# cortes-ciriano-lab/DeMethify

Measured on AMD Instinct MI355X. Metric: NMF update iters/sec (1e6 CpG x 256 samples x 16 types), higher is better.
Workload: dtype f64; 1 GPU; headline_1e6x256_12+4; N_cpg=1000000, S_samples=256, n_known=12, n_unknown=4, inner_iters=20, restarts=64, restart_seed=1 + k, restart_placement=k mod n_gpus, parallelism=restart-sharded x1

## Files before the change

demethify_amd/_lib.py:

```python
from __future__ import annotations

import ctypes as C
from pathlib import Path

LIB_PATH = Path(__file__).resolve().parent / "libdemethify_hip.so"

DMF_OK = 0
DMF_PTR_DEVICE = 1
DMF_INIT_IN_UNIT_RANGE = 4
DMF_SELECT_COUNTS_F32_EXACT, DMF_SELECT_PURITY, DMF_SELECT_ALPHA_OUTSIDE_UNIT, DMF_SELECT_V_UNALIGNED = 1, 2, 4, 8
DMF_SELECT_X16 = 16
DMF_COUNTS_F64 = 2
DMF_WLS_TARGET_V, DMF_WLS_TARGET_DV = 0, 1
DMF_WLS_F64_ARRAYS = 8
DMF_ERR_BAD_ARG, DMF_ERR_NONFINITE, DMF_ERR_UNSUPPORTED = 1, 4, 5
DMF_ERR_BAD_SHAPE = 2
DMF_GRAM_INTEGER, DMF_GRAM_FP64, DMF_GRAM_LAST = 0, 1, 2
DMF_ROUTE_SOLVER, DMF_ROUTE_UPDATE_U = 0, 1
MOMENTUM_SCALARS = ("a1", "a2", "l_w", "l_w_prev", "l_h", "l_h_prev", "dsq", "rt_norm2", "u_norm2", "cf", "cf_prev",
                    "iters", "done", "arrive", "mom_n", "mom_i")
REPORT_INTS = ("N", "S", "n_c", "ND", "SD", "N16", "plane_stride", "has_D16", "has_X16", "has_W16", "has_Dt8", "has_mask_bits",
               "rtp_width", "rtp_borrows_rt", "n_test", "d_f32_exact")
REPORT_DBLS = ("kDsq", "kRtSumsq", "kDmax", "kF32ResidualMax", "kIntCountMax", "kRtOutsideUnit", "x16_dev", "x16_sum")
PROBLEM_ARRAYS = {"V": 0, "D": 1, "Rt": 2, "Rtp": 3, "D16": 4, "X16": 5, "W16": 6, "Dt8": 7, "mask_bits": 8, "consts": 9}
DMF_MODE_PARTIAL = 0
DMF_MODE_UNSUPERVISED = 1
MAX_K = 64
SMALL_MAX_S, SMALL_MAX_K, SMALL_MAX_NU, SMALL_MAX_ELEMENTS = 64, 16, 4, 1 << 20
SVD_MAX_S, SVD_MAX_NC, SVD_MAX_RANK, SVD_MAX_LDS = 512, 64, 64, 160 * 1024


def svd_project_lds_bytes(n_samples, rank):
    return 8 * (n_samples * rank + 8 * ((n_samples + 63) // 64 * 64 + 16) + 512)


KERNEL_ROWPASS, KERNEL_GRAM, KERNEL_ALPHA, KERNEL_COST = 0, 1, 2, 3
KERNEL_FAMILIES = ("rowpass", "gram", "alpha", "cost")

_p = C.c_void_p
_i64 = C.c_int64
_dbl_p = C.POINTER(C.c_double)

SIGNATURES = {
    "dmf_status_string": (C.c_char_p, [C.c_int]),
    "dmf_last_error": (C.c_char_p, []),
    "dmf_abi_version": (C.c_int, []),
    "dmf_context_create": (C.c_int, [C.c_int, _p, C.POINTER(_p)]),
    "dmf_context_destroy": (C.c_int, [_p]),
    "dmf_context_synchronize": (C.c_int, [_p]),
    "dmf_context_set_profiling": (C.c_int, [_p, C.c_int]),
    "dmf_context_kernel_time": (C.c_int, [_p, C.c_int, _dbl_p, C.POINTER(_i64)]),
    "dmf_context_reset_kernel_time": (C.c_int, [_p]),
    "dmf_context_set_generic": (C.c_int, [_p, C.c_int]),
    "dmf_context_set_x16": (C.c_int, [_p, C.c_int]),
    "dmf_context_set_rowpass_pair": (C.c_int, [_p, C.c_int]),
    "dmf_context_set_stop_confirmation": (C.c_int, [_p, C.c_int]),
    "dmf_problem_create": (C.c_int, [_p, _i64, _i64, _i64, _p, _p, _p, C.c_int, C.POINTER(_p)]),
    "dmf_problem_gather": (C.c_int, [_p, _p, _p, _i64, C.POINTER(_p)]),
    "dmf_problem_gather_device": (C.c_int, [_p, _p, _p, _i64, C.POINTER(_p)]),
    "dmf_problem_mask": (C.c_int, [_p, _p, _p, C.c_int, C.POINTER(_p)]),
    "dmf_solver_holdout_error": (C.c_int, [_p, _p, _dbl_p, C.POINTER(_i64)]),
    "dmf_problem_destroy": (C.c_int, [_p]),
    "dmf_problem_shape": (C.c_int, [_p, C.POINTER(_i64), C.POINTER(_i64), C.POINTER(_i64)]),
    "dmf_problem_gram_known": (C.c_int, [_p, _p, C.c_char_p, _i64]),
    "dmf_problem_report": (C.c_int, [_p, C.POINTER(_i64), _dbl_p]),
    "dmf_problem_copy_out": (C.c_int, [_p, C.c_int, _p, _i64]),
    "dmf_gram_i8_describe": (C.c_int, [_i64, _i64, _i64, _i64, C.c_int, C.c_char_p, _i64]),
    "dmf_solver_gram": (C.c_int, [_p, C.c_int, _p, C.c_char_p, _i64]),
    "dmf_solver_row_moments": (C.c_int, [_p, _p, C.c_char_p, _i64]),
    "dmf_solver_momentum_state": (C.c_int, [_p, _dbl_p, _p, _p]),
    "dmf_cost": (C.c_int, [_p, _p, _p, _i64, _p, C.c_int, _dbl_p]),
    "dmf_cost_describe": (C.c_int, [_i64, _i64, _i64, C.c_int, _i64, C.c_int, C.c_int, C.c_int, C.c_char_p, _i64]),
    "dmf_problem_cost_describe": (C.c_int, [_p, _p, _i64, C.c_char_p, _i64]),
    "dmf_project_simplex": (C.c_int, [_p, _p, _i64, _i64, C.c_double, C.c_int, _p]),
    "dmf_update_u": (C.c_int, [_p, _p, _p, _p, _p, _i64, _i64, C.c_int, C.c_int, _dbl_p, _p, _p]),
    "dmf_update_alpha": (C.c_int, [_p, _p, _p, _i64, _p, _p, _i64, C.c_int, _dbl_p, _p, _p]),
    "dmf_wls_intercept": (C.c_int, [_p, _p, _p, _i64, C.c_int, C.c_int, _p, C.POINTER(C.c_int)]),
    "dmf_wls_moments": (C.c_int, [_p, _p, _p, _i64, C.c_int, C.c_int, _p]),
    "dmf_nnls_normal": (C.c_int, [_p, _p, _p, _i64, _i64, _p, C.POINTER(C.c_int)]),
    "dmf_svd_gram": (C.c_int, [_p, _p, _p, C.c_int, _p, C.POINTER(_i64)]),
    "dmf_svd_factor": (C.c_int, [_p, _p, _p, _p, _i64, C.c_int, _p, C.POINTER(_p)]),
    "dmf_svd_finish": (C.c_int, [_p, _p, _i64, _i64, _p, _p, C.c_int, _p]),
    "dmf_percentile_axis0": (C.c_int, [_p, _p, _i64, _i64, _p, _i64, C.c_int, _p]),
    "dmf_nanpercentile_axis0": (C.c_int, [_p, _p, _i64, _i64, _p, _i64, C.c_int, _p]),
    "dmf_solver_create": (C.c_int, [_p, _p, _p, _p, _i64, C.c_int, C.c_int, C.POINTER(_p)]),
    "dmf_solver_set_purity": (C.c_int, [_p, _p, C.c_int]),
    "dmf_solver_step": (C.c_int, [_p, _i64, _i64, C.c_double, C.POINTER(_i64), C.POINTER(C.c_int)]),
    "dmf_solver_get": (C.c_int, [_p, C.c_int, _p, _p, _dbl_p, C.POINTER(_i64)]),
    "dmf_solver_match_components": (C.c_int, [_p, _p, _i64, _p, _p]),
    "dmf_solver_get_u_permuted": (C.c_int, [_p, C.POINTER(C.c_int32), _p]),
    "dmf_solver_get_u_by_row": (C.c_int, [_p, _p, _i64, C.POINTER(C.c_int32), _p]),
    "dmf_solver_cost": (C.c_int, [_p, _dbl_p]),
    "dmf_solver_cost_begin": (C.c_int, [_p]),
    "dmf_solver_cost_end": (C.c_int, [_p, _dbl_p]),
    "dmf_solver_destroy": (C.c_int, [_p]),
    "dmf_solver_describe": (C.c_int, [_p, _i64, C.c_char_p, _i64]),
    "dmf_select_describe": (C.c_int, [_i64, _i64, _i64, _i64, C.c_int, C.c_int, _i64, C.c_int, C.c_char_p, _i64]),
    "dmf_u_phase_describe": (C.c_int, [_i64, _i64, _i64, _i64, C.c_int, C.c_int, _i64, C.c_int, C.c_int, C.c_char_p, _i64]),
    "dmf_solver_u_phase_describe": (C.c_int, [_p, _i64, C.c_int, C.c_char_p, _i64]),
    "dmf_solver_stop_info": (C.c_int, [_p, C.POINTER(C.c_int), C.POINTER(_i64), C.POINTER(_i64), _dbl_p]),
    "dmf_solver_rowpass_launches": (C.c_int, [_p, C.POINTER(_i64), C.POINTER(_i64)]),
    "dmf_table_scan": (C.c_int, [C.c_char_p, C.c_char, C.POINTER(_i64), C.POINTER(C.c_int), C.POINTER(C.c_int),
                                 C.POINTER(C.c_int)]),
    "dmf_table_read": (C.c_int, [C.c_char_p, C.c_char, C.c_int, C.c_int, _i64, _p, _i64, C.c_double, _p, _i64, C.c_int]),
    "dmf_host_alloc": (_p, [C.c_size_t, C.POINTER(C.c_int)]),
    "dmf_host_free": (None, [_p, C.c_int]),
    "dmf_write_interval_csv": (C.c_int, [C.c_char_p, C.c_char_p, _p, _p, _i64, C.c_int, C.c_int, C.c_int]),
    "dmf_stage_upload": (C.c_int, [_p, _p, C.c_size_t, C.POINTER(C.c_void_p)]),
    "dmf_stage_free": (C.c_int, [_p, _p]),
    "dmf_stage_download": (C.c_int, [_p, _p, C.c_size_t, _p]),
    "dmf_mask_draw": (C.c_int, [_p, _p, C.POINTER(C.c_int), _i64, _i64, C.c_uint64, C.POINTER(C.c_void_p),
                                C.POINTER(_i64)]),
    "dmf_solve": (C.c_int, [_p, _p, _p, _p, _i64, C.c_int, _i64, _i64, C.c_double, C.c_int, _p, _p,
                            _dbl_p, C.POINTER(_i64)]),
    "dmf_solve_small_supported": (C.c_int, [_i64, _i64, _i64, _i64, C.c_int]),
    "dmf_solve_small": (C.c_int, [_p, _p, _i64, _p, _p, _p, _i64, C.c_int, _i64, _i64, C.c_double, _i64, C.c_int, _p, _p, _p, _p]),
    "dmf_solve_small_purity": (C.c_int, [_p, _p, _i64, _p, _p, _p, _p, _i64, C.c_int, _i64, _i64, C.c_double, _i64, C.c_int, _p, _p,
                                         _p, _p]),
}

_lib = None


class DemethifyHipError(RuntimeError):

    def __init__(self, status: int, where: str, detail: str = ""):
        self.status = status
        msg = f"{where}: status {status}"
        if detail:
            msg += f" ({detail})"
        super().__init__(msg)


def _preload_torch_hip_runtime():
    import importlib.util
    import os

    if os.environ.get("DEMETHIFY_SYSTEM_HIP") == "1":
        return
    try:
        spec = importlib.util.find_spec("torch")
        if spec is None or not spec.submodule_search_locations:
            return
        cand = Path(list(spec.submodule_search_locations)[0]) / "lib" / "libamdhip64.so"
        if cand.exists():
            C.CDLL(str(cand), mode=C.RTLD_GLOBAL)
    except Exception:
        pass


def load():
    global _lib
    if _lib is not None:
        return _lib
    if not LIB_PATH.exists():
        raise ImportError(
            f"{LIB_PATH} is missing: build it with `python -m demethify_amd._build` "
            "(there is no CPU fallback)")
    import sys

    torch = sys.modules.get("torch")
    if torch is not None:
        try:
            if torch.cuda.is_available():
                torch.cuda.init()
        except Exception:
            pass
    else:
        _preload_torch_hip_runtime()
    lib = C.CDLL(str(LIB_PATH))
    for name, (restype, argtypes) in SIGNATURES.items():
        fn = getattr(lib, name)
        fn.restype = restype
        fn.argtypes = argtypes
    _lib = lib
    return lib


def check(status: int, where: str):
    if status != DMF_OK:
        lib = load()
        text = lib.dmf_status_string(status).decode()
        err = lib.dmf_last_error().decode()
        raise DemethifyHipError(status, where, f"{text}; {err}" if err else text)
```

demethify_amd/csrc/dmf_api.h:

```cpp
#pragma once
#include <hip/hip_runtime.h>

#include <cmath>
#include <cstdio>
#include <cstdlib>
#include <cstring>
#include <memory>
#include <mutex>
#include <new>
#include <unordered_map>
#include <utility>
#include <vector>

#include "../../include/demethify_hip.h"
#include "dmf_internal.h"
#include "dmf_select.h"

using dmf::SolverState;

namespace dmf_api {

int hip_fail(hipError_t e, const char* what, const char* file, int line);

#define HIP_TRY(expr)                                                                          \
    do {                                                                                       \
        hipError_t e_ = (expr);                                                                \
        if (e_ != hipSuccess) return dmf_api::hip_fail(e_, #expr, __FILE_NAME__, __LINE__);    \
    } while (0)

#define DMF_TRY(expr)                 \
    do {                              \
        int s_ = (expr);              \
        if (s_ != DMF_OK) return s_;  \
    } while (0)

constexpr int kEventPool = 2048;

struct FamilyClock {
    std::vector<hipEvent_t> start, stop;
    int used = 0;
    double total_ms = 0.0;
    int64_t launches = 0;
};

}

struct dmf_context {
    int device = 0;
    hipStream_t stream = nullptr;
    bool own_stream = false;
    unsigned profiling = 0;
    int stop_confirmation = 0;
    int generic_level = 0;
    bool x16 = true;
    bool rowpass_pair = true;
    double* scratch = nullptr;
    hipMemPool_t pool = nullptr;
    std::unordered_map<void*, size_t> live;
    std::unordered_map<size_t, std::vector<void*>> kept;
    size_t kept_bytes = 0;
    std::vector<hipEvent_t> events;
    std::vector<double*> pinned_moms;
    std::vector<void*> pinned_states;
    hipStream_t copy_stream = nullptr;
    std::mutex copy_mutex;
    dmf_api::FamilyClock clocks[DMF_KERNEL_FAMILIES];
};

namespace dmf_api {

hipError_t pool_alloc(dmf_context* ctx, void** p, size_t bytes);
void pool_free(dmf_context* ctx, void* p);
hipError_t stage_alloc(dmf_context* ctx, hipStream_t st, void** p, size_t bytes);
void stage_release(dmf_context* ctx, hipStream_t st, void* p);

template <class T>
class DevBuf {
  public:
    DevBuf() = default;
    DevBuf(DevBuf&& o) noexcept : ctx_(o.ctx_), ptr_(o.ptr_), owned_(o.owned_), stage_(o.stage_) {
        o.ptr_ = nullptr, o.owned_ = false;
    }
    DevBuf& operator=(DevBuf&& o) noexcept {
        if (this != &o) {
            reset();
            ctx_ = o.ctx_, ptr_ = o.ptr_, owned_ = o.owned_, stage_ = o.stage_;
            o.ptr_ = nullptr, o.owned_ = false;
        }
        return *this;
    }
    ~DevBuf() { reset(); }
    hipError_t alloc(dmf_context* ctx, size_t count) {
        reset();
        const hipError_t e = pool_alloc(ctx, (void**)&ptr_, count * sizeof(T));
        if (e != hipSuccess) ptr_ = nullptr;
        ctx_ = ctx, owned_ = e == hipSuccess, stage_ = nullptr;
        return e;
    }
    hipError_t alloc_staged(dmf_context* ctx, size_t count, hipStream_t st) {
        reset();
        const hipError_t e = stage_alloc(ctx, st, (void**)&ptr_, count * sizeof(T));
        if (e != hipSuccess) ptr_ = nullptr;
        ctx_ = ctx, owned_ = e == hipSuccess, stage_ = st;
        return e;
    }
    T* release() {
        T* p = ptr_;
        ptr_ = nullptr, owned_ = false;
        return p;
    }
    void borrow(const T* p) { reset(), ptr_ = const_cast<T*>(p); }
    void reset() {
        if (owned_ && stage_ != nullptr) stage_release(ctx_, stage_, ptr_);
        else if (owned_) pool_free(ctx_, ptr_);
        ptr_ = nullptr, owned_ = false;
    }
    T* get() const { return ptr_; }
    operator T*() const { return ptr_; }
    T* operator->() const { return ptr_; }

  private:
    dmf_context* ctx_ = nullptr;
    T* ptr_ = nullptr;
    bool owned_ = false;
    hipStream_t stage_ = nullptr;
};

enum ProblemConst { kDsq, kRtSumsq, kDmax, kF32ResidualMax, kIntCountMax, kRtOutsideUnit, kProblemConsts };

struct JobTable {
    std::vector<short> h_k, h_l;
    std::vector<int> h_dst;
    DevBuf<short> k, l;
    DevBuf<int> dst;
    int n = 0;
    template <class Keep>
    void build(int l_first, int l_last, Keep keep) {
        for (int ll = l_first; ll <= l_last; ++ll)
            for (int kk = 0; kk <= ll; ++kk) {
                if (!keep(kk, ll)) continue;
                h_k.push_back((short)kk);
                h_l.push_back((short)ll);
                h_dst.push_back(dmf::tri(kk, ll));
            }
        n = (int)h_k.size();
    }
    int upload(dmf_context* ctx) {
        HIP_TRY(k.alloc(ctx, n));
        HIP_TRY(l.alloc(ctx, n));
        HIP_TRY(dst.alloc(ctx, n));
        HIP_TRY(hipMemcpyAsync(k, h_k.data(), n * sizeof(short), hipMemcpyHostToDevice, ctx->stream));
        HIP_TRY(hipMemcpyAsync(l, h_l.data(), n * sizeof(short), hipMemcpyHostToDevice, ctx->stream));
        HIP_TRY(hipMemcpyAsync(dst, h_dst.data(), n * sizeof(int), hipMemcpyHostToDevice, ctx->stream));
        return DMF_OK;
    }
};

}

struct dmf_problem {
    dmf_context* ctx = nullptr;
    int64_t N = 0, S = 0, n_c = 0;
    dmf_api::DevBuf<double> V, D, Rt;
    dmf_api::DevBuf<double> Rtp;
    dmf_api::DevBuf<double> consts;
    double h_consts[dmf_api::kProblemConsts] = {};
    dmf_api::DevBuf<unsigned short> D16;
    dmf_api::DevBuf<signed char> Dt8;
    int ND = 0;
    int SD = 0;
    int64_t N16 = 0, plane_stride = 0;
    dmf_api::DevBuf<unsigned short> X16;
    double x16_dev = 0.0, x16_sum = 0.0;
    bool d_f32_exact = false;
    dmf_api::DevBuf<double> gb_known;
    dmf::GramRan known_ran;
    dmf_api::DevBuf<unsigned char> mask_bits;
    dmf_api::DevBuf<unsigned short> W16;
    int64_t n_test = 0;
    dmf::ProblemView view() const {
        dmf::ProblemView v;
        v.V = V, v.D = D, v.D16 = D16, v.X16 = X16, v.Dt8 = Dt8;
        v.plane_stride = plane_stride, v.SD = SD, v.ND = ND;
        v.Rt = Rt, v.Rtp = Rtp;
        v.N = N, v.S = (int)S, v.n_c = (int)n_c;
        return v;
    }
};

constexpr size_t kPinnedStateBytes = (sizeof(SolverState) + 15) / 16 * 16 + 16;

struct dmf_solver {
    dmf_context* ctx = nullptr;
    const dmf_problem* p = nullptr;
    int64_t n_u = 0;
    int mode = 0;
    dmf::ShapeKey key;
    dmf::PathSpec spec;
    dmf_api::DevBuf<double> cm;
    dmf_api::DevBuf<double> beta_tab;
    int64_t beta_cap = 0;
    dmf_api::DevBuf<long long> slab_i8;
    int64_t slab_i8_words = 0;
    dmf_api::DevBuf<long long> acc_i8;
    dmf_api::DevBuf<double> purity;
    dmf_api::DevBuf<double> u2_partials;
    dmf_api::DevBuf<double> u, u_prev, u_next;
    dmf_api::DevBuf<double> alpha, alpha_prev;
    dmf_api::DevBuf<double> gb;
    dmf::GramRan last_gram;
    int last_gram_source = -1;
    dmf_api::DevBuf<double> slab;
    int64_t slab_doubles = 0;
    dmf_api::DevBuf<double> partials;
    dmf_api::DevBuf<SolverState> state;
    SolverState* h_state = nullptr;
    dmf_api::JobTable jobs;
    bool cf_pending = true;
    double* mom_host = nullptr;
    dmf_api::DevBuf<double> mom_dev;
    hipEvent_t cost_event = nullptr;
    bool cost_pending = false;
    bool in_flight = false;
    bool confirm_stops = false;
    double cf_stream = 0.0;
    long long cf_stream_iter = -1;
    long long n_rowpass = 0, n_rowpass_pair = 0;
    long long n_confirmed = 0, n_unconfirmed = 0;
    dmf::IterateView iterate() const {
        dmf::IterateView it;
        it.u = u, it.u_prev = u_prev, it.alpha = alpha, it.state = state;
        it.n_u = (int)n_u, it.mode = mode;
        return it;
    }
    dmf::AlphaView alpha_view() const {
        dmf::AlphaView a;
        a.gb = gb, a.alpha = alpha, a.alpha_prev = alpha_prev, a.purity = purity, a.state = state, a.partials = partials;
        a.S = (int)p->S, a.n_c = (int)p->n_c, a.n_u = (int)n_u;
        return a;
    }
    dmf::UScratch scratch() const {
        dmf::UScratch sc;
        sc.cm = cm, sc.beta = beta_tab, sc.slab = slab, sc.u2_partials = u2_partials;
        return sc;
    }
};

namespace dmf_api {

struct HandleDeleter {
    void operator()(dmf_problem* p) const { dmf_problem_destroy(p); }
    void operator()(dmf_solver* s) const { dmf_solver_destroy(s); }
};
using ProblemPtr = std::unique_ptr<dmf_problem, HandleDeleter>;
using SolverPtr = std::unique_ptr<dmf_solver, HandleDeleter>;

int clock_drain(dmf_context* ctx, FamilyClock& c);

struct FamilyScope {
    dmf_context* ctx;
    FamilyClock* c = nullptr;
    int slot = -1;
    FamilyScope(dmf_context* ctx_, int family) : ctx(ctx_) {
        if (!((ctx->profiling >> family) & 1u)) return;
        c = &ctx->clocks[family];
        if (c->start.empty()) {
            c->start.resize(kEventPool);
            c->stop.resize(kEventPool);
            for (int i = 0; i < kEventPool; ++i) {
                hipEventCreateWithFlags(&c->start[i], hipEventDisableSystemFence);
                hipEventCreateWithFlags(&c->stop[i], hipEventDisableSystemFence);
            }
        }
        if (c->used == kEventPool) clock_drain(ctx, *c);
        slot = c->used++;
        hipEventRecord(c->start[slot], ctx->stream);
    }
    ~FamilyScope() {
        if (c != nullptr) hipEventRecord(c->stop[slot], ctx->stream);
    }
};

int check_ctx(dmf_context* ctx);

template <class T>
int import_array(dmf_context* ctx, const void* src, size_t count, int flags, DevBuf<T>& dst) {
    dst.reset();
    if (count == 0) return DMF_OK;
    if (flags & DMF_PTR_DEVICE) {
        dst.borrow(static_cast<const T*>(src));
        return DMF_OK;
    }
    HIP_TRY(dst.alloc(ctx, count));
    HIP_TRY(hipMemcpyAsync(dst, src, count * sizeof(T), hipMemcpyHostToDevice, ctx->stream));
    HIP_TRY(hipStreamSynchronize(ctx->stream));
    return DMF_OK;
}
int export_array(dmf_context* ctx, const void* dev_src, size_t bytes, int flags, void* dst);

hipError_t enqueue_cost(dmf_context* ctx, const dmf::ProblemView& p, const double* u, const double* alpha, int n_u,
                        double* scratch, double* out);
bool cost_reads_u16_only(dmf_context* ctx, const dmf::ProblemView& p, int n_u);
int cost_to_host(dmf_context* ctx, const dmf::ProblemView& p, const double* u, const double* alpha, int n_u,
                 double* host_slot, bool wait);

int enqueue_u_phase(dmf_solver* s, int n_iter2, dmf::RowKind row);
dmf::RowKind standalone_row_kind(const dmf_solver* s, int n_iter2);
int enqueue_gram(dmf_solver* s, dmf::GramKind kind, bool heed_done = true, dmf::GramRan* ran = nullptr);
dmf::GramKind fp64_gram_kind(const dmf_solver* s);
int enqueue_alpha_phase(dmf_solver* s, dmf::AlphaKind kind, int n_iter2);
int fetch_state(dmf_solver* s);
int push_state(dmf_solver* s);

}
```

demethify_amd/csrc/dmf_api_context.hip:

```cpp
#include "dmf_api.h"

namespace dmf_api {

static thread_local char g_last_error[512] = "";

int hip_fail(hipError_t e, const char* what, const char* file, int line) {
    snprintf(g_last_error, sizeof(g_last_error), "%s failed at %s:%d: %s", what, file, line, hipGetErrorString(e));
    return DMF_ERR_HIP;
}

int clock_drain(dmf_context* ctx, FamilyClock& c) {
    if (c.used == 0) return DMF_OK;
    HIP_TRY(hipStreamSynchronize(ctx->stream));
    for (int i = 0; i < c.used; ++i) {
        float ms = 0.f;
        HIP_TRY(hipEventElapsedTime(&ms, c.start[i], c.stop[i]));
        c.total_ms += ms;
    }
    c.launches += c.used;
    c.used = 0;
    return DMF_OK;
}

static bool pool_enabled() {
    static const bool on = [] {
        const char* v = getenv("DEMETHIFY_NO_POOL");
        return !(v != nullptr && v[0] == '1');
    }();
    return on;
}
constexpr size_t kKeepMinBytes = (size_t)1 << 20, kKeepBytes = (size_t)24 << 30;
constexpr int kKeepPerSize = 3;
hipError_t pool_alloc(dmf_context* ctx, void** p, size_t bytes) {
    if (!pool_enabled() || ctx->pool == nullptr) return hipMalloc(p, bytes);
    if (bytes >= kKeepMinBytes) {
        auto it = ctx->kept.find(bytes);
        if (it != ctx->kept.end() && !it->second.empty()) {
            *p = it->second.back();
            it->second.pop_back();
            ctx->kept_bytes -= bytes;
            ctx->live[*p] = bytes;
            return hipSuccess;
        }
    }
    hipError_t e = hipMallocFromPoolAsync(p, bytes, ctx->pool, ctx->stream);
    if (e != hipSuccess && ctx->kept_bytes > 0) {
        (void)hipGetLastError();
        for (auto& kv : ctx->kept)
            for (void* q : kv.second) (void)hipFreeAsync(q, ctx->stream);
        ctx->kept.clear();
        ctx->kept_bytes = 0;
        (void)hipStreamSynchronize(ctx->stream);
        e = hipMallocFromPoolAsync(p, bytes, ctx->pool, ctx->stream);
    }
    if (e == hipSuccess && bytes >= kKeepMinBytes) ctx->live[*p] = bytes;
    return e;
}
void pool_free(dmf_context* ctx, void* p) {
    if (p == nullptr) return;
    if (!pool_enabled() || ctx->pool == nullptr) {
        (void)hipStreamSynchronize(ctx->stream);
        (void)hipFree(p);
        return;
    }
    auto it = ctx->live.find(p);
    if (it != ctx->live.end()) {
        const size_t bytes = it->second;
        ctx->live.erase(it);
        auto& slot = ctx->kept[bytes];
        if ((int)slot.size() < kKeepPerSize && ctx->kept_bytes + bytes <= kKeepBytes) {
            slot.push_back(p);
            ctx->kept_bytes += bytes;
            return;
        }
    }
    (void)hipFreeAsync(p, ctx->stream);
}

hipError_t stage_alloc(dmf_context* ctx, hipStream_t st, void** p, size_t bytes) {
    if (!pool_enabled() || ctx->pool == nullptr) return hipMalloc(p, bytes);
    return hipMallocFromPoolAsync(p, bytes, ctx->pool, st);
}
void stage_release(dmf_context* ctx, hipStream_t st, void* p) {
    if (!pool_enabled() || ctx->pool == nullptr) (void)hipFree(p);
    else (void)hipFreeAsync(p, st);
}

int export_array(dmf_context* ctx, const void* dev_src, size_t bytes, int flags, void* dst) {
    if (bytes == 0 || dst == nullptr) return DMF_OK;
    const hipMemcpyKind kind = (flags & DMF_PTR_DEVICE) ? hipMemcpyDeviceToDevice : hipMemcpyDeviceToHost;
    HIP_TRY(hipMemcpyAsync(dst, dev_src, bytes, kind, ctx->stream));
    HIP_TRY(hipStreamSynchronize(ctx->stream));
    return DMF_OK;
}

int check_ctx(dmf_context* ctx) {
    if (ctx == nullptr) return DMF_ERR_BAD_ARG;
    HIP_TRY(hipSetDevice(ctx->device));
    return DMF_OK;
}

}

using namespace dmf_api;

extern "C" {

const char* dmf_status_string(int status) {
    switch (status) {
        case DMF_OK: return "ok";
        case DMF_ERR_BAD_ARG: return "bad argument";
        case DMF_ERR_BAD_SHAPE: return "shape mismatch";
        case DMF_ERR_HIP: return "HIP runtime error";
        case DMF_ERR_NONFINITE: return "non-finite input";
        case DMF_ERR_UNSUPPORTED: return "unsupported size";
        case DMF_ERR_NO_DEVICE: return "no gfx950 device";
        default: return "unknown status";
    }
}

const char* dmf_last_error(void) { return g_last_error; }

int dmf_abi_version(void) { return 1; }

int dmf_context_create(int device, void* stream, dmf_context** out) {
    if (out == nullptr) return DMF_ERR_BAD_ARG;
    *out = nullptr;
    int count = 0;
    if (hipGetDeviceCount(&count) != hipSuccess || count <= 0) return DMF_ERR_NO_DEVICE;
    if (device < 0 || device >= count) return DMF_ERR_BAD_ARG;
    HIP_TRY(hipSetDevice(device));
    hipDeviceProp_t prop;
    HIP_TRY(hipGetDeviceProperties(&prop, device));
    if (strncmp(prop.gcnArchName, "gfx950", 6) != 0) {
        snprintf(g_last_error, sizeof(g_last_error), "device %d is %s, this library is built for gfx950",
                 device, prop.gcnArchName);
        return DMF_ERR_NO_DEVICE;
    }
    dmf_context* ctx = new (std::nothrow) dmf_context();
    if (ctx == nullptr) return DMF_ERR_BAD_ARG;
    ctx->device = device;
    if (stream != nullptr) {
        ctx->stream = (hipStream_t)stream;
    } else {
        hipError_t e = hipStreamCreateWithFlags(&ctx->stream, hipStreamNonBlocking);
        if (e != hipSuccess) {
            delete ctx;
            return hip_fail(e, "hipStreamCreate", __FILE_NAME__, __LINE__);
        }
        ctx->own_stream = true;
    }
    hipError_t e = hipMalloc((void**)&ctx->scratch, 4096 * sizeof(double));
    if (e != hipSuccess) {
        if (ctx->own_stream) hipStreamDestroy(ctx->stream);
        delete ctx;
        return hip_fail(e, "hipMalloc(scratch)", __FILE_NAME__, __LINE__);
    }
    if (pool_enabled()) {
        hipMemPoolProps props = {};
        props.allocType = hipMemAllocationTypePinned;
        props.handleTypes = hipMemHandleTypeNone;
        props.location.type = hipMemLocationTypeDevice;
        props.location.id = device;
        if (hipMemPoolCreate(&ctx->pool, &props) == hipSuccess && ctx->pool != nullptr) {
            uint64_t keep = UINT64_MAX;
            (void)hipMemPoolSetAttribute(ctx->pool, hipMemPoolAttrReleaseThreshold, &keep);
        } else {
            ctx->pool = nullptr;
            (void)hipGetLastError();
        }
    }
    *out = ctx;
    return DMF_OK;
}

int dmf_context_destroy(dmf_context* ctx) {
    if (ctx == nullptr) return DMF_OK;
    hipSetDevice(ctx->device);
    hipStreamSynchronize(ctx->stream);
    for (auto& c : ctx->clocks) {
        for (auto ev : c.start) hipEventDestroy(ev);
        for (auto ev : c.stop) hipEventDestroy(ev);
    }
    hipFree(ctx->scratch);
    for (auto& kv : ctx->kept)
        for (void* q : kv.second) (void)hipFreeAsync(q, ctx->stream);
    ctx->kept.clear();
    (void)hipStreamSynchronize(ctx->stream);
    for (void* h : ctx->pinned_states) (void)hipHostFree(h);
    for (double* h : ctx->pinned_moms) (void)hipHostFree(h);
    for (hipEvent_t ev : ctx->events) (void)hipEventDestroy(ev);
    if (ctx->copy_stream != nullptr) {
        hipStreamSynchronize(ctx->copy_stream);
        hipStreamDestroy(ctx->copy_stream);
    }
    if (ctx->pool != nullptr) (void)hipMemPoolDestroy(ctx->pool);
    if (ctx->own_stream) hipStreamDestroy(ctx->stream);
    delete ctx;
    return DMF_OK;
}

int dmf_stage_upload(dmf_context* ctx, const void* host, size_t bytes, void** out_dev) {
    if (ctx == nullptr || host == nullptr || out_dev == nullptr || bytes == 0) return DMF_ERR_BAD_ARG;
    HIP_TRY(hipSetDevice(ctx->device));
    std::lock_guard<std::mutex> lock(ctx->copy_mutex);
    if (ctx->copy_stream == nullptr) HIP_TRY(hipStreamCreateWithFlags(&ctx->copy_stream, hipStreamNonBlocking));
    void* d = nullptr;
    HIP_TRY(stage_alloc(ctx, ctx->copy_stream, &d, bytes));
    hipError_t e = hipMemcpyAsync(d, host, bytes, hipMemcpyHostToDevice, ctx->copy_stream);
    e = e != hipSuccess ? e : hipStreamSynchronize(ctx->copy_stream);
    if (e != hipSuccess) {
        stage_release(ctx, ctx->copy_stream, d);
        return hip_fail(e, "dmf_stage_upload", __FILE_NAME__, __LINE__);
    }
    *out_dev = d;
    return DMF_OK;
}

int dmf_stage_download(dmf_context* ctx, const void* dev, size_t bytes, void* host) {
    if (ctx == nullptr || dev == nullptr || host == nullptr || bytes == 0) return DMF_ERR_BAD_ARG;
    HIP_TRY(hipSetDevice(ctx->device));
    std::lock_guard<std::mutex> lock(ctx->copy_mutex);
    if (ctx->copy_stream == nullptr) HIP_TRY(hipStreamCreateWithFlags(&ctx->copy_stream, hipStreamNonBlocking));
    HIP_TRY(hipMemcpyAsync(host, dev, bytes, hipMemcpyDeviceToHost, ctx->copy_stream));
    HIP_TRY(hipStreamSynchronize(ctx->copy_stream));
    return DMF_OK;
}

int dmf_mask_draw(dmf_context* ctx, uint32_t key[624], int* pos, int64_t N, int64_t S, uint64_t threshold, void** out_bits,
                  int64_t* n_kept) {
    if (ctx == nullptr || key == nullptr || pos == nullptr || out_bits == nullptr || n_kept == nullptr) return DMF_ERR_BAD_ARG;
    *out_bits = nullptr;
    if (*pos < 0 || *pos > 624 || N < 1 || S < 1 || threshold > ((uint64_t)1 << 53)) return DMF_ERR_BAD_ARG;
    if (S > dmf::kMaskDrawMaxS || N > dmf::kMaskDrawMaxElements / S) return DMF_ERR_UNSUPPORTED;
    HIP_TRY(hipSetDevice(ctx->device));
    std::lock_guard<std::mutex> lock(ctx->copy_mutex);
    if (ctx->copy_stream == nullptr) HIP_TRY(hipStreamCreateWithFlags(&ctx->copy_stream, hipStreamNonBlocking));
    const hipStream_t st = ctx->copy_stream;
    constexpr size_t kStateWords = 624 + 4;
    DevBuf<unsigned char> bits;
    DevBuf<uint32_t> state;
    HIP_TRY(bits.alloc_staged(ctx, (size_t)N * (size_t)((S + 7) / 8), st));
    HIP_TRY(state.alloc_staged(ctx, kStateWords, st));
    uint32_t h_state[kStateWords] = {};
    std::memcpy(h_state, key, 624 * sizeof(uint32_t));
    HIP_TRY(hipMemcpyAsync(state, h_state, sizeof(h_state), hipMemcpyHostToDevice, st));
    HIP_TRY(dmf::launch_mask_draw(state, *pos, N, S, threshold, bits, reinterpret_cast<unsigned long long*>(state + 624), st));
    HIP_TRY(hipMemcpyAsync(h_state, state, sizeof(h_state), hipMemcpyDeviceToHost, st));
    HIP_TRY(hipStreamSynchronize(st));
    unsigned long long result[2];
    std::memcpy(result, h_state + 624, sizeof(result));
    std::memcpy(key, h_state, 624 * sizeof(uint32_t));
    *pos = (int)result[1];
    *n_kept = (int64_t)result[0];
    *out_bits = bits.release();
    return DMF_OK;
}

int dmf_stage_free(dmf_context* ctx, void* dev) {
    if (ctx == nullptr) return DMF_ERR_BAD_ARG;
    if (dev == nullptr) return DMF_OK;
    HIP_TRY(hipSetDevice(ctx->device));
    pool_free(ctx, dev);
    return DMF_OK;
}

int dmf_context_synchronize(dmf_context* ctx) {
    DMF_TRY(check_ctx(ctx));
    HIP_TRY(hipStreamSynchronize(ctx->stream));
    return DMF_OK;
}

int dmf_context_set_profiling(dmf_context* ctx, int enabled) {
    DMF_TRY(check_ctx(ctx));
    if (!enabled)
        for (auto& c : ctx->clocks) DMF_TRY(clock_drain(ctx, c));
    ctx->profiling = enabled == 0 ? 0u : enabled == 1 ? ~0u : (unsigned)enabled >> 1;
    return DMF_OK;
}

int dmf_context_kernel_time(dmf_context* ctx, int family, double* total_ms, int64_t* launches) {
    DMF_TRY(check_ctx(ctx));
    if (family < 0 || family >= DMF_KERNEL_FAMILIES) return DMF_ERR_BAD_ARG;
    FamilyClock& c = ctx->clocks[family];
    DMF_TRY(clock_drain(ctx, c));
    if (total_ms) *total_ms = c.total_ms;
    if (launches) *launches = c.launches;
    return DMF_OK;
}

int dmf_context_reset_kernel_time(dmf_context* ctx) {
    DMF_TRY(check_ctx(ctx));
    for (auto& c : ctx->clocks) {
        DMF_TRY(clock_drain(ctx, c));
        c.total_ms = 0.0;
        c.launches = 0;
    }
    return DMF_OK;
}

int dmf_context_set_generic(dmf_context* ctx, int enabled) {
    if (ctx == nullptr) return DMF_ERR_BAD_ARG;
    if (enabled < 0 || enabled > 4) return DMF_ERR_BAD_ARG;
    ctx->generic_level = enabled;
    return DMF_OK;
}

int dmf_context_set_x16(dmf_context* ctx, int enabled) {
    if (ctx == nullptr || enabled < 0 || enabled > 1) return DMF_ERR_BAD_ARG;
    ctx->x16 = enabled != 0;
    return DMF_OK;
}

int dmf_context_set_rowpass_pair(dmf_context* ctx, int enabled) {
    if (ctx == nullptr || enabled < 0 || enabled > 1) return DMF_ERR_BAD_ARG;
    ctx->rowpass_pair = enabled != 0;
    return DMF_OK;
}

int dmf_context_set_stop_confirmation(dmf_context* ctx, int mode) {
    if (ctx == nullptr || mode < 0 || mode > 2) return DMF_ERR_BAD_ARG;
    ctx->stop_confirmation = mode;
    return DMF_OK;
}

}
```

demethify_amd/csrc/dmf_api_solver.hip:

```cpp
#include "dmf_api.h"

namespace dmf_api {

using dmf::kSplitInnerSteps;

static int ensure_split_scratch(dmf_solver* s, int n_iter2) {
    dmf_context* ctx = s->ctx;
    if (s->cm == nullptr) HIP_TRY(s->cm.alloc(ctx, (size_t)dmf::u_phase_split_cm_doubles(s->p->N, (int)s->n_u)));
    if (s->beta_cap < n_iter2 || s->beta_tab == nullptr) {
        s->beta_cap = n_iter2 > 0 ? n_iter2 : 1;
        HIP_TRY(s->beta_tab.alloc(ctx, (size_t)s->beta_cap));
    }
    return DMF_OK;
}

int enqueue_u_phase(dmf_solver* s, int n_iter2, dmf::RowKind row) {
    dmf_context* ctx = s->ctx;
    const dmf::ProblemView pv = s->p->view();
    FamilyScope scope(ctx, DMF_KERNEL_ROWPASS);
    switch (row) {
        case dmf::RowKind::CmI8InnerRows:
            DMF_TRY(ensure_split_scratch(s, n_iter2));
            HIP_TRY(dmf::launch_u_phase_split_i8(pv, s->iterate(), n_iter2, s->scratch(), ctx->stream));
            return DMF_OK;
        case dmf::RowKind::UPhaseBig:
            HIP_TRY(dmf::launch_u_phase_big(pv, s->iterate(), n_iter2, ctx->stream));
            return DMF_OK;
        case dmf::RowKind::UPhaseMfmaSplit:
            DMF_TRY(ensure_split_scratch(s, n_iter2));
            HIP_TRY(dmf::launch_u_phase_split(pv, s->iterate(), n_iter2, s->scratch(), ctx->stream));
            return DMF_OK;
        case dmf::RowKind::UPhaseMfma:
            HIP_TRY(dmf::launch_u_phase_mfma(pv, s->iterate(), n_iter2, ctx->stream));
            return DMF_OK;
        case dmf::RowKind::UPhaseGram:
            HIP_TRY(dmf::launch_u_phase_gram(pv, s->iterate(), n_iter2, ctx->stream));
            return DMF_OK;
        case dmf::RowKind::UStepDirect:
            for (int t = 0; t < n_iter2; ++t) {
                HIP_TRY(dmf::launch_u_step_direct(pv, s->iterate(), s->u_next, t, ctx->stream));
                std::swap(s->u_prev, s->u);
                std::swap(s->u, s->u_next);
            }
            return DMF_OK;
        default: return DMF_ERR_BAD_ARG;
    }
}

dmf::RowKind standalone_row_kind(const dmf_solver* s, int n_iter2) {
    return dmf::plan_iteration(s->key, dmf::standalone_spec(s->spec), n_iter2, false).row;
}

struct GramI8Buffers {
    double* slab_bu = nullptr;
    long long* slab_i8 = nullptr;
    int64_t slab_i8_words = 0;
    long long* acc = nullptr;
    double* gb = nullptr;
    const int* done = nullptr;
};

static GramI8Buffers solver_i8_buffers(dmf_solver* s) {
    GramI8Buffers b;
    b.slab_bu = s->slab, b.slab_i8 = s->slab_i8, b.slab_i8_words = s->slab_i8_words, b.acc = s->acc_i8, b.gb = s->gb;
    b.done = &s->state->done;
    return b;
}

static int gram_i8_and_reduce(dmf_solver* s, const GramI8Buffers& b, int n_slabs, const double* u2_partials, int n_u2,
                              dmf::GramRan* ran = nullptr) {
    dmf_context* ctx = s->ctx;
    const dmf_problem* p = s->p;
    const int S = (int)p->S, n_c = (int)p->n_c, n_u = (int)s->n_u, nf = n_c * n_u + n_u * (n_u + 1) / 2;
    int ny = 0;
    HIP_TRY(dmf::launch_gram_i8(p->view(), s->u, n_u, s->jobs.k, s->jobs.l, nf, b.slab_i8, b.slab_i8_words, b.done, &ny,
                                ctx->stream, ran));
    HIP_TRY(dmf::launch_gram_v2_reduce(b.slab_i8, ny, nf, p->SD, b.slab_bu, n_slabs, n_u, S, b.acc, s->jobs.dst, b.gb, b.done,
                                       u2_partials, n_u2, s->state, ctx->stream));
    return DMF_OK;
}

static int gram_bu_cols_i8(dmf_solver* s, const GramI8Buffers& b, dmf::GramRan* ran = nullptr) {
    int n_slabs = 0;
    HIP_TRY(dmf::launch_bu_cols(s->p->view(), s->u, (int)s->n_u, b.slab_bu, b.done, &n_slabs, s->ctx->stream));
    return gram_i8_and_reduce(s, b, n_slabs, nullptr, 0, ran);
}

int enqueue_gram(dmf_solver* s, dmf::GramKind kind, bool heed_done, dmf::GramRan* ran) {
    dmf_context* ctx = s->ctx;
    const dmf::ProblemView pv = s->p->view();
    const int S = pv.S, n_u = (int)s->n_u;
    const int* done = heed_done ? &s->state->done : nullptr;
    FamilyScope scope(ctx, DMF_KERNEL_GRAM);
    if (kind == dmf::GramKind::BuColsI8) {
        GramI8Buffers b = solver_i8_buffers(s);
        b.done = done;
        return gram_bu_cols_i8(s, b, ran);
    }
    if (kind == dmf::GramKind::GramU) {
        int ny = 0;
        HIP_TRY(dmf::launch_gram_u(pv, s->u, n_u, s->slab, done, &ny, ctx->stream, ran));
        HIP_TRY(dmf::launch_gram_reduce(s->slab, ny, s->jobs.n, S, s->jobs.dst, s->gb, done, ctx->stream));
        return DMF_OK;
    }
    dmf::GramJobTable jobs{s->jobs.k, s->jobs.l, s->jobs.dst, s->jobs.n};
    if (kind == dmf::GramKind::GramMfma) {
        int ny = 0;
        HIP_TRY(dmf::launch_gram_mfma(pv, s->u, n_u, jobs, s->jobs.n - n_u, s->slab, s->slab_doubles, done, &ny, ctx->stream, ran));
        HIP_TRY(dmf::launch_gram_reduce(s->slab, ny, s->jobs.n, S, s->jobs.dst, s->gb, done, ctx->stream));
        return DMF_OK;
    }
    HIP_TRY(dmf::launch_gram(pv, s->u, n_u, jobs, s->slab, s->slab_doubles, s->gb, done, ctx->stream, ran));
    return DMF_OK;
}

dmf::GramKind fp64_gram_kind(const dmf_solver* s) {
    return s->spec.use_gram_spec ? dmf::GramKind::GramU : s->spec.use_gram_mfma ? dmf::GramKind::GramMfma : dmf::GramKind::Gram;
}

int enqueue_alpha_phase(dmf_solver* s, dmf::AlphaKind kind, int n_iter2) {
    FamilyScope scope(s->ctx, DMF_KERNEL_ALPHA);
    HIP_TRY(dmf::launch_alpha(kind, s->alpha_view(), n_iter2, s->ctx->stream));
    return DMF_OK;
}

constexpr int kLastGramI8Tail = 100, kLastGramFused = 101;
static dmf::GramRan* last_gram_slot(dmf_solver* s, int source) {
    if (s->last_gram_source == source) return nullptr;
    s->last_gram_source = source;
    return &s->last_gram;
}

static int enqueue_gram_i8_tail(dmf_solver* s, dmf::AlphaKind alpha, int n_iter2, int grid) {
    {
        FamilyScope scope(s->ctx, DMF_KERNEL_GRAM);
        DMF_TRY(gram_i8_and_reduce(s, solver_i8_buffers(s), grid, s->u2_partials, grid, last_gram_slot(s, kLastGramI8Tail)));
    }
    return enqueue_alpha_phase(s, alpha, n_iter2);
}

static int enqueue_outer_iteration(dmf_solver* s, int n_iter2) {
    dmf_context* ctx = s->ctx;
    s->in_flight = true;
    const dmf_problem* p = s->p;
    const int S = (int)p->S;
    const dmf::IterationPlan plan = dmf::plan_iteration(s->key, s->spec, n_iter2, s->purity != nullptr);
    if (plan.row == dmf::RowKind::RowpassV2) {
        int grid = 0;
        bool paired = false;
        {
            FamilyScope scope(ctx, DMF_KERNEL_ROWPASS);
            dmf::ProblemView pv = p->view();
            if (!s->key.x16) pv.X16 = nullptr;
            HIP_TRY(dmf::launch_rowpass_v2(pv, s->iterate(), n_iter2, s->scratch(), &grid, s->key.rowpass_pair, &paired,
                                           ctx->stream));
            ++s->n_rowpass;
            s->n_rowpass_pair += paired ? 1 : 0;
        }
        return enqueue_gram_i8_tail(s, plan.alpha, n_iter2, grid);
    }
    if (plan.row == dmf::RowKind::CmI8InnerBu) {
        int grid = 0;
        DMF_TRY(ensure_split_scratch(s, n_iter2));
        {
            FamilyScope scope(ctx, DMF_KERNEL_ROWPASS);
            HIP_TRY(dmf::launch_u_phase_split_i8_bu(p->view(), s->iterate(), n_iter2, s->scratch(), &grid, ctx->stream));
        }
        return enqueue_gram_i8_tail(s, plan.alpha, n_iter2, grid);
    }
    if (plan.row == dmf::RowKind::RowpassFused) {
        const int64_t n_full = p->N - (p->N & 15), n_tail = p->N - n_full;
        const dmf::ProblemView pv = p->view();
        int grid = 0, ny_tail = 0;
        {
            FamilyScope scope(ctx, DMF_KERNEL_ROWPASS);
            HIP_TRY(dmf::launch_rowpass_fused(pv.rows(0, n_full), s->iterate(), n_iter2, s->scratch(), &grid, ctx->stream));
        }
        if (n_tail > 0) {
            const dmf::ProblemView tail = pv.rows(n_full, n_tail);
            const dmf::IterateView it_tail = s->iterate().rows(n_full);
            HIP_TRY(dmf::launch_u_phase_mfma(tail, it_tail, n_iter2, ctx->stream));
            HIP_TRY(dmf::launch_sumsq_f64(it_tail.u, n_tail * s->n_u, ctx->scratch, s->u2_partials + grid, &s->state->done,
                                          ctx->stream));
            HIP_TRY(dmf::launch_gram_u(tail, it_tail.u, it_tail.n_u, s->slab + (int64_t)2 * grid * s->jobs.n * S,
                                       &s->state->done, &ny_tail, ctx->stream));
        }
        if (dmf::GramRan* ran = last_gram_slot(s, kLastGramFused))
            snprintf(ran->text, sizeof(ran->text), "k_rowpass_fused<%d,%d> phase C slabs=%d%s", (int)(p->n_c + 3) / 4, (int)s->n_u,
                     2 * grid, n_tail > 0 ? " + k_gram_u tail" : "");
        HIP_TRY(dmf::launch_finish_u_norm(s->u2_partials, grid + (n_tail > 0 ? 1 : 0), s->state, ctx->stream));
        {
            FamilyScope scope(ctx, DMF_KERNEL_GRAM);
            HIP_TRY(dmf::launch_gram_reduce(s->slab, 2 * grid + ny_tail, s->jobs.n, S, s->jobs.dst, s->gb,
                                            &s->state->done, ctx->stream));
        }
        return enqueue_alpha_phase(s, plan.alpha, n_iter2);
    }
    DMF_TRY(enqueue_u_phase(s, n_iter2, plan.row));
    HIP_TRY(dmf::launch_sumsq_f64(s->u, p->N * s->n_u, ctx->scratch, &s->state->u_norm2, &s->state->done,
                                  ctx->stream));
    HIP_TRY(dmf::launch_set_lh(s->state, ctx->stream));
    DMF_TRY(enqueue_gram(s, plan.gram, true, last_gram_slot(s, (int)plan.gram)));
    return enqueue_alpha_phase(s, plan.alpha, n_iter2);
}

int fetch_state(dmf_solver* s) {
    HIP_TRY(hipMemcpyAsync(s->h_state, s->state, sizeof(SolverState), hipMemcpyDeviceToHost, s->ctx->stream));
    HIP_TRY(hipStreamSynchronize(s->ctx->stream));
    s->in_flight = false;
    return DMF_OK;
}

int push_state(dmf_solver* s) {
    HIP_TRY(hipMemcpyAsync(s->state, s->h_state, sizeof(SolverState), hipMemcpyHostToDevice, s->ctx->stream));
    HIP_TRY(hipStreamSynchronize(s->ctx->stream));
    return DMF_OK;
}

constexpr int kMomRows = 64, kMomSteps = 64;

__global__ void k_set_momentum(SolverState* state, const double* mom, int stride, int rows, int n) {
    state->mom = mom;
    state->mom_stride = stride;
    state->mom_rows = rows;
    state->mom_i = 0;
    state->mom_n = n;
}

static double momentum_advance(double& a) {
#pragma clang fp contract(off)
    const double a0 = a;
    const double sq = 4.0 * a0 * a0;
    a = (1.0 + std::sqrt(1.0 + sq)) / 2.0;
    return (a0 - 1.0) / a;
}

static int upload_momentum_rows(dmf_solver* s, int rows, int n) {
    dmf_context* ctx = s->ctx;
    const int stride = 2 + 2 * n;
    if (s->mom_host == nullptr) {
        if (!ctx->pinned_moms.empty()) {
            s->mom_host = ctx->pinned_moms.back();
            ctx->pinned_moms.pop_back();
        } else {
            HIP_TRY(hipHostMalloc((void**)&s->mom_host, (size_t)kMomRows * (2 + 2 * kMomSteps) * sizeof(double)));
        }
        HIP_TRY(s->mom_dev.alloc(ctx, (size_t)kMomRows * (2 + 2 * kMomSteps)));
    }
    double a1 = s->h_state->a1, a2 = s->h_state->a2;
    for (int r = 0; r < rows; ++r) {
        double* row = s->mom_host + (size_t)r * stride;
        for (int t = 0; t < n; ++t) {
            row[2 + t] = momentum_advance(a1);
            row[2 + n + t] = momentum_advance(a2);
        }
        row[0] = a1;
        row[1] = a2;
    }
    HIP_TRY(hipMemcpyAsync(s->mom_dev, s->mom_host, (size_t)rows * stride * sizeof(double), hipMemcpyHostToDevice, ctx->stream));
    hipLaunchKernelGGL(k_set_momentum, dim3(1), dim3(1), 0, ctx->stream, s->state.get(), (const double*)s->mom_dev.get(), stride,
                       rows, n);
    HIP_TRY(hipGetLastError());
    return DMF_OK;
}

__global__ void k_set_tol(SolverState* state, double tol, double band) {
    state->tol = tol;
    state->band = band;
}

constexpr double kConfirmBand = 10.0;
constexpr double kGramCostRelErr = 1e-15;

static double* cost_slot(const dmf_solver* s) {
    return reinterpret_cast<double*>(reinterpret_cast<char*>(s->h_state) + kPinnedStateBytes - 16);
}

static int solver_setup(dmf_solver* s, const double* u0, const double* alpha0, int flags) {
    dmf_context* ctx = s->ctx;
    const dmf_problem* p = s->p;
    const int64_t N = p->N, S = p->S, n_c = p->n_c, n_u = s->n_u, K = n_c + n_u;
    dmf::ShapeKey& key = s->key;
    key.N = N;
    key.S = (int)S;
    key.n_c = (int)n_c;
    key.n_u = (int)n_u;
    key.nd = (p->ND > 0 && p->D16 != nullptr) ? p->ND : 0;
    key.SD = p->SD;
    key.x16 = key.nd > 0 && p->X16 != nullptr;
    key.rowpass_pair = ctx->rowpass_pair;
    key.level = ctx->generic_level;
    key.d_f32_exact = p->d_f32_exact;
    key.rtp_present = n_c == 0 || p->Rtp != nullptr;
    key.v_align = (unsigned)(reinterpret_cast<uintptr_t>(p->V.get()) & 15);
    key.rtp_align = (unsigned)(reinterpret_cast<uintptr_t>(p->Rtp.get()) & 15);
    key.alpha_unit = true;
    s->spec = dmf::select_path(key);
    if ((s->spec.use_v2 || s->spec.use_cm_i8) && !(flags & DMF_INIT_IN_UNIT_RANGE)) {
        bool in_unit = true;
        if (flags & DMF_PTR_DEVICE) {
            double outside = 0.0;
            HIP_TRY(dmf::launch_unit_range_check(alpha0, K * S, ctx->scratch, ctx->scratch + 2048, ctx->stream));
            HIP_TRY(hipMemcpyAsync(&outside, ctx->scratch + 2048, sizeof(double), hipMemcpyDeviceToHost, ctx->stream));
            HIP_TRY(hipStreamSynchronize(ctx->stream));
            in_unit = outside == 0.0;
        } else {
            for (int64_t i = 0; i < K * S; ++i)
                if (!(alpha0[i] >= 0.0 && alpha0[i] <= 1.0)) {
                    in_unit = false;
                    break;
                }
        }
        if (!in_unit) {
            key.alpha_unit = false;
            s->spec = dmf::select_path(key);
        }
    }
    if (!s->spec.supported) return DMF_ERR_UNSUPPORTED;
    s->in_flight = true;
    s->jobs.build((int)n_c, (int)K, [n_c, K](int k, int l) {
        if (l == (int)K && k < (int)n_c) return false;
        return !(l == (int)K && k == (int)K);
    });
    const int n_jobs = s->jobs.n;
    s->slab_doubles = dmf::gram_slab_doubles(N, (int)S, n_jobs);
    if (s->spec.use_gram_spec) {
        const int64_t spec = dmf::gram_u_slab_doubles(N, (int)S, (int)n_c, (int)n_u);
        if (spec > s->slab_doubles) s->slab_doubles = spec;
    }
    if (s->spec.use_gram_mfma) {
        const int64_t need = dmf::gram_mfma_slab_doubles(N, (int)S, n_jobs);
        if (need > s->slab_doubles) s->slab_doubles = need;
    }
    if (s->spec.use_fused) {
        const int64_t spec = dmf::rowpass_fused_slab_doubles(N - (N & 15), (int)S, (int)n_c, (int)n_u) +
                             dmf::gram_u_slab_doubles(16, (int)S, (int)n_c, (int)n_u);
        if (spec > s->slab_doubles) s->slab_doubles = spec;
    }
    if (s->spec.use_v2) {
        const int64_t bu = (int64_t)dmf::rowpass_v2_grid(N, (int)S) * n_u * S;
        if (bu > s->slab_doubles) s->slab_doubles = bu;
    }
    if (s->spec.use_gram_i8) {
        const int64_t bu = (int64_t)dmf::bu_cols_grid(N) * n_u * S;
        if (bu > s->slab_doubles) s->slab_doubles = bu;
        if (s->spec.use_cm_i8) {
            const int64_t bu2 = (int64_t)dmf::u_inner_bu_grid(N, (int)S) * n_u * S;
            if (bu2 > s->slab_doubles) s->slab_doubles = bu2;
        }
    }
    const size_t un = (size_t)N * n_u, an = (size_t)K * S;
    const size_t un_alloc = (un + 1) & ~(size_t)1;
    const size_t gbn = (size_t)(K + 1) * (K + 2) / 2 * S;
    const int nb_alpha = (int)((S + 63) / 64);
    HIP_TRY(s->u.alloc(ctx, un_alloc));
    HIP_TRY(s->u_prev.alloc(ctx, un_alloc));
    if (s->spec.u_path == 2) HIP_TRY(s->u_next.alloc(ctx, un_alloc));
    HIP_TRY(s->alpha.alloc(ctx, an));
    HIP_TRY(s->alpha_prev.alloc(ctx, an));
    HIP_TRY(s->gb.alloc(ctx, gbn));
    HIP_TRY(s->slab.alloc(ctx, (size_t)s->slab_doubles));
    HIP_TRY(s->partials.alloc(ctx, (size_t)2 * (nb_alpha + S)));
    HIP_TRY(s->u2_partials.alloc(ctx, 4096));
    if (s->spec.use_v2 || s->spec.use_gram_i8) {
        s->slab_i8_words = dmf::gram_i8_slab_words(N, p->SD, (int)n_c, (int)n_u);
        HIP_TRY(s->slab_i8.alloc(ctx, (size_t)s->slab_i8_words));
        const size_t acc_words = (size_t)dmf::gram_i8_acc_words((int)S, (int)n_c, (int)n_u);
        HIP_TRY(s->acc_i8.alloc(ctx, acc_words));
        HIP_TRY(hipMemsetAsync(s->acc_i8, 0, acc_words * sizeof(long long), ctx->stream));
    }
    HIP_TRY(s->state.alloc(ctx, 1));
    if (!ctx->pinned_states.empty()) {
        s->h_state = (SolverState*)ctx->pinned_states.back();
        ctx->pinned_states.pop_back();
    } else {
        HIP_TRY(hipHostMalloc((void**)&s->h_state, kPinnedStateBytes));
    }
    const hipMemcpyKind in_kind = (flags & DMF_PTR_DEVICE) ? hipMemcpyDeviceToDevice : hipMemcpyHostToDevice;
    HIP_TRY(hipMemsetAsync(s->state, 0, sizeof(SolverState), ctx->stream));
    HIP_TRY(hipMemsetAsync(s->gb, 0, gbn * sizeof(double), ctx->stream));
    HIP_TRY(hipMemcpyAsync(s->u, u0, un * sizeof(double), in_kind, ctx->stream));
    HIP_TRY(hipMemcpyAsync(s->u_prev, s->u, un * sizeof(double), hipMemcpyDeviceToDevice, ctx->stream));
    HIP_TRY(hipMemcpyAsync(s->alpha, alpha0, an * sizeof(double), in_kind, ctx->stream));
    HIP_TRY(hipMemcpyAsync(s->alpha_prev, s->alpha, an * sizeof(double), hipMemcpyDeviceToDevice, ctx->stream));
    DMF_TRY(s->jobs.upload(ctx));
    HIP_TRY(dmf::launch_scatter_known_block(p->gb_known, s->gb, (int)n_c, (int)K, (int)S, ctx->stream));
    HIP_TRY(dmf::launch_sumsq_f64(s->u, N * n_u, ctx->scratch, &s->state->u_norm2, nullptr, ctx->stream));
    HIP_TRY(dmf::launch_init_state(s->state, p->consts, s->alpha, (int)S, (int)n_c, (int)n_u, ctx->stream));
    if (!(flags & DMF_PTR_DEVICE)) HIP_TRY(hipStreamSynchronize(ctx->stream));
    return DMF_OK;
}

}

using namespace dmf_api;

extern "C" {

int dmf_solver_create(dmf_context* ctx, const dmf_problem* p, const double* u0, const double* alpha0,
                      int64_t n_u, int mode, int flags, dmf_solver** out) {
    DMF_TRY(check_ctx(ctx));
    if (out == nullptr) return DMF_ERR_BAD_ARG;
    *out = nullptr;
    if (p == nullptr || u0 == nullptr || alpha0 == nullptr || n_u < 1) return DMF_ERR_BAD_ARG;
    if (mode != DMF_MODE_PARTIAL && mode != DMF_MODE_UNSUPERVISED) return DMF_ERR_BAD_ARG;
    if (p->n_c + n_u > dmf::kMaxK) return DMF_ERR_UNSUPPORTED;
    SolverPtr s(new (std::nothrow) dmf_solver());
    if (s == nullptr) return DMF_ERR_BAD_ARG;
    s->ctx = ctx;
    s->p = p;
    s->n_u = n_u;
    s->mode = mode;
    DMF_TRY(solver_setup(s.get(), u0, alpha0, flags));
    *out = s.release();
    return DMF_OK;
}

int dmf_solver_step(dmf_solver* s, int64_t n_outer, int64_t n_iter2, double tol,
                    int64_t* iters_done_total, int* converged) {
    if (s == nullptr || n_outer < 0 || n_iter2 < 0 || n_iter2 > (1 << 20)) return DMF_ERR_BAD_ARG;
    dmf_context* ctx = s->ctx;
    DMF_TRY(check_ctx(ctx));
    const dmf_problem* p = s->p;
    const double gram_err = kGramCostRelErr * (double)p->N * (double)p->S * p->h_consts[kDmax] +
                            (s->key.x16 ? p->x16_dev * p->x16_sum : 0.0);
    s->confirm_stops = tol > 0.0 && ctx->stop_confirmation != 2 && (ctx->stop_confirmation == 1 || gram_err >= tol / 20.0);
    hipLaunchKernelGGL(k_set_tol, dim3(1), dim3(1), 0, ctx->stream, s->state.get(), tol, s->confirm_stops ? kConfirmBand : 1.0);
    HIP_TRY(hipGetLastError());
    if (s->cf_pending && tol > 0.0 && n_outer > 0) {
        FamilyScope scope(ctx, DMF_KERNEL_COST);
        HIP_TRY(enqueue_cost(ctx, p->view(), s->u, s->alpha, (int)s->n_u, ctx->scratch + 1024, &s->state->cf));
        s->cf_pending = false;
        s->cf_stream_iter = -2;
    }
    DMF_TRY(fetch_state(s));
    if (s->cf_stream_iter == -2) {
        s->cf_stream = s->h_state->cf;
        s->cf_stream_iter = s->h_state->iters;
    }
    int64_t check_every = s->spec.u_path != 2 ? 8 : 1;
    if (tol == 0.0 && s->spec.u_path != 2) check_every = kMomRows;
    const long long iters0 = s->h_state->iters;
    const dmf::IterationPlan plan = dmf::plan_iteration(s->key, s->spec, (int)n_iter2, s->purity != nullptr);
    const bool use_mom = n_iter2 >= 1 && n_iter2 <= kMomSteps && plan.row == dmf::RowKind::RowpassV2 &&
                         plan.alpha == dmf::AlphaKind::PhaseRow16;
    if (!use_mom && s->h_state->mom_n >= 0) {
        hipLaunchKernelGGL(k_set_momentum, dim3(1), dim3(1), 0, ctx->stream, s->state.get(), (const double*)nullptr, 0, 0, -1);
        HIP_TRY(hipGetLastError());
    }
    while (s->h_state->iters - iters0 < n_outer && s->h_state->done != 1) {
        const int64_t left = n_outer - (s->h_state->iters - iters0);
        const int64_t batch = left < check_every ? left : check_every;
        if (use_mom) DMF_TRY(upload_momentum_rows(s, (int)batch, (int)n_iter2));
        for (int64_t b = 0; b < batch; ++b) DMF_TRY(enqueue_outer_iteration(s, (int)n_iter2));
        DMF_TRY(fetch_state(s));
        if (s->h_state->iters > iters0) s->cf_pending = false;
        if (s->h_state->done == 2) {
            double cs = 0.0;
            DMF_TRY(cost_to_host(ctx, p->view(), s->u, s->alpha, (int)s->n_u, &cs, true));
            bool stop;
            if (s->cf_stream_iter == s->h_state->iters - 1) {
                stop = std::fabs(cs - s->cf_stream) < tol;
                s->n_confirmed += 1;
            } else {
                stop = std::fabs(s->h_state->cf - s->h_state->cf_prev) < tol;
                s->n_unconfirmed += 1;
            }
            s->cf_stream = cs;
            s->cf_stream_iter = s->h_state->iters;
            s->h_state->done = stop ? 1 : 0;
            DMF_TRY(push_state(s));
            check_every = 1;
        } else if (s->spec.u_path != 2 && check_every < 64 && check_every > 1) {
            check_every *= 2;
        }
    }
    if (iters_done_total) *iters_done_total = s->h_state->iters;
    if (converged) *converged = s->h_state->done == 1;
    return DMF_OK;
}

int dmf_solver_set_purity(dmf_solver* s, const double* purity, int flags) {
    if (s == nullptr || purity == nullptr) return DMF_ERR_BAD_ARG;
    dmf_context* ctx = s->ctx;
    DMF_TRY(check_ctx(ctx));
    if (s->mode != DMF_MODE_PARTIAL) return DMF_ERR_BAD_ARG;
    const size_t bytes = (size_t)s->p->S * sizeof(double);
    if (s->purity == nullptr) HIP_TRY(s->purity.alloc(ctx, (size_t)s->p->S));
    const hipMemcpyKind kind = (flags & DMF_PTR_DEVICE) ? hipMemcpyDeviceToDevice : hipMemcpyHostToDevice;
    HIP_TRY(hipMemcpyAsync(s->purity, purity, bytes, kind, ctx->stream));
    HIP_TRY(hipStreamSynchronize(ctx->stream));
    return DMF_OK;
}

int dmf_solver_get(dmf_solver* s, int flags, double* out_u, double* out_alpha, double* out_cost,
                   int64_t* out_iters) {
    if (s == nullptr) return DMF_ERR_BAD_ARG;
    dmf_context* ctx = s->ctx;
    DMF_TRY(check_ctx(ctx));
    const dmf_problem* p = s->p;
    DMF_TRY(export_array(ctx, s->u, (size_t)p->N * s->n_u * sizeof(double), flags, out_u));
    DMF_TRY(export_array(ctx, s->alpha, (size_t)(p->n_c + s->n_u) * p->S * sizeof(double), flags, out_alpha));
    if (s->cf_pending && out_cost != nullptr) {
        FamilyScope scope(ctx, DMF_KERNEL_COST);
        HIP_TRY(enqueue_cost(ctx, p->view(), s->u, s->alpha, (int)s->n_u, ctx->scratch + 1024, &s->state->cf));
        s->cf_pending = false;
    }
    DMF_TRY(fetch_state(s));
    if (out_cost) *out_cost = s->h_state->cf;
    if (out_iters) *out_iters = s->h_state->iters;
    return DMF_OK;
}

int dmf_solver_cost(dmf_solver* s, double* out_cost) {
    if (s == nullptr || out_cost == nullptr) return DMF_ERR_BAD_ARG;
    DMF_TRY(check_ctx(s->ctx));
    return cost_to_host(s->ctx, s->p->view(), s->u, s->alpha, (int)s->n_u, out_cost, true);
}

int dmf_solver_cost_begin(dmf_solver* s) {
    if (s == nullptr) return DMF_ERR_BAD_ARG;
    dmf_context* ctx = s->ctx;
    DMF_TRY(check_ctx(ctx));
    if (s->cost_event == nullptr) {
        if (!ctx->events.empty()) {
            s->cost_event = ctx->events.back();
            ctx->events.pop_back();
        } else {
            HIP_TRY(hipEventCreateWithFlags(&s->cost_event, hipEventDisableTiming));
        }
    }
    DMF_TRY(cost_to_host(ctx, s->p->view(), s->u, s->alpha, (int)s->n_u, cost_slot(s), false));
    HIP_TRY(hipEventRecord(s->cost_event, ctx->stream));
    s->cost_pending = true;
    return DMF_OK;
}

int dmf_solver_cost_end(dmf_solver* s, double* out_cost) {
    if (s == nullptr || out_cost == nullptr || !s->cost_pending) return DMF_ERR_BAD_ARG;
    DMF_TRY(check_ctx(s->ctx));
    HIP_TRY(hipEventSynchronize(s->cost_event));
    s->cost_pending = false;
    *out_cost = *cost_slot(s);
    return DMF_OK;
}

int dmf_solver_holdout_error(dmf_solver* s, const dmf_problem* full, double* sum_sq, int64_t* n_test) {
    if (s == nullptr || full == nullptr || sum_sq == nullptr || n_test == nullptr) return DMF_ERR_BAD_ARG;
    dmf_context* ctx = s->ctx;
    DMF_TRY(check_ctx(ctx));
    const dmf_problem* p = s->p;
    if (p->mask_bits == nullptr || full->mask_bits != nullptr || full->ctx != ctx) return DMF_ERR_BAD_ARG;
    if (full->N != p->N || full->S != p->S || full->n_c != p->n_c) return DMF_ERR_BAD_SHAPE;
    *n_test = p->n_test;
    *sum_sq = 0.0;
    if (p->n_test == 0) return DMF_OK;
    dmf::ProblemView pv;
    pv.N = p->N, pv.S = (int)p->S, pv.n_c = (int)p->n_c;
    pv.V = full->V, pv.Rt = p->Rt, pv.Rtp = p->Rtp;
    pv.D16 = p->W16, pv.SD = p->SD;
    DevBuf<double> weights;
    if (!cost_reads_u16_only(ctx, pv, (int)s->n_u)) {
        HIP_TRY(weights.alloc(ctx, (size_t)p->N * p->S));
        HIP_TRY(dmf::launch_holdout_weights_f64(p->mask_bits, weights, p->N, (int)p->S, ctx->stream));
        pv.D = weights, pv.D16 = nullptr, pv.SD = 0;
    }
    return cost_to_host(ctx, pv, s->u, s->alpha, (int)s->n_u, sum_sq, true);
}

static int solver_gram_enqueue(dmf_solver* s, int kind, double* out_gb, dmf::GramRan* ran) {
    dmf_context* ctx = s->ctx;
    const dmf_problem* p = s->p;
    const int64_t N = p->N, S = p->S, n_c = p->n_c, n_u = s->n_u, K = n_c + n_u;
    const size_t gbn = (size_t)(K + 1) * (K + 2) / 2 * S;
    DevBuf<double> slab_bu;
    DevBuf<long long> slab_i8, acc;
    if (kind == DMF_GRAM_LAST) {
        *ran = s->last_gram;
    } else if (kind == DMF_GRAM_FP64) {
        DMF_TRY(enqueue_gram(s, fp64_gram_kind(s), false, ran));
    } else {
        GramI8Buffers b;
        b.slab_i8_words = dmf::gram_i8_slab_words(N, p->SD, (int)n_c, (int)n_u);
        const size_t acc_words = (size_t)dmf::gram_i8_acc_words((int)S, (int)n_c, (int)n_u);
        HIP_TRY(slab_bu.alloc(ctx, (size_t)dmf::bu_cols_grid(N) * n_u * S));
        HIP_TRY(slab_i8.alloc(ctx, (size_t)b.slab_i8_words));
        HIP_TRY(acc.alloc(ctx, acc_words));
        HIP_TRY(hipMemsetAsync(acc, 0, acc_words * sizeof(long long), ctx->stream));
        b.slab_bu = slab_bu, b.slab_i8 = slab_i8, b.acc = acc, b.gb = s->gb;
        FamilyScope scope(ctx, DMF_KERNEL_GRAM);
        DMF_TRY(gram_bu_cols_i8(s, b, ran));
    }
    HIP_TRY(hipMemcpyAsync(out_gb, s->gb, gbn * sizeof(double), hipMemcpyDeviceToHost, ctx->stream));
    HIP_TRY(hipStreamSynchronize(ctx->stream));
    return DMF_OK;
}

int dmf_solver_gram(dmf_solver* s, int kind, double* out_gb, char* out_text, int64_t cap) {
    if (s == nullptr || out_gb == nullptr || (kind != DMF_GRAM_INTEGER && kind != DMF_GRAM_FP64 && kind != DMF_GRAM_LAST))
        return DMF_ERR_BAD_ARG;
    if (out_text != nullptr && cap < 1) return DMF_ERR_BAD_ARG;
    dmf_context* ctx = s->ctx;
    DMF_TRY(check_ctx(ctx));
    const dmf_problem* p = s->p;
    if (kind == DMF_GRAM_INTEGER &&
        (p->ND < 1 || p->D16 == nullptr || p->Dt8 == nullptr || (p->n_c > 0 && p->Rtp == nullptr) ||
         (reinterpret_cast<uintptr_t>(p->Rtp.get()) & 15) != 0 ||
         !dmf::gram_i8_supported((int)p->n_c, (int)s->n_u, p->ND, p->N, p->SD)))
        return DMF_ERR_UNSUPPORTED;
    dmf::GramRan ran;
    s->in_flight = true;
    const int status = solver_gram_enqueue(s, kind, out_gb, &ran);
    if (status != DMF_OK) (void)hipStreamSynchronize(ctx->stream);
    s->in_flight = false;
    if (status == DMF_OK && out_text != nullptr) snprintf(out_text, (size_t)cap, "%s", ran.text);
    return status;
}

static dmf::RowKind row_moments_kind(const dmf_solver* s) { return standalone_row_kind(s, kSplitInnerSteps + 1); }

static int solver_row_moments_enqueue(dmf_solver* s, dmf::RowKind row, double* out_cm, dmf::CmRan* ran) {
    dmf_context* ctx = s->ctx;
    const dmf::ProblemView pv = s->p->view();
    const int n_iter2 = kSplitInnerSteps + 1;
    DMF_TRY(ensure_split_scratch(s, 1));
    {
        FamilyScope scope(ctx, DMF_KERNEL_ROWPASS);
        if (row == dmf::RowKind::UPhaseMfmaSplit) {
            HIP_TRY(dmf::launch_u_phase_mfma_impl(pv, s->iterate(), n_iter2, s->cm, ctx->stream));
            dmf::describe_row_launch(dmf::u_phase_mfma_plan(pv.N, pv.S, pv.n_c, (int)s->n_u, n_iter2, pv.D16 != nullptr, pv.SD, true),
                                     ran->text, sizeof(ran->text));
        } else {
            HIP_TRY(dmf::launch_cm_i8(pv, s->iterate(), s->cm, ctx->stream, ran));
        }
    }
    const size_t n = (size_t)dmf::u_phase_split_cm_doubles(pv.N, (int)s->n_u);
    HIP_TRY(hipMemcpyAsync(out_cm, s->cm, n * sizeof(double), hipMemcpyDeviceToHost, ctx->stream));
    HIP_TRY(hipStreamSynchronize(ctx->stream));
    return DMF_OK;
}

int dmf_solver_row_moments(dmf_solver* s, double* out_cm, char* out_text, int64_t cap) {
    if (s == nullptr || out_cm == nullptr || (out_text != nullptr && cap < 1)) return DMF_ERR_BAD_ARG;
    dmf_context* ctx = s->ctx;
    DMF_TRY(check_ctx(ctx));
    const dmf::RowKind row = row_moments_kind(s);
    if (row != dmf::RowKind::CmI8InnerRows && row != dmf::RowKind::CmI8InnerBu && row != dmf::RowKind::UPhaseMfmaSplit)
        return DMF_ERR_UNSUPPORTED;
    DMF_TRY(fetch_state(s));
    if (s->h_state->done != 0) return DMF_ERR_BAD_ARG;
    dmf::CmRan ran;
    s->in_flight = true;
    const int status = solver_row_moments_enqueue(s, row, out_cm, &ran);
    if (status != DMF_OK) (void)hipStreamSynchronize(ctx->stream);
    s->in_flight = false;
    if (status == DMF_OK && out_text != nullptr) snprintf(out_text, (size_t)cap, "%s", ran.text);
    return status;
}

int dmf_solver_momentum_state(const dmf_solver* s, double* scalars, double* alpha_prev, double* u_prev) {
    if (s == nullptr || scalars == nullptr) return DMF_ERR_BAD_ARG;
    dmf_context* ctx = s->ctx;
    DMF_TRY(check_ctx(ctx));
    const dmf_problem* p = s->p;
    SolverState st;
    HIP_TRY(hipMemcpyAsync(&st, s->state.get(), sizeof(SolverState), hipMemcpyDeviceToHost, ctx->stream));
    if (alpha_prev != nullptr)
        HIP_TRY(hipMemcpyAsync(alpha_prev, s->alpha_prev.get(), (size_t)(p->n_c + s->n_u) * p->S * sizeof(double), hipMemcpyDeviceToHost,
                               ctx->stream));
    if (u_prev != nullptr)
        HIP_TRY(hipMemcpyAsync(u_prev, s->u_prev.get(), (size_t)p->N * s->n_u * sizeof(double), hipMemcpyDeviceToHost, ctx->stream));
    HIP_TRY(hipStreamSynchronize(ctx->stream));
    const double out[DMF_MOMENTUM_SCALARS] = {st.a1, st.a2, st.l_w, st.l_w_prev, st.l_h, st.l_h_prev, st.dsq, st.rt_norm2,
                                              st.u_norm2, st.cf, st.cf_prev, (double)st.iters, (double)st.done,
                                              (double)st.arrive, (double)st.mom_n, (double)st.mom_i};
    for (int i = 0; i < DMF_MOMENTUM_SCALARS; ++i) scalars[i] = out[i];
    return DMF_OK;
}

int dmf_solver_destroy(dmf_solver* s) {
    if (s == nullptr) return DMF_OK;
    dmf_context* ctx = s->ctx;
    hipSetDevice(ctx->device);
    if (s->cost_pending) (void)hipEventSynchronize(s->cost_event);
    if (s->in_flight) (void)hipStreamSynchronize(ctx->stream);
    if (s->cost_event) ctx->events.push_back(s->cost_event);
    if (s->mom_host) ctx->pinned_moms.push_back(s->mom_host);
    if (s->h_state) ctx->pinned_states.push_back(s->h_state);
    delete s;
    return DMF_OK;
}

int dmf_solver_describe(const dmf_solver* s, int64_t n_iter2, char* buf, int64_t cap) {
    if (s == nullptr || buf == nullptr || cap < 1 || n_iter2 < 0) return DMF_ERR_BAD_ARG;
    const dmf::IterationPlan plan = dmf::plan_iteration(s->key, s->spec, (int)n_iter2, s->purity != nullptr);
    dmf::describe_plan(s->key, plan, buf, (size_t)cap);
    return DMF_OK;
}

int dmf_solver_u_phase_describe(const dmf_solver* s, int64_t n_iter2, int route, char* buf, int64_t cap) {
    if (s == nullptr || buf == nullptr || cap < 1 || n_iter2 < 0 || n_iter2 > (1 << 20) ||
        (route != DMF_ROUTE_SOLVER && route != DMF_ROUTE_UPDATE_U))
        return DMF_ERR_BAD_ARG;
    dmf::describe_u_phase(s->key, s->spec, (int)n_iter2, s->purity != nullptr, route == DMF_ROUTE_UPDATE_U, buf, (size_t)cap);
    return DMF_OK;
}

int dmf_solver_stop_info(const dmf_solver* s, int* confirm_stops, int64_t* n_confirmed, int64_t* n_unconfirmed,
                         double* last_stream_cost) {
    if (s == nullptr) return DMF_ERR_BAD_ARG;
    if (confirm_stops) *confirm_stops = s->confirm_stops ? 1 : 0;
    if (n_confirmed) *n_confirmed = s->n_confirmed;
    if (n_unconfirmed) *n_unconfirmed = s->n_unconfirmed;
    if (last_stream_cost) *last_stream_cost = s->cf_stream_iter >= 0 ? s->cf_stream : std::nan("");
    return DMF_OK;
}

int dmf_solver_rowpass_launches(const dmf_solver* s, int64_t* total, int64_t* paired) {
    if (s == nullptr) return DMF_ERR_BAD_ARG;
    if (total) *total = s->n_rowpass;
    if (paired) *paired = s->n_rowpass_pair;
    return DMF_OK;
}

int dmf_solve(dmf_context* ctx, const dmf_problem* p, const double* u0, const double* alpha0, int64_t n_u,
              int mode, int64_t n_iter1, int64_t n_iter2, double tol, int flags, double* out_u,
              double* out_alpha, double* out_cost, int64_t* out_iters) {
    dmf_solver* raw = nullptr;
    DMF_TRY(dmf_solver_create(ctx, p, u0, alpha0, n_u, mode, flags, &raw));
    SolverPtr s(raw);
    DMF_TRY(dmf_solver_step(raw, n_iter1, n_iter2, tol, nullptr, nullptr));
    return dmf_solver_get(raw, flags, out_u, out_alpha, out_cost, out_iters);
}

}
```

demethify_amd/csrc/dmf_internal.h:

```cpp
#pragma once
#include <hip/hip_runtime.h>
#include <stdint.h>

#include "dmf_select.h"

namespace dmf {

struct SolverState {
    double a1;
    double a2;
    double l_w;
    double l_w_prev;
    double l_h;
    double l_h_prev;
    double dsq;
    double rt_norm2;
    double u_norm2;
    double cf;
    double cf_prev;
    double tol;
    long long iters;
    double band;
    int done;
    int arrive;
    const double* mom;
    int mom_stride, mom_rows, mom_i, mom_n;
};

__device__ __forceinline__ const double* momentum_row(const SolverState* __restrict__ state, int n_iter2) {
    return (state->mom != nullptr && state->mom_n == n_iter2 && state->mom_i < state->mom_rows)
               ? state->mom + (int64_t)state->mom_i * state->mom_stride
               : nullptr;
}

__host__ __device__ inline int tri(int k, int l) { return l * (l + 1) / 2 + k; }

constexpr int kMaxK = 64;
constexpr int kGramChunk = 16;
constexpr int kRowsPerBlockU = 64;

struct GramJobTable {
    const short* k_idx;
    const short* l_idx;
    const int* dst_row;
    int count;
};

struct PercentilePlan {
    long long k_prev, k_next;
    double gamma;
    int from_top;
    int pad;
};

struct ProblemView {
    const double* V = nullptr;
    const double* D = nullptr;
    const unsigned short* D16 = nullptr;
    const unsigned short* X16 = nullptr;
    const signed char* Dt8 = nullptr;
    int64_t plane_stride = 0;
    int SD = 0, ND = 0;
    const double* Rt = nullptr;
    const double* Rtp = nullptr;
    int64_t N = 0;
    int S = 0, n_c = 0;
    unsigned v_align() const { return (unsigned)(reinterpret_cast<uintptr_t>(V) & 15); }
    ProblemView rows(int64_t first, int64_t count) const {
        ProblemView r;
        r.V = V + first * S;
        r.D = D + first * S;
        r.Rt = Rt ? Rt + first * n_c : nullptr;
        r.Rtp = Rtp ? Rtp + first * ((n_c + 3) / 4 * 4) : nullptr;
        r.N = count;
        r.S = S;
        r.n_c = n_c;
        return r;
    }
};

struct IterateView {
    double* u = nullptr;
    double* u_prev = nullptr;
    const double* alpha = nullptr;
    SolverState* state = nullptr;
    int n_u = 0, mode = 0;
    IterateView rows(int64_t first) const {
        IterateView r = *this;
        r.u = u + first * n_u;
        r.u_prev = u_prev + first * n_u;
        return r;
    }
};

struct AlphaView {
    const double* gb = nullptr;
    double* alpha = nullptr;
    double* alpha_prev = nullptr;
    const double* purity = nullptr;
    SolverState* state = nullptr;
    double* partials = nullptr;
    int S = 0, n_c = 0, n_u = 0;
};

struct UScratch {
    double* cm = nullptr;
    double* beta = nullptr;
    double* slab = nullptr;
    double* u2_partials = nullptr;
};


hipError_t launch_convert_counts(const long long* src, double* dst, int64_t n, hipStream_t st);
hipError_t launch_max_f64(const double* x, int64_t n, double* scratch, double* out, hipStream_t st);
hipError_t launch_f32_residual_max(const double* x, int64_t n, double* scratch, double* out, hipStream_t st);
hipError_t launch_int_count_max(const double* x, int64_t n, double* scratch, double* out, hipStream_t st);
hipError_t launch_unit_range_check(const double* x, int64_t n, double* scratch, double* out, hipStream_t st);
hipError_t launch_sumsq_f64(const double* x, int64_t n, double* scratch, double* out,
                            const int* done_flag, hipStream_t st);
hipError_t launch_pad_rows(const double* src, double* dst, int64_t n_rows, int width_src, int width_dst,
                           hipStream_t st);
hipError_t launch_index_range_check(const long long* idx, int64_t n_idx, int64_t n_src, unsigned int* flag, hipStream_t st);
hipError_t launch_gather_rows(const double* src, double* dst, const long long* idx, int64_t n_idx,
                              int64_t width, hipStream_t st);

inline CostKey cost_key(const ProblemView& p, int n_u, int level) {
    CostKey k;
    k.S = p.S, k.n_c = p.n_c, k.n_u = n_u;
    k.d16 = p.D16 != nullptr;
    k.SD = p.SD;
    k.v_align = p.v_align();
    k.rtp_present = p.Rtp != nullptr;
    k.level = level;
    return k;
}
hipError_t launch_cost_plan(const CostPlan& plan, const ProblemView& p, const double* u, const double* alpha, int n_u,
                            double* scratch, double* out, hipStream_t st);
int vdv_cols_grid(int64_t N);
hipError_t launch_vdv_cols(const ProblemView& p, double* slab, double* out, hipStream_t st);

struct GramRan {
    char text[192] = "";
};

hipError_t launch_gram(const ProblemView& p, const double* u, int n_u, GramJobTable jobs, double* slab, int64_t slab_doubles,
                       double* gb, const int* done_flag, hipStream_t st, GramRan* ran = nullptr);
int64_t gram_slab_doubles(int64_t N, int S, int n_jobs);
hipError_t launch_gram_reduce(const double* slab, int ny, int n_jobs, int S, const int* dst_row,
                              double* gb, const int* done_flag, hipStream_t st);
bool gram_u_supported(int n_c, int n_u);
int64_t gram_u_slab_doubles(int64_t N, int S, int n_c, int n_u);
hipError_t launch_gram_u(const ProblemView& p, const double* u, int n_u, double* slab, const int* done_flag, int* ny_out,
                         hipStream_t st, GramRan* ran = nullptr);

struct RowLaunch {
    bool supported = false;
    int nw = 0;
    int grid = 0;
    size_t lds = 0;
    bool raise = false;
    int64_t blocks_per_wg = 0;
};
struct UPhaseMfmaPlan : RowLaunch {
    int nkc = 0, nu = 0;
    bool vec = false, d16 = false;
    bool split = false;
};
UPhaseMfmaPlan u_phase_mfma_plan(int64_t N, int S, int n_c, int n_u, int n_iter2, bool has_d16, int SD, bool split);
struct RowpassFusedPlan : RowLaunch {
    int nkc = 0, nu = 0;
};
RowpassFusedPlan rowpass_fused_plan(int64_t N, int S, int n_c, int n_u, int n_iter2);
struct UPhaseBigPlan : RowLaunch {
    int nkc = 0, gs = 16, n_u = 0;
};
UPhaseBigPlan u_phase_big_plan(int64_t N, int S, int n_c, int n_u, int n_iter2);
struct UPhaseGramPlan : RowLaunch {
    int nu = 0;
    bool alpha_in_lds = false;
};
UPhaseGramPlan u_phase_gram_plan(int64_t N, int S, int n_c, int n_u);
struct UStepDirectPlan : RowLaunch {
    int n_u = 0;
};
UStepDirectPlan u_step_direct_plan(int64_t N, int S, int n_c, int n_u);
int describe_row_launch(const UPhaseMfmaPlan& g, char* buf, size_t cap);
int describe_row_launch(const RowpassFusedPlan& g, char* buf, size_t cap);
int describe_row_launch(const UPhaseBigPlan& g, char* buf, size_t cap);
int describe_row_launch(const UPhaseGramPlan& g, char* buf, size_t cap);
int describe_row_launch(const UStepDirectPlan& g, char* buf, size_t cap);

hipError_t launch_u_phase_gram(const ProblemView& p, const IterateView& it, int n_iter2, hipStream_t st);
bool u_phase_gram_supported(int S, int n_c, int n_u);
bool u_phase_mfma_supported(int S, int n_c, int n_u);
hipError_t launch_u_phase_mfma(const ProblemView& p, const IterateView& it, int n_iter2, hipStream_t st);
hipError_t launch_u_phase_mfma_impl(const ProblemView& p, const IterateView& it, int n_iter2, double* cm_out, hipStream_t st);
bool rowpass_fused_supported(int S, int n_c, int n_u);
int rowpass_fused_grid(int64_t N, int S);
int64_t rowpass_fused_slab_doubles(int64_t N, int S, int n_c, int n_u);
hipError_t launch_rowpass_fused(const ProblemView& p, const IterateView& it, int n_iter2, const UScratch& scratch,
                                int* grid_out, hipStream_t st);
hipError_t launch_finish_u_norm(const double* u2_partials, int n, SolverState* state, hipStream_t st);
hipError_t launch_u_step_direct(const ProblemView& p, const IterateView& it, double* u_next, int t, hipStream_t st);
bool u_step_direct_supported(int S, int n_c, int n_u);

hipError_t launch_alpha(AlphaKind kind, const AlphaView& a, int n_iter2, hipStream_t st);
hipError_t launch_set_lh(SolverState* state, hipStream_t st);
hipError_t launch_project_simplex(const double* X, double* out, int K, int S, double z,
                                  hipStream_t st);
hipError_t launch_scatter_known_block(const double* gb_known, double* gb, int n_c, int K, int S,
                                      hipStream_t st);
hipError_t launch_init_state(SolverState* state, const double* consts, const double* alpha,
                             int S, int n_c, int n_u, hipStream_t st);

int64_t u_phase_split_cm_doubles(int64_t N, int n_u);
hipError_t launch_u_phase_split(const ProblemView& p, const IterateView& it, int n_iter2, const UScratch& scratch,
                                hipStream_t st);

bool cm_i8_supported(unsigned v_align, int S, int n_c, int n_u, int ND, int SD);
struct CmI8Launch {
    int mt0 = 0, mt1 = 0;
    int c_tile = 0, c_store = 0;
    size_t lds = 0;
    int grid = 0;
    int64_t blocks_per_wave = 0;
};
struct CmI8Panel {
    int col0 = 0, Sp = 0;
    bool s4 = false;
    int ncgx = 2;
    int tpl = 0;
    int n_launch = 0;
    CmI8Launch first, last;
};
constexpr int kCmMaxPanels = 8;
struct CmI8Plan {
    bool supported = false;
    int64_t N = 0;
    int S = 0, n_c = 0, n_u = 0;
    int nkc = 0, nd = 1;
    int nmt = 0, n_ct = 0;
    int n_panels = 0;
    CmI8Panel panel[kCmMaxPanels];
};
CmI8Plan cm_i8_plan(int64_t N, int S, int n_c, int n_u, int ND);
CmI8Launch cm_i8_launch_of(const CmI8Plan& g, int panel, int li);
int describe_cm_i8_plan(const CmI8Plan& g, char* buf, size_t cap);
struct CmRan {
    char text[2048] = "";
};
hipError_t launch_cm_i8(const ProblemView& p, const IterateView& it, double* cm, hipStream_t st, CmRan* ran = nullptr);
hipError_t launch_u_phase_split_i8(const ProblemView& p, const IterateView& it, int n_iter2, const UScratch& scratch,
                                   hipStream_t st);

bool u_inner_bu_supported(unsigned v_align, int S, int SD, int n_u, int n_iter2);
int u_inner_bu_grid(int64_t N, int S);
hipError_t launch_u_phase_split_i8_bu(const ProblemView& p, const IterateView& it, int n_iter2, const UScratch& scratch,
                                      int* grid_out, hipStream_t st);

bool u_phase_big_supported(int S, int n_c, int n_u, int n_iter2);
hipError_t launch_u_phase_big(const ProblemView& p, const IterateView& it, int n_iter2, hipStream_t st);

hipError_t launch_gram_mfma(const ProblemView& p, const double* u, int n_u, GramJobTable jobs, int n_dense, double* slab,
                            int64_t slab_doubles, const int* done_flag, int* ny_out, hipStream_t st, GramRan* ran = nullptr);
int64_t gram_mfma_slab_doubles(int64_t N, int S, int n_jobs);

hipError_t launch_gather_counts_int(const unsigned short* src16, const unsigned short* src_x16, const long long* idx,
                                    int64_t n_idx, int SD, int ND, unsigned short* D16, unsigned short* X16, int64_t N16,
                                    signed char* Dt8, int64_t plane_stride, unsigned int* max_out,
                                    unsigned long long* xsum_out, hipStream_t st);
constexpr double kX16MaxDev = 8.0 * 0x1p-53;
hipError_t launch_build_counts_int(const double* D, const double* V, int64_t N, int S, int ND, unsigned short* D16,
                                   unsigned short* X16, int64_t N16, int SD, signed char* Dt8, int64_t plane_stride,
                                   unsigned long long* x_stats, hipStream_t st);
hipError_t launch_build_dt8(const unsigned short* D16, int64_t N, int SD, int ND, signed char* Dt8, int64_t plane_stride,
                            hipStream_t st);
hipError_t launch_mask_problem(const double* srcV, const double* srcD, const unsigned short* src16,
                               const unsigned short* srcX, const unsigned char* bits, double* dstV, double* dstD,
                               unsigned short* dst16, unsigned short* dstX, unsigned short* W16, int64_t N, int64_t N16, int S,
                               int SD, unsigned long long* stats, hipStream_t st);
hipError_t launch_holdout_weights_f64(const unsigned char* bits, double* W, int64_t N, int S, hipStream_t st);
constexpr int64_t kMaskDrawMaxS = ((int64_t)1 << 31) - 1, kMaskDrawMaxElements = (int64_t)1 << 60;
hipError_t launch_mask_draw(unsigned int* key_io, int pos, int64_t N, int64_t S, unsigned long long threshold,
                            unsigned char* bits, unsigned long long* result, hipStream_t st);
bool rowpass_v2_supported(int S, int n_c, int n_u, int n_iter2);
int rowpass_v2_grid(int64_t N, int S);
hipError_t launch_rowpass_v2(const ProblemView& p, const IterateView& it, int n_iter2, const UScratch& scratch, int* grid_out,
                             bool pair, bool* paired_out, hipStream_t st);
bool rowpass_v2_pair_fits(int S, int n_u, int n_iter2);
bool gram_i8_supported(int n_c, int n_u, int ND, int64_t N, int SD);
struct GramI8Plan {
    bool supported = false;
    int xl = 1, nd = 1, ring = 8;
    int nf = 0, launches = 0;
    int nsh = 0, ny = 0;
    int64_t rows_per_wg = 0;
    int blocks = 0, last = 0;
    int tail = 0;
    bool xcd = false;
};
GramI8Plan gram_i8_plan(int64_t N, int SD, int n_c, int n_u, int ND);
void describe_gram_i8_plan(const GramI8Plan& g, char* buf, size_t cap);
int64_t gram_i8_slab_words(int64_t N, int SD, int n_c, int n_u);
int64_t gram_i8_acc_words(int S, int n_c, int n_u);
bool gram_i8_known_supported(int n_c, int ND, int64_t N, int SD);
int64_t gram_i8_slab_words_nf(int64_t N, int SD, int nf);
int64_t gram_i8_acc_words_nf(int S, int nf, int n_bu);
hipError_t launch_gram_i8(const ProblemView& p, const double* u, int n_u, const short* feat_a, const short* feat_b, int NF,
                          long long* slab, int64_t slab_words, const int* done_flag, int* ny_out, hipStream_t st,
                          GramRan* ran = nullptr);
int bu_cols_grid(int64_t N);
hipError_t launch_bu_cols(const ProblemView& p, const double* u, int n_u, double* slab, const int* done_flag,
                          int* n_slabs_out, hipStream_t st, bool* with_vdv = nullptr);
hipError_t launch_gram_v2_reduce(const long long* slab_i8, int ny, int NF, int SD, const double* slab_bu, int n_bu_slabs,
                                 int n_u, int S, long long* acc_words, const int* dst_row, double* gb, const int* done_flag,
                                 const double* u2_partials, int n_u2, SolverState* state, hipStream_t st);

hipError_t launch_percentile_pair(const double* x, int64_t n, int64_t m, PercentilePlan p0, PercentilePlan p1,
                                  double* out0, double* out1, hipStream_t st);
hipError_t launch_nanpercentile_pair(const double* x, int64_t n, int64_t m, PercentilePlan p0, PercentilePlan p1, double q0,
                                     double q1, double* out0, double* out1, hipStream_t st);
int64_t percentile_max_replicates();

int wls_moments_grid(int64_t N);
int64_t wls_slab_doubles(int64_t N, int S, int K);
hipError_t launch_wls_moments(const ProblemView& p, const double* u, int n_u, int target_dv, double* slab, double* mom,
                              hipStream_t st);
hipError_t launch_nnls_intercept(const double* gb, const double* mom, int K, int S, double* out, int* status, hipStream_t st);

constexpr int kSvdMaxS = 512, kSvdMaxNc = 64, kSvdMaxRank = 64;
constexpr size_t kSvdMaxLds = 160 * 1024;
size_t svd_project_lds_bytes(int S, int rank);
struct SvdColumns {
    double sign[kSvdMaxRank], scale[kSvdMaxRank];
};
bool svd_supported(int S, int n_c, int rank);
int svd_gram_grid(int64_t N, int S);
int64_t svd_gram_slab_doubles(int64_t N, int S);
hipError_t launch_svd_gram(const ProblemView& p, const double* H1, double* slab, int* flags, double* C, hipStream_t st);
int64_t svd_project_slab_doubles(int64_t N, int rank);
hipError_t launch_svd_project(const ProblemView& p, const double* H1, const double* Es, int rank, double* T, double* slab,
                              double* norms, hipStream_t st);
hipError_t launch_svd_finish(double* T, int64_t N, int rank, const SvdColumns& cols, hipStream_t st);

struct MatchColumns {
    int src[kMaxK];
};
int match_gram_grid(int64_t N, int n_u);
int64_t match_gram_slab_doubles(int64_t N, int n_u);
hipError_t launch_match_gram(const double* u, const double* anchor, const long long* idx, int64_t N, int64_t n_anchor_rows,
                             int n_u, double* slab, int* flags, double* P, hipStream_t st);
hipError_t launch_copy_cols_permuted(const double* u, double* dst, int64_t N, int n_u, const MatchColumns& cols,
                                     hipStream_t st);
constexpr long long kNotDrawn = 0x7fffffffffffffffLL;
hipError_t launch_first_occurrence(const long long* idx, int64_t M, int64_t n_dst_rows, long long* first,
                                   unsigned long long* n_bad, hipStream_t st);
hipError_t launch_copy_rows_first(const double* u, const long long* first, double* dst, int64_t n_dst_rows, int n_u,
                                  const MatchColumns& cols, hipStream_t st);

}
```

demethify_amd/csrc/dmf_kernels_rowpass2.hip:

```cpp
#include "dmf_device.h"
#include "dmf_dispatch.h"
#include "dmf_internal.h"
#include "dmf_ustep.h"
#include "dmf_fixedpoint.h"
#include <cstdlib>
#include <type_traits>

namespace dmf {

typedef double v4d __attribute__((ext_vector_type(4)));
typedef double v2d __attribute__((ext_vector_type(2)));
typedef unsigned int v4u __attribute__((ext_vector_type(4)));
typedef unsigned int v2u __attribute__((ext_vector_type(2)));
typedef int v4i __attribute__((ext_vector_type(4)));

#ifdef DMF_STAMPS
#define DMF2_STAMP_DECL unsigned long long st_last = dmf2_stamp(), st_seg[16] = {0, 0, 0, 0, 0, 0, 0, 0, 0, 0, 0, 0, 0, 0, 0, 0};
#define DMF2_STAMP(i) { const unsigned long long st_now = dmf2_stamp(); st_seg[i] += st_now - st_last; st_last = st_now; }
#define DMF2_STAMP_FLUSH                                                                                        \
    st_seg[15] = __builtin_amdgcn_s_getreg(4 | (31 << 11));                                                     \
    if (lane == 0) for (int i_ = 0; i_ < 16; ++i_) stamps_out[((size_t)blockIdx.x * 4 + wave) * 16 + i_] = st_seg[i_];
__device__ __forceinline__ unsigned long long dmf2_stamp() {
    unsigned long long t;
    __builtin_amdgcn_sched_barrier(0);
    asm volatile("s_memtime %0\n\ts_waitcnt lgkmcnt(0)" : "=s"(t)::"memory");
    __builtin_amdgcn_sched_barrier(0);
    return t;
}
#define DMF2_SUB_BEGIN unsigned long long st_sub = dmf2_stamp();
#define DMF2_SUB(i) { const unsigned long long st_now = dmf2_stamp(); st_seg[i] += st_now - st_sub; st_sub = st_now; }
#else
#define DMF2_STAMP_DECL
#define DMF2_STAMP(i)
#define DMF2_STAMP_FLUSH
#define DMF2_SUB_BEGIN
#define DMF2_SUB(i)
#endif

#ifndef DMF_V2_STAGGER
#define DMF_V2_STAGGER 12
#endif

namespace {
constexpr int kRowV = 66;
constexpr int kRowD = 72;
constexpr int kTileVBytes2 = 16 * kRowV * 8;
constexpr int kTileDBytes2 = 16 * kRowD * 2;
constexpr int kTileBytes2 = kTileVBytes2 + kTileDBytes2;
constexpr int kTileBytesX = 2 * kTileDBytes2;
}

template <int NU, bool AT_PREV>
__device__ __forceinline__ void inner_steps(double& uu, double& up, double cj, const double (&Ms)[NU], int b_lo, int b_hi,
                                            int t_end, int lane0) {
    int t2 = 0;
    for (; t2 + 1 < t_end; t2 += 2) {
        inner_step<NU, AT_PREV>(uu, up, cj, Ms, b_lo, b_hi, t2, lane0);
        inner_step<NU, AT_PREV>(up, uu, cj, Ms, b_lo, b_hi, t2 + 1, lane0);
    }
    if (t2 < t_end) {
        inner_step<NU, AT_PREV>(uu, up, cj, Ms, b_lo, b_hi, t2, lane0);
        const double tmp = uu;
        uu = up;
        up = tmp;
    }
}

constexpr int kUnrolledSteps = 20;

template <int NU, bool AT_PREV>
__device__ __forceinline__ void inner_steps_unrolled(double& uu, double& up, double cj, const double (&Ms)[NU], int b_lo, int b_hi,
                                                     int lane0) {
    static_assert(kUnrolledSteps % 2 == 0 && kUnrolledSteps <= 64, "pairs of steps; beta_t in lane t of one register pair");
#pragma unroll
    for (int t2 = 0; t2 < kUnrolledSteps; t2 += 2) {
        inner_step<NU, AT_PREV>(uu, up, cj, Ms, b_lo, b_hi, t2, lane0);
        inner_step<NU, AT_PREV>(up, uu, cj, Ms, b_lo, b_hi, t2 + 1, lane0);
    }
}

template <int NKC, int NU, int MAXW = 4, bool XS = false, bool PAIR = false>
__global__ __launch_bounds__(64 * MAXW, MAXW == 4 ? 2 : 1) void k_rowpass_v2(
    const double* __restrict__ V, const unsigned short* __restrict__ D16, const unsigned short* __restrict__ X16, int SD,
    const double* __restrict__ Rtp,
    const double* __restrict__ alpha, double* __restrict__ u, double* __restrict__ u_prev,
    const SolverState* __restrict__ state, int64_t N, int S, int n_c, int n_iter2, int mode, int nd,
    double* __restrict__ slab, double* __restrict__ u2_partials
#ifdef DMF_STAMPS
    , unsigned long long* __restrict__ stamps_out
#endif
    ) {
    static_assert(NU >= 1 && NU <= 4, "one phase-B pass per block, 4x4x4 MFMA for the c product");
    static_assert(!PAIR || (XS && MAXW == 4), "the pair schedule: X16 form, two workgroups per CU");
    constexpr int NSET = PAIR ? 2 : 1;
    constexpr int NCT = 4 * NKC;
    constexpr int NP = NU * (NU + 1) / 2;
    constexpr int SLOT = (NU + 2) & ~1;
    constexpr int NV = NU * SLOT;
    extern __shared__ double lds_dyn[];
    if (state->done) return;

    const int NW = blockDim.x >> 6;
    const int wave = __builtin_amdgcn_readfirstlane(threadIdx.x >> 6);
    const int lane = threadIdx.x & 63;
    const int wcol0 = wave * 64;

    double* __restrict__ beta_tab = lds_dyn;
    double* __restrict__ ubuf = beta_tab + ((n_iter2 + 1) & ~1);
    double* __restrict__ red = ubuf + NSET * 16 * NU;
    double* __restrict__ u2red = red + NSET * MAXW * NV * 16;
    constexpr int TB = XS ? kTileBytesX : kTileBytes2;
    char* __restrict__ tile = reinterpret_cast<char*>(u2red + MAXW) + (size_t)wave * TB;
    struct BlockTile {
        double* V;
        unsigned short *D, *X;
    };
    auto block_tile = [&](int set) {
        char* const t = tile + (size_t)set * NW * TB;
        unsigned short* const d = reinterpret_cast<unsigned short*>(t + (XS ? 0 : kTileVBytes2));
        return BlockTile{reinterpret_cast<double*>(t), d, d + 16 * kRowD};
    };

    if (const double* __restrict__ mrow = momentum_row(state, n_iter2)) {
        const double lw_prev = state->l_w_prev, lw = state->l_w;
        for (int t2 = threadIdx.x; t2 < n_iter2; t2 += blockDim.x)
            beta_tab[t2] = fmin(mrow[2 + t2], t2 == 0 ? 0.9999 * sqrt(lw_prev / lw) : 0.9999);
    } else if (threadIdx.x == 0) {
        fill_momentum_table(state, n_iter2, beta_tab);
    }
    for (int i = threadIdx.x; i < NSET * MAXW * NV * 16; i += blockDim.x) red[i] = 0.0;
    const double inv_lw = 1.0 / state->l_w;
    const double m_scale_v = -inv_lw * 0x1p-52;
    const double m_scale = __hiloint2double(__builtin_amdgcn_readfirstlane(__double2hiint(m_scale_v)),
                                            __builtin_amdgcn_readfirstlane(__double2loint(m_scale_v)));

    const int m16 = lane & 15, q = lane >> 4;
    const int sw_row = (m16 >= 4 && m16 < 12) ? 1 : 0;
    const int qs = q ^ sw_row;
    const int c_row = 8 * (q & 1) + 4 * (q >> 1);
    const int mC = m16 ^ ((q == 1 || q == 2) ? 4 : 0);
    const int e_col = wcol0 + 4 * (m16 & 3) + (m16 >> 2);
    const int k_col = wcol0 + 4 * q;
    double a1r[4][NKC > 0 ? NKC : 1];
    double a2r[4][4];
    v4i pdg[7];
    int pj = 0, pl = 0;
    while ((pl + 1) * (pl + 2) / 2 <= m16) ++pl;
    pj = m16 - pl * (pl + 1) / 2;
    {
        const bool pair_ok = m16 < NP;
        const bool a2_ok = (m16 & 3) < NU;
#pragma unroll
        for (int t = 0; t < 4; ++t) {
#pragma unroll
            for (int kc = 0; kc < NKC; ++kc) {
                const int row = kc * 4 + q, col = e_col + 16 * t;
                a1r[t][kc] = (row < n_c && col < S) ? -alpha[(int64_t)row * S + col] : 0.0;
            }
#pragma unroll
            for (int r = 0; r < 4; ++r) {
                const int col = k_col + 16 * t + r;
                a2r[t][r] = (col < S && a2_ok) ? alpha[(int64_t)(n_c + (m16 & 3)) * S + col] * inv_lw : 0.0;
            }
        }
#pragma unroll
        for (int g = 0; g < 4; ++g) {
            unsigned int lo[4], hi[4], tl[4], th[4];
#pragma unroll
            for (int i = 0; i < 4; ++i) {
                const int col = wcol0 + 16 * q + 4 * g + i;
                const bool in = pair_ok && col < S;
                const double aj = in ? alpha[(int64_t)(n_c + pj) * S + col] : 0.0;
                const double al = in ? alpha[(int64_t)(n_c + pl) * S + col] : 0.0;
                z_to_biased(aj, al, lo[i], hi[i]);
            }
            transpose4(lo, tl);
            transpose4(hi, th);
            pdg[0][g] = (int)(tl[0] ^ 0x80808080u);
            pdg[1][g] = (int)(tl[1] ^ 0x80808080u);
            pdg[2][g] = (int)(tl[2] ^ 0x80808080u);
            pdg[3][g] = (int)(tl[3] ^ 0x80808080u);
            pdg[4][g] = (int)(th[0] ^ 0x80808080u);
            pdg[5][g] = (int)(th[1] ^ 0x80808080u);
            pdg[6][g] = (int)th[2];
        }
    }
    __syncthreads();

    double bu[4] = {0.0, 0.0, 0.0, 0.0};
    double u2_acc = 0.0;
    DMF2_STAMP_DECL
    const int64_t nblk = (N + 15) / 16;
    const int nk = (int)((nblk - blockIdx.x + gridDim.x - 1) / gridDim.x);

    const int ld_row = lane >> 5;
    const int ld_col = (lane & 31) * 2;
    int ld_gcol = wcol0 + ld_col;
    const int last_pair = (S - 1) & ~1;
    if (ld_gcol > last_pair) ld_gcol = last_pair;
    const int d_row = lane >> 3, d_col = (lane & 7) * 8;
    const int ld_col_sw = ((lane & 31) ^ 2) * 2;
    v2d pv[NSET][XS ? 1 : 8];
    v4u pd[NSET][2], px[NSET][XS ? 2 : 1];
    double nrt[NSET][NKC > 0 ? NKC : 1];
    double pu, pup;
    constexpr int RPWB = 64 / NU;
    const int rl = lane / NU, jb = lane - rl * NU;
    const bool b_lane = rl < 16 && rl < RPWB;
    const unsigned int v_off = (unsigned int)(ld_row * S + ld_gcol) * 8u;
    const unsigned int d_off = (unsigned int)(d_row * SD + wcol0 + d_col) * 2u;
    const unsigned int r_off = (unsigned int)(m16 * NCT + q) * 8u;
    const unsigned int u_off = b_lane ? (unsigned int)lane * 8u : 0xFFFFFFF0u;
    auto span = [](int64_t bytes) { return (unsigned int)(bytes < 0 ? 0 : (bytes > 0x7FFFFFFF ? 0x7FFFFFFF : bytes)); };
    auto prefetch_u = [&](int64_t blk) {
        const int64_t r0 = blk * 16;
        const int64_t left = N - r0;
        const __amdgpu_buffer_rsrc_t ru = __builtin_amdgcn_make_buffer_rsrc((void*)(u + r0 * NU), 0, span(left * NU * 8), 0x00020000);
        const __amdgpu_buffer_rsrc_t rp = __builtin_amdgcn_make_buffer_rsrc((void*)(u_prev + r0 * NU), 0, span(left * NU * 8), 0x00020000);
        const v2u a = __builtin_amdgcn_raw_buffer_load_b64(ru, u_off, 0, 0);
        const v2u b = __builtin_amdgcn_raw_buffer_load_b64(rp, u_off, 0, 0);
        pu = __hiloint2double((int)a.y, (int)a.x);
        pup = __hiloint2double((int)b.y, (int)b.x);
    };
    auto prefetch_tile = [&](int64_t blk, int set) {
        const int64_t r0 = blk * 16;
        const int64_t left = N - r0;
        if (NKC > 0) {
            const __amdgpu_buffer_rsrc_t rr = __builtin_amdgcn_make_buffer_rsrc((void*)(Rtp + r0 * NCT), 0, span(left * NCT * 8), 0x00020000);
#pragma unroll
            for (int kc = 0; kc < NKC; ++kc) {
                const v2u a = __builtin_amdgcn_raw_buffer_load_b64(rr, r_off, kc * 32, 0);
                nrt[set][kc] = __hiloint2double((int)a.y, (int)a.x);
            }
        }
        if constexpr (!XS) {
            const __amdgpu_buffer_rsrc_t rv = __builtin_amdgcn_make_buffer_rsrc((void*)(V + r0 * S), 0, span(left * S * 8), 0x00020000);
#pragma unroll
            for (int i = 0; i < 8; ++i) {
                const v4u a = __builtin_amdgcn_raw_buffer_load_b128(rv, v_off, 2 * i * S * 8, 0);
                pv[set][i] = v2d{__hiloint2double((int)a.y, (int)a.x), __hiloint2double((int)a.w, (int)a.z)};
            }
        } else {
            const __amdgpu_buffer_rsrc_t rx = __builtin_amdgcn_make_buffer_rsrc((void*)(X16 + r0 * SD), 0, span((int64_t)16 * SD * 2), 0x00020000);
            px[set][0] = __builtin_amdgcn_raw_buffer_load_b128(rx, d_off, 0, 0);
            px[set][1] = __builtin_amdgcn_raw_buffer_load_b128(rx, d_off, 8 * SD * 2, 0);
        }
        {
            const __amdgpu_buffer_rsrc_t rd = __builtin_amdgcn_make_buffer_rsrc((void*)(D16 + r0 * SD), 0, span((int64_t)16 * SD * 2), 0x00020000);
            pd[set][0] = __builtin_amdgcn_raw_buffer_load_b128(rd, d_off, 0, 0);
            pd[set][1] = __builtin_amdgcn_raw_buffer_load_b128(rd, d_off, 8 * SD * 2, 0);
        }
    };
    auto pair_set = [&](int s) { return (PAIR && s + 1 < nk && wave == (s + 1) % NW) ? 1 : 0; };
    if (nk > 0) {
        prefetch_u(blockIdx.x + (int64_t)pair_set(0) * gridDim.x);
        prefetch_tile(blockIdx.x, 0);
        if (PAIR && nk > 1) prefetch_tile(blockIdx.x + gridDim.x, 1);
    }

    double* __restrict__ const mine_c = red + (size_t)wave * NV * 16 + (m16 * NU + q) * SLOT;
    double* __restrict__ const mine_m1 = red + (size_t)wave * NV * 16 + (4 * q * NU + pl) * SLOT + 1 + (pj - pl + NU) % NU;
    double* __restrict__ const mine_m2 = red + (size_t)wave * NV * 16 + (4 * q * NU + pj) * SLOT + 1 + (pl - pj) % NU;

    auto tile_store = [&](int set) {
        const BlockTile T = block_tile(set);
        if constexpr (XS) {
#pragma unroll
            for (int i = 0; i < 2; ++i) *reinterpret_cast<v4u*>(T.X + (8 * i + d_row) * kRowD + d_col) = px[set][i];
        } else {
#pragma unroll
            for (int i = 0; i < 8; ++i)
                *reinterpret_cast<v2d*>(T.V + (2 * i + ld_row) * kRowV + ((i >= 2 && i < 6) ? ld_col_sw : ld_col)) = pv[set][i];
        }
#ifndef DMF_ABLATE_DSTORE
#pragma unroll
        for (int i = 0; i < 2; ++i) *reinterpret_cast<v4u*>(T.D + (8 * i + d_row) * kRowD + d_col) = pd[set][i];
#endif
    };

    auto phase_a = [&](int set, int st_a, int st_p) {
        const BlockTile T = block_tile(set);
        const double* __restrict__ const tileV = T.V;
        unsigned short* __restrict__ const tileD = T.D;
        unsigned short* __restrict__ const tileX = T.X;
        const double (&rtop)[NKC > 0 ? NKC : 1] = nrt[set];
        struct StripV {
            v2d v01, v23;
            v2u dw;
        };
        struct StripX {
            v2u dw, xw;
        };
        using Strip = std::conditional_t<XS, StripX, StripV>;
        auto load_strip = [&](int t, Strip& R) {
            if constexpr (XS) {
                R.xw = *reinterpret_cast<const v2u*>(tileX + m16 * kRowD + t * 16 + 4 * q);
            } else {
                const double* __restrict__ tv = tileV + m16 * kRowV + t * 16 + 4 * qs;
                R.v01 = *reinterpret_cast<const v2d*>(tv);
                R.v23 = *reinterpret_cast<const v2d*>(tv + 2);
            }
            R.dw = *reinterpret_cast<const v2u*>(tileD + m16 * kRowD + t * 16 + 4 * q);
        };
        double csm0 = 0.0, csm1 = 0.0;
        auto e_init = [&](const Strip& R) {
            if constexpr (XS) return v4d{0.0, 0.0, 0.0, 0.0};
            else return v4d{R.v01.x, R.v01.y, R.v23.x, R.v23.y};
        };
        auto run_strip = [&](const Strip& R, v4d e, const Strip& Rn, const double (&a1n)[NKC > 0 ? NKC : 1],
                             const double (&a2)[4], bool has_next) {
            const v4d d = {(double)(R.dw.x & 0xFFFFu), (double)(R.dw.x >> 16), (double)(R.dw.y & 0xFFFFu), (double)(R.dw.y >> 16)};
            v4d w;
            if constexpr (XS) {
                const v4d x = {(double)(R.xw.x & 0xFFFFu), (double)(R.xw.x >> 16), (double)(R.xw.y & 0xFFFFu), (double)(R.xw.y >> 16)};
#pragma unroll
                for (int r = 0; r < 4; ++r) w[r] = fma(d[r], e[r], x[r]);
            } else {
                w = d * e;
            }
            v4d en = e_init(Rn);
#pragma unroll
            for (int r = 0; r < 4; ++r) {
                if (r & 1) csm1 = __builtin_amdgcn_mfma_f64_4x4x4f64(a2[r], w[r], csm1, 0, 0, 0);
                else csm0 = __builtin_amdgcn_mfma_f64_4x4x4f64(a2[r], w[r], csm0, 0, 0, 0);
                if (has_next && r < NKC) en = __builtin_amdgcn_mfma_f64_16x16x4f64(a1n[r], rtop[r], en, 0, 0, 0);
            }
            return en;
        };
#ifdef DMF_ABLATE_E
        const double csm = XS ? (double)tileX[m16 * kRowD + 4 * q] : tileV[m16 * kRowV + 4 * qs];
#else
        Strip sa, sb;
        load_strip(0, sa);
        load_strip(1, sb);
        __builtin_amdgcn_sched_barrier(0);
        v4d e0 = e_init(sa);
#pragma unroll
        for (int kc = 0; kc < NKC; ++kc) e0 = __builtin_amdgcn_mfma_f64_16x16x4f64(a1r[0][kc], rtop[kc], e0, 0, 0, 0);
        const v4d e1 = run_strip(sa, e0, sb, a1r[1], a2r[0], true);
        load_strip(2, sa);
        __builtin_amdgcn_sched_barrier(0);
        const v4d e2 = run_strip(sb, e1, sa, a1r[2], a2r[1], true);
        load_strip(3, sb);
        __builtin_amdgcn_sched_barrier(0);
        const v4d e3 = run_strip(sa, e2, sb, a1r[3], a2r[2], true);
        (void)run_strip(sb, e3, sb, a1r[3], a2r[3], false);
        const double csm = csm0 + csm1;
#endif
        v4i mw[8];
#pragma unroll
        for (int w8 = 0; w8 < 8; ++w8) mw[w8] = v4i{0, 0, 0, 0};
#ifndef DMF_ABLATE_M
        {
            const v4u wa = *reinterpret_cast<const v4u*>(tileD + m16 * kRowD + 16 * q);
            const v4u wb = *reinterpret_cast<const v4u*>(tileD + m16 * kRowD + 16 * q + 8);
            const unsigned int e0 = wa.x + 0x00800080u, e1 = wa.y + 0x00800080u, e2 = wa.z + 0x00800080u, e3 = wa.w + 0x00800080u;
            const unsigned int e4 = wb.x + 0x00800080u, e5 = wb.y + 0x00800080u, e6 = wb.z + 0x00800080u, e7 = wb.w + 0x00800080u;
            const v4i c0 = {(int)(__builtin_amdgcn_perm(e1, e0, 0x06040200u) ^ 0x80808080u),
                            (int)(__builtin_amdgcn_perm(e3, e2, 0x06040200u) ^ 0x80808080u),
                            (int)(__builtin_amdgcn_perm(e5, e4, 0x06040200u) ^ 0x80808080u),
                            (int)(__builtin_amdgcn_perm(e7, e6, 0x06040200u) ^ 0x80808080u)};
#pragma unroll
            for (int t = 0; t < 7; ++t) mw[t] = __builtin_amdgcn_mfma_i32_16x16x64_i8(c0, pdg[t], mw[t], 0, 0, 0);
            if (nd == 2) {
                const v4i c1 = {(int)__builtin_amdgcn_perm(e1, e0, 0x07050301u), (int)__builtin_amdgcn_perm(e3, e2, 0x07050301u),
                                (int)__builtin_amdgcn_perm(e5, e4, 0x07050301u), (int)__builtin_amdgcn_perm(e7, e6, 0x07050301u)};
#pragma unroll
                for (int t = 0; t < 7; ++t) mw[t + 1] = __builtin_amdgcn_mfma_i32_16x16x64_i8(c1, pdg[t], mw[t + 1], 0, 0, 0);
            }
        }
#endif
        double mrow[4];
#ifdef DMF_ABLATE_M
#pragma unroll
        for (int rr = 0; rr < 4; ++rr) mrow[rr] = 0.25 * (rr == (m16 & 3));
#else
#pragma unroll
        for (int rr = 0; rr < 4; ++rr) {
#ifndef DMF_CHAIN_NO_I32
            const double lo = fma((double)(mw[3][rr] * 256 + mw[2][rr]), 65536.0, (double)(mw[1][rr] * 256 + mw[0][rr]));
            const double hi = fma((double)(mw[7][rr] * 256 + mw[6][rr]), 65536.0, (double)(mw[5][rr] * 256 + mw[4][rr]));
#else
            const double lo = fma(fma(fma((double)mw[3][rr], 256.0, (double)mw[2][rr]), 256.0, (double)mw[1][rr]), 256.0, (double)mw[0][rr]);
            const double hi = fma(fma(fma((double)mw[7][rr], 256.0, (double)mw[6][rr]), 256.0, (double)mw[5][rr]), 256.0, (double)mw[4][rr]);
#endif
            mrow[rr] = fma(hi, 0x1p32, lo) * m_scale;
        }
#endif
        DMF2_STAMP(st_a)
        {
            const size_t so = (size_t)set * MAXW * NV * 16;
            if (q < NU) mine_c[so] = csm;
            if (m16 < NP) {
#pragma unroll
                for (int rr = 0; rr < 4; ++rr) mine_m1[so + rr * NU * SLOT] = mrow[rr];
                if (pj != pl) {
#pragma unroll
                    for (int rr = 0; rr < 4; ++rr) mine_m2[so + rr * NU * SLOT] = mrow[rr];
                }
            }
        }
        DMF2_STAMP(st_p)
    };

    auto phase_b = [&](int set, int64_t row0, double uu0, double up0) {
        __builtin_amdgcn_s_setprio(3);
        DMF2_SUB_BEGIN
        const bool ok = b_lane && row0 + rl < N;
        const int lane0 = lane - jb;
        const int rlc = rl < 16 ? rl : 15;
        double cj = 0.0, Ms[NU];
#pragma unroll
        for (int l = 0; l < NU; ++l) Ms[l] = 0.0;
        {
            const double* __restrict__ slot = red + (size_t)set * MAXW * NV * 16 + (rlc * NU + jb) * SLOT;
#pragma unroll 1
            for (int w0 = 0; w0 < MAXW; w0 += 4) {
                v2d part[4][SLOT / 2];
#pragma unroll
                for (int w = 0; w < 4; ++w)
#pragma unroll
                    for (int h = 0; h < SLOT / 2; ++h)
                        part[w][h] = *reinterpret_cast<const v2d*>(slot + (w0 + w) * NV * 16 + 2 * h);
#pragma unroll
                for (int w = 0; w < 4; ++w) {
                    cj += part[w][0].x;
#pragma unroll
                    for (int l = 0; l < NU; ++l) Ms[l] += (l & 1) ? part[w][(l + 1) / 2].x : part[w][l / 2].y;
                }
            }
        }
        double uu = uu0, up = up0;
        DMF2_SUB(8)
#ifndef DMF_CHAIN_NO_UNROLL
        if (XS && MAXW == 4 && n_iter2 == kUnrolledSteps) {
            const double bvec = beta_tab[lane < kUnrolledSteps ? lane : kUnrolledSteps - 1];
            const int b_lo = __double2loint(bvec), b_hi = __double2hiint(bvec);
            if (mode == 1) {
                inner_steps_unrolled<NU, true>(uu, up, cj, Ms, b_lo, b_hi, lane0);
            } else {
                Ms[0] += 1.0;
                inner_steps_unrolled<NU, false>(uu, up, cj, Ms, b_lo, b_hi, lane0);
            }
        } else
#endif
        for (int t0 = 0; t0 < n_iter2; t0 += 64) {
            const int tl = t0 + lane < n_iter2 ? t0 + lane : n_iter2 - 1;
            const double bvec = beta_tab[tl];
            const int b_lo = __double2loint(bvec), b_hi = __double2hiint(bvec);
            const int t_end = n_iter2 - t0 < 64 ? n_iter2 - t0 : 64;
            if (mode == 1) {
                inner_steps<NU, true>(uu, up, cj, Ms, b_lo, b_hi, t_end, lane0);
            } else {
                if (t0 == 0) Ms[0] += 1.0;
                inner_steps<NU, false>(uu, up, cj, Ms, b_lo, b_hi, t_end, lane0);
            }
        }
        DMF2_SUB(9)
        if (b_lane) ubuf[set * 16 * NU + rl * NU + jb] = ok ? uu : 0.0;
        if (ok) {
            const __amdgpu_buffer_rsrc_t ru = __builtin_amdgcn_make_buffer_rsrc((void*)(u + row0 * NU), 0, span((N - row0) * NU * 8), 0x00020000);
            const __amdgpu_buffer_rsrc_t rp = __builtin_amdgcn_make_buffer_rsrc((void*)(u_prev + row0 * NU), 0, span((N - row0) * NU * 8), 0x00020000);
            __builtin_amdgcn_raw_buffer_store_b64(v2u{(unsigned int)__double2loint(uu), (unsigned int)__double2hiint(uu)}, ru, u_off, 0, 0);
            __builtin_amdgcn_raw_buffer_store_b64(v2u{(unsigned int)__double2loint(up), (unsigned int)__double2hiint(up)}, rp, u_off, 0, 0);
            u2_acc = fma(uu, uu, u2_acc);
        }
        DMF2_SUB(10)
        __builtin_amdgcn_s_setprio(0);
    };

    auto phase_c = [&](int set) {
#ifndef DMF_ABLATE_C
        const BlockTile T = block_tile(set);
        const double* __restrict__ const ub = ubuf + set * 16 * NU;
#pragma unroll
        for (int half = 0; half < 2; ++half) {
            double vv[2][4], ua[2];
            unsigned short dd[2][4];
#pragma unroll
            for (int rr = 0; rr < 2; ++rr) {
                const int row = 2 * half + rr + c_row;
#pragma unroll
                for (int t = 0; t < 4; ++t) {
                    if constexpr (XS) {
                        dd[rr][t] = T.X[row * kRowD + 16 * t + m16];
                    } else {
                        vv[rr][t] = T.V[row * kRowV + 16 * t + mC];
                        dd[rr][t] = T.D[row * kRowD + 16 * t + m16];
                    }
                }
                ua[rr] = (m16 & 3) < NU ? ub[row * NU + (m16 & 3)] : 0.0;
            }
#pragma unroll
            for (int rr = 0; rr < 2; ++rr)
#pragma unroll
                for (int t = 0; t < 4; ++t)
                    bu[t] = __builtin_amdgcn_mfma_f64_4x4x4f64(ua[rr], XS ? (double)dd[rr][t] : (double)dd[rr][t] * vv[rr][t], bu[t], 0, 0, 0);
        }
#endif
    };

    for (int s = 0; s < nk; s += NSET) {
        const bool has2 = PAIR && s + 1 < nk;
        const int64_t blk = blockIdx.x + (int64_t)s * gridDim.x;
        __builtin_amdgcn_s_setprio(1);
        tile_store(0);
        if (has2) tile_store(1);
        const int bset = pair_set(s);
        const bool my_turn = bset == 1 || wave == s % NW;
        const double uu0 = pu;
        const double up0 = pup;
        __builtin_amdgcn_wave_barrier();
        __builtin_amdgcn_s_setprio(0);
        DMF2_STAMP(0)
        phase_a(0, 1, 2);
        if (has2) phase_a(1, 11, 12);
        asm volatile("s_waitcnt lgkmcnt(0)" ::: "memory");
        __builtin_amdgcn_s_barrier();
        DMF2_STAMP(3)
#ifndef DMF_V2_NO_STAGGER
        if (!my_turn) __builtin_amdgcn_s_sleep(DMF_V2_STAGGER);
#endif
        if (s + NSET < nk) {
            const int64_t nb = blk + NSET * (int64_t)gridDim.x;
            prefetch_u(nb + (int64_t)pair_set(s + NSET) * gridDim.x);
            prefetch_tile(nb, 0);
            if (PAIR && s + 3 < nk) prefetch_tile(nb + gridDim.x, 1);
        }
        DMF2_STAMP(7)
        if (my_turn) phase_b(bset, (blk + (int64_t)bset * gridDim.x) * 16, uu0, up0);
        DMF2_STAMP(4)
        asm volatile("s_waitcnt lgkmcnt(0)" ::: "memory");
        __builtin_amdgcn_s_barrier();
        DMF2_STAMP(5)
        phase_c(0);
        DMF2_STAMP(6)
        if (has2) phase_c(1);
        __builtin_amdgcn_s_setprio(0);
        DMF2_STAMP(13)
    }

    DMF2_STAMP_FLUSH
    const double w2 = wave_sum(u2_acc);
    if (lane == 0) u2red[wave] = w2;
    __syncthreads();
    if (q < NU) {
#pragma unroll
        for (int t = 0; t < 4; ++t) {
            const int sC = wcol0 + 16 * t + m16;
            if (sC < S) slab[((int64_t)blockIdx.x * NU + q) * S + sC] = bu[t];
        }
    }
    if (threadIdx.x == 0) {
        double tot = 0.0;
        for (int w = 0; w < NW; ++w) tot += u2red[w];
        u2_partials[blockIdx.x] = tot;
    }
}

size_t rowpass_v2_lds_bytes(int S, int n_u, int n_iter2, bool x16, bool pair = false) {
    const int NW = (S + 63) / 64;
    const int maxw = NW <= 4 ? 4 : 8;
    const int nset = pair ? 2 : 1;
    const int nv = n_u * ((n_u + 2) & ~1);
    const size_t doubles = (size_t)((n_iter2 + 1) & ~1) + (size_t)nset * (16 * n_u + maxw * nv * 16) + maxw;
    return doubles * sizeof(double) + (size_t)nset * NW * (x16 ? kTileBytesX : kTileBytes2);
}

bool rowpass_v2_supported(int S, int n_c, int n_u, int n_iter2) {
    if (S < 2 || S > 512 || n_c > 16 || n_u < 1 || n_u > 4) return false;
    return rowpass_v2_lds_bytes(S, n_u, n_iter2, false) <= (size_t)(S <= 256 ? 80 : 160) * 1024;
}

static int rowpass_v2_per_cu(int NW) {
    return per_cu_knob("DMF_V2_PER_CU", NW > 4 ? 1 : 8 / NW);
}

bool rowpass_v2_pair_fits(int S, int n_u, int n_iter2) {
    const int NW = (S + 63) / 64;
    if (NW < 2 || NW > 4) return false;
    return rowpass_v2_lds_bytes(S, n_u, n_iter2, true, true) * (size_t)rowpass_v2_per_cu(NW) <= (size_t)160 * 1024;
}

int rowpass_v2_grid(int64_t N, int S) {
    const int per_cu = rowpass_v2_per_cu((S + 63) / 64);
    const int64_t nblk = (N + 15) / 16;
    const int64_t g = 256 * per_cu;
    return (int)(nblk < g ? nblk : g);
}

hipError_t launch_rowpass_v2(const ProblemView& p, const IterateView& it, int n_iter2, const UScratch& scratch, int* grid_out,
                             bool pair, bool* paired_out, hipStream_t st) {
    const int S = p.S, NW = (S + 63) / 64;
    pair = pair && p.X16 != nullptr && rowpass_v2_pair_fits(S, it.n_u, n_iter2);
    if (paired_out != nullptr) *paired_out = pair;
    return dispatch_int<0, 4>((p.n_c + 3) / 4, [&](auto nkc) {
        return dispatch_bool(p.X16 != nullptr, [&](auto xs) {
            return dispatch_int<1, 4>(it.n_u, [&](auto nu) {
                const auto launch = [&](auto maxw, auto pair_t) {
                    constexpr int NU = decltype(nu)::value, MAXW = decltype(maxw)::value;
                    constexpr bool XS = decltype(xs)::value, PAIR = decltype(pair_t)::value;
                    constexpr auto kernel = k_rowpass_v2<decltype(nkc)::value, NU, MAXW, XS, PAIR>;
                    const size_t lds = rowpass_v2_lds_bytes(S, NU, n_iter2, XS, PAIR);
                    constexpr size_t kLdsCap = (size_t)(MAXW == 4 ? 80 : 160) * 1024;
                    if (NW > MAXW || (MAXW == 8 && NW <= 4) || (PAIR && NW < 2) || lds > kLdsCap || p.N < 1 ||
                        p.SD < NW * 64 || (p.SD & 7) != 0 || p.ND < 1 || p.ND > 2)
                        return hipErrorInvalidValue;
                    if (lds > 48 * 1024) {
                        const hipError_t e = raise_dynamic_lds<kernel>(kLdsCap);
                        if (e != hipSuccess) return e;
                    }
                    const int grid = rowpass_v2_grid(p.N, S);
                    *grid_out = grid;
                    hipLaunchKernelGGL(kernel, dim3(grid), dim3(NW * 64), lds, st, p.V, p.D16, p.X16, p.SD, p.Rtp, it.alpha,
                                       it.u, it.u_prev, it.state, p.N, S, p.n_c, n_iter2, it.mode, p.ND, scratch.slab,
                                       scratch.u2_partials
#ifdef DMF_STAMPS
                                       , (unsigned long long*)nullptr
#endif
                                       );
                    return hipGetLastError();
                };
                if (S > 256) return launch(std::integral_constant<int, 8>{}, std::false_type{});
                if constexpr (decltype(xs)::value) {
                    if (pair) return launch(std::integral_constant<int, 4>{}, std::true_type{});
                }
                return launch(std::integral_constant<int, 4>{}, std::false_type{});
            });
        });
    });
}

}
```

demethify_amd/csrc/dmf_select.h:

```cpp
#pragma once
#include <cstddef>
#include <cstdint>

namespace dmf {

constexpr int kSplitInnerSteps = 50;
constexpr int kCmI8MinNu = 5;
constexpr int kSplitMinNu = 7;
constexpr int kGramI8MinFp64Acc = 48;
constexpr int kGramI8MinPairsNoKnown = 33;

struct ShapeKey {
    int64_t N = 0;
    int S = 0, n_c = 0, n_u = 0;
    int nd = 0;
    int SD = 0;
    bool x16 = false;
    bool rowpass_pair = true;
    int level = 0;
    bool d_f32_exact = false;
    bool rtp_present = true;
    unsigned v_align = 0;
    unsigned rtp_align = 0;
    bool alpha_unit = true;
};

struct PathSpec {
    int u_path = 2;
    bool use_gram_spec = false, use_gram_mfma = false, use_u_big = false;
    bool use_v2 = false, use_cm_i8 = false, use_gram_i8 = false, use_fused = false;
    bool supported = true;
};

enum class RowKind {
    RowpassV2,
    CmI8InnerBu,
    CmI8InnerRows,
    RowpassFused,
    UPhaseBig,
    UPhaseMfmaSplit,
    UPhaseMfma,
    UPhaseGram,
    UStepDirect
};
enum class GramKind { InRowPass, I8, BuColsI8, GramU, GramMfma, Gram };
enum class AlphaKind { FrankWolfeRow16, FrankWolfe, PhaseRow16, PhaseLanes, Phase, PhaseDyn };

struct IterationPlan {
    RowKind row = RowKind::UStepDirect;
    GramKind gram = GramKind::Gram;
    AlphaKind alpha = AlphaKind::PhaseDyn;
};

PathSpec select_path(const ShapeKey& k);
IterationPlan plan_iteration(const ShapeKey& k, const PathSpec& s, int n_iter2, bool purity);
int describe_plan(const ShapeKey& k, const IterationPlan& plan, char* buf, size_t cap);
PathSpec standalone_spec(PathSpec s);
int describe_u_phase(const ShapeKey& k, const PathSpec& s, int n_iter2, bool purity, bool standalone, char* buf, size_t cap);

struct CostKey {
    int S = 0, n_c = 0, n_u = 0;
    bool d16 = false;
    int SD = 0;
    unsigned v_align = 0;
    bool rtp_present = true;
    int level = 0;
};
enum class CostKind {
    Cols,
    Cols2,
    Cols2Wide,
    Generic
};
struct CostPlan {
    CostKind kind = CostKind::Generic;
    int nkc = 0, nu = 0;
    bool d16 = false;
    bool odd = false;
    bool alpha_in_lds = false;
};
constexpr int kCostPartials = 1024;
CostPlan cost_plan(const CostKey& k);
int describe_cost_plan(const CostPlan& plan, char* buf, size_t cap);

}
```

demethify_amd/device.py:

```python
from __future__ import annotations

import ctypes as C
import os

import numpy as np

from . import _lib as L

_contexts: dict[int, "Context"] = {}


def _is_torch(x) -> bool:
    return type(x).__module__.startswith("torch")


def _host_f64(x, name):
    a = np.ascontiguousarray(x, dtype=np.float64)
    if not np.all(np.isfinite(a)):
        raise ValueError(f"{name} holds non-finite values (use --fillna)")
    return a


def _ptr(a):
    if a is None:
        return None
    if _is_torch(a) or hasattr(a, "data_ptr"):
        return C.c_void_p(a.data_ptr())
    return a.ctypes.data_as(C.c_void_p)


def pack_mask(mask) -> np.ndarray:
    m = np.asarray(mask)
    if m.ndim != 2:
        raise ValueError(f"a mask is N x S, got shape {m.shape}")
    return np.packbits(m.astype(bool, copy=False), axis=1, bitorder="little")


def mask_threshold(fraction) -> int:
    import math

    f = float(fraction)
    if not f > 0.0:
        return 0
    if f >= 1.0:
        return 1 << 53
    return math.ceil(f * 9007199254740992.0)


class Context:

    def __init__(self, device: int = 0, stream: int | None = None):
        self._lib = L.load()
        h = C.c_void_p()
        L.check(self._lib.dmf_context_create(int(device), C.c_void_p(stream) if stream else None, C.byref(h)),
                "dmf_context_create")
        self._h = h
        self.device = int(device)
        self.generic_level = 0

    def close(self):
        if getattr(self, "_h", None):
            self._lib.dmf_context_destroy(self._h)
            self._h = None

    def __del__(self):
        try:
            self.close()
        except Exception:
            pass

    def synchronize(self):
        L.check(self._lib.dmf_context_synchronize(self._h), "dmf_context_synchronize")

    def set_profiling(self, enabled, families=None):
        mode = int(bool(enabled))
        if mode and families is not None:
            mode = sum(1 << (1 + int(f)) for f in families)
        L.check(self._lib.dmf_context_set_profiling(self._h, mode), "dmf_context_set_profiling")

    def set_generic(self, level: int):
        L.check(self._lib.dmf_context_set_generic(self._h, int(level)), "dmf_context_set_generic")
        self.generic_level = int(level)

    def set_x16(self, enabled: bool):
        L.check(self._lib.dmf_context_set_x16(self._h, int(bool(enabled))), "dmf_context_set_x16")

    def set_rowpass_pair(self, enabled: bool):
        L.check(self._lib.dmf_context_set_rowpass_pair(self._h, int(bool(enabled))), "dmf_context_set_rowpass_pair")

    def set_stop_confirmation(self, mode: int):
        L.check(self._lib.dmf_context_set_stop_confirmation(self._h, int(mode)), "dmf_context_set_stop_confirmation")

    def reset_kernel_time(self):
        L.check(self._lib.dmf_context_reset_kernel_time(self._h), "dmf_context_reset_kernel_time")

    def kernel_time(self, family: int):
        ms, n = C.c_double(), C.c_int64()
        L.check(self._lib.dmf_context_kernel_time(self._h, int(family), C.byref(ms), C.byref(n)),
                "dmf_context_kernel_time")
        return ms.value, n.value

    def project_simplex(self, X, z=1.0):
        X = np.ascontiguousarray(X, dtype=np.float64)
        out = np.empty_like(X)
        K, S = X.shape
        L.check(self._lib.dmf_project_simplex(self._h, _ptr(X), K, S, float(z), 0, _ptr(out)),
                "dmf_project_simplex")
        return out

    def nnls_normal(self, G, mom):
        mom = np.ascontiguousarray(mom, dtype=np.float64)
        if mom.ndim != 2 or mom.shape[0] < 4 or mom.shape[0] % 2:
            raise ValueError(f"mom is (2 K + 2) x S, got shape {mom.shape}")
        K, S = mom.shape[0] // 2 - 1, mom.shape[1]
        G = np.asarray(G, dtype=np.float64)
        if G.shape == (S, K, K):
            if not np.array_equal(G, G.transpose(0, 2, 1)):
                raise ValueError("G must be symmetric")
            i, j = np.triu_indices(K)
            gb = np.empty((K * (K + 1) // 2, S), dtype=np.float64)
            gb[j * (j + 1) // 2 + i] = G[:, i, j].T
        elif G.shape == (K * (K + 1) // 2, S):
            gb = np.ascontiguousarray(G)
        else:
            raise ValueError(f"G shape {G.shape} is neither {(S, K, K)} nor {(K * (K + 1) // 2, S)}")
        out = np.full((K, S), np.nan, dtype=np.float64)
        status = np.full(S, -1, dtype=np.intc)
        L.check(self._lib.dmf_nnls_normal(self._h, _ptr(gb), _ptr(mom), K, S, _ptr(out),
                                          status.ctypes.data_as(C.POINTER(C.c_int))), "dmf_nnls_normal")
        return out, status

    def percentile_axis0(self, x, q):
        return self._percentile_axis0(x, q, "dmf_percentile_axis0")

    def nanpercentile_axis0(self, x, q):
        return self._percentile_axis0(x, q, "dmf_nanpercentile_axis0")

    def _percentile_axis0(self, x, q, entry):
        fn = getattr(self._lib, entry)
        qs = np.ascontiguousarray(np.atleast_1d(q), dtype=np.float64)
        if _is_torch(x) and x.is_cuda:
            import torch

            if x.dtype != torch.float64:
                raise TypeError(f"{entry[4:]} takes float64 data")
            x = x.contiguous()
            n, tail = x.shape[0], tuple(x.shape[1:])
            m = int(np.prod(tail, dtype=np.int64))
            out = torch.empty((len(qs),) + tail, dtype=torch.float64, device=x.device)
            torch.cuda.current_stream(x.device).synchronize()
            L.check(fn(self._h, _ptr(x), n, m, _ptr(qs), len(qs), L.DMF_PTR_DEVICE, _ptr(out)), entry)
            return out
        if _is_torch(x):
            x = x.numpy()
        x = np.ascontiguousarray(x, dtype=np.float64)
        n, tail = x.shape[0], tuple(x.shape[1:])
        m = int(np.prod(tail, dtype=np.int64))
        out = np.empty((len(qs),) + tail, dtype=np.float64)
        L.check(fn(self._h, _ptr(x), n, m, _ptr(qs), len(qs), 0, _ptr(out)), entry)
        return out


def get_context(device: int | None = None) -> Context:
    if device is None:
        device = int(os.environ.get("DEMETHIFY_DEVICE", os.environ.get("LOCAL_RANK", "0")))
    ctx = _contexts.get(device)
    if ctx is None:
        ctx = _contexts[device] = Context(device)
    return ctx


def _route(route) -> int:
    try:
        return {"solver": L.DMF_ROUTE_SOLVER, "update_u": L.DMF_ROUTE_UPDATE_U}[route]
    except KeyError:
        raise ValueError(f'route must be "solver" or "update_u", got {route!r}') from None


def u_phase_describe(N, S, n_c, n_u, nd=0, level=0, n_iter2=20, flags=0, route="solver"):
    buf = C.create_string_buffer(2048)
    st = L.load().dmf_u_phase_describe(int(N), int(S), int(n_c), int(n_u), int(nd), int(level), int(n_iter2), int(flags),
                                       _route(route), buf, len(buf))
    if st == L.DMF_ERR_UNSUPPORTED:
        return None
    L.check(st, "dmf_u_phase_describe")
    return buf.value.decode()


def small_solve_supported(N, S, n_c, n_u, mode=L.DMF_MODE_PARTIAL) -> bool:
    return bool(L.load().dmf_solve_small_supported(int(N), int(S), int(n_c), int(n_u), int(mode)))


class Problem:

    def __init__(self, ctx: Context, V, counts, Rt=None):
        self.ctx = ctx
        self._lib = ctx._lib
        flags = 0
        if _is_torch(V):
            import torch

            flags |= L.DMF_PTR_DEVICE
            for t in (V, counts) + ((Rt,) if Rt is not None else ()):
                if not (t.is_cuda and t.is_contiguous() and t.device.index == ctx.device):
                    raise ValueError("device tensors must be contiguous and on the context's GPU")
            if V.dtype != torch.float64 or (Rt is not None and Rt.dtype != torch.float64):
                raise ValueError("V and R_trunc must be float64")
            if counts.dtype == torch.float64:
                flags |= L.DMF_COUNTS_F64
            elif counts.dtype != torch.int64:
                raise ValueError("counts must be int64 or float64")
            torch.cuda.current_stream(V.device).synchronize()
            N, S = V.shape
        else:
            V = _host_f64(V, "meth_frequency")
            counts = np.asarray(counts)
            if counts.dtype.kind in "iub":
                counts = np.ascontiguousarray(counts, dtype=np.int64)
            else:
                counts = _host_f64(counts, "counts")
                flags |= L.DMF_COUNTS_F64
            if Rt is not None:
                Rt = _host_f64(Rt, "R_trunc")
            N, S = V.shape
        if tuple(counts.shape) != (N, S):
            raise ValueError(f"counts shape {tuple(counts.shape)} != meth_frequency shape {(N, S)}")
        n_c = 0
        if Rt is not None:
            if Rt.ndim != 2 or Rt.shape[0] != N:
                raise ValueError(f"R_trunc shape {tuple(Rt.shape)} does not match {N} CpG rows")
            n_c = int(Rt.shape[1])
        self._keep = (V, counts, Rt)
        self.N, self.S, self.n_c = int(N), int(S), n_c
        h = C.c_void_p()
        L.check(self._lib.dmf_problem_create(ctx._h, self.N, self.S, self.n_c, _ptr(V), _ptr(counts),
                                             _ptr(Rt) if n_c else None, flags, C.byref(h)),
                "dmf_problem_create")
        self._h = h

    @classmethod
    def _from_handle(cls, ctx, h, N, S, n_c):
        self = cls.__new__(cls)
        self.ctx, self._lib, self._h = ctx, ctx._lib, h
        self.N, self.S, self.n_c = N, S, n_c
        self._keep = ()
        return self

    def gather(self, idx) -> "Problem":
        h = C.c_void_p()
        if getattr(idx, "is_cuda", False):
            n = int(np.prod(idx.shape))
            L.check(self._lib.dmf_problem_gather_device(self.ctx._h, self._h, C.c_void_p(idx.data_ptr()), n, C.byref(h)),
                    "dmf_problem_gather_device")
            return Problem._from_handle(self.ctx, h, n, self.S, self.n_c)
        idx = np.ascontiguousarray(idx, dtype=np.int64)
        L.check(self._lib.dmf_problem_gather(self.ctx._h, self._h, _ptr(idx), idx.size, C.byref(h)),
                "dmf_problem_gather")
        return Problem._from_handle(self.ctx, h, int(idx.size), self.S, self.n_c)

    def masked(self, train_mask) -> "Problem":
        nb = (self.S + 7) // 8
        flags = 0
        if getattr(train_mask, "is_cuda", False):
            if _is_torch(train_mask):
                import torch

                ok = (train_mask.dtype == torch.uint8 and train_mask.is_contiguous()
                      and tuple(train_mask.shape) == (self.N, nb) and train_mask.device.index == self.ctx.device)
                if ok:
                    torch.cuda.current_stream(train_mask.device).synchronize()
            else:
                ok = getattr(train_mask, "packed_mask", None) == (self.N, nb) and train_mask.ctx is self.ctx
            if not ok:
                raise ValueError(f"a device mask must be the packed bits: contiguous uint8, shape {(self.N, nb)}, on the "
                                 "context's GPU")
            bits, flags = train_mask, L.DMF_PTR_DEVICE
        else:
            m = np.asarray(train_mask)
            if m.dtype == np.bool_:
                if m.shape != (self.N, self.S):
                    raise ValueError(f"mask shape {m.shape} != problem shape {(self.N, self.S)}")
                bits = pack_mask(m)
            elif m.dtype == np.uint8:
                if m.shape != (self.N, nb):
                    raise ValueError(f"packed mask shape {m.shape} != {(self.N, nb)} (ceil(S / 8) bytes per row)")
                bits = np.ascontiguousarray(m)
            else:
                raise TypeError("train_mask must be a bool N x S array or packed uint8 bits")
        h = C.c_void_p()
        L.check(self._lib.dmf_problem_mask(self.ctx._h, self._h, _ptr(bits), flags, C.byref(h)), "dmf_problem_mask")
        out = Problem._from_handle(self.ctx, h, self.N, self.S, self.n_c)
        out._keep = (self,)
        return out

    def close(self):
        if getattr(self, "_h", None):
            if getattr(self.ctx, "_h", None):
                self._lib.dmf_problem_destroy(self._h)
            self._h = None
            self._keep = ()

    def __del__(self):
        try:
            self.close()
        except Exception:
            pass

    def __enter__(self):
        return self

    def __exit__(self, *exc):
        self.close()

    def cost(self, u, alpha) -> float:
        alpha = np.ascontiguousarray(alpha, dtype=np.float64)
        n_u = 0
        if u is not None:
            u = np.ascontiguousarray(u, dtype=np.float64).reshape(self.N, -1)
            n_u = u.shape[1]
        if alpha.shape != (self.n_c + n_u, self.S):
            raise ValueError(f"alpha shape {alpha.shape} != {(self.n_c + n_u, self.S)}")
        out = C.c_double()
        L.check(self._lib.dmf_cost(self.ctx._h, self._h, _ptr(u) if n_u else None, n_u, _ptr(alpha), 0,
                                   C.byref(out)), "dmf_cost")
        return out.value

    def cost_describe(self, n_u: int) -> str:
        buf = C.create_string_buffer(128)
        L.check(self._lib.dmf_problem_cost_describe(self.ctx._h, self._h, int(n_u), buf, len(buf)),
                "dmf_problem_cost_describe")
        return buf.value.decode()

    def gram_known(self):
        out = np.empty(((self.n_c + 1) * (self.n_c + 2) // 2, self.S), dtype=np.float64)
        buf = C.create_string_buffer(256)
        L.check(self._lib.dmf_problem_gram_known(self._h, _ptr(out), buf, len(buf)), "dmf_problem_gram_known")
        return out, buf.value.decode()

    def report(self) -> dict:
        ints = (C.c_int64 * len(L.REPORT_INTS))()
        dbls = (C.c_double * len(L.REPORT_DBLS))()
        L.check(self._lib.dmf_problem_report(self._h, ints, dbls), "dmf_problem_report")
        out = {k: int(v) for k, v in zip(L.REPORT_INTS, ints)}
        out.update({k: float(v) for k, v in zip(L.REPORT_DBLS, dbls)})
        return out

    def copy_out(self, name: str, report: dict | None = None) -> np.ndarray:
        r = self.report() if report is None else report
        shape, dtype = {
            "V": ((r["N"], r["S"]), np.float64), "D": ((r["N"], r["S"]), np.float64),
            "Rt": ((r["N"], r["n_c"]), np.float64), "Rtp": ((r["N"], r["rtp_width"]), np.float64),
            "D16": ((r["N16"], r["SD"]), np.uint16), "X16": ((r["N16"], r["SD"]), np.uint16),
            "W16": ((r["N16"], r["SD"]), np.uint16),
            "Dt8": ((r["ND"], (r["N"] + 31) // 32, r["SD"] // 32, 32, 32), np.int8),
            "mask_bits": ((r["N"], (r["S"] + 7) // 8), np.uint8), "consts": ((6,), np.float64),
        }[name]
        out = np.empty(shape, dtype=dtype)
        L.check(self._lib.dmf_problem_copy_out(self._h, L.PROBLEM_ARRAYS[name], _ptr(out), out.nbytes),
                "dmf_problem_copy_out")
        return out

    def wls_intercept(self, u=None, target="v", host_arrays=None, f64_arrays=False):
        tg, u, n_u, flags = self._wls_args(u, target, f64_arrays)
        K = self.n_c + n_u
        out = np.zeros((K, self.S), dtype=np.float64)
        status = np.full(self.S, -1, dtype=np.intc)
        L.check(self._lib.dmf_wls_intercept(self.ctx._h, self._h, _ptr(u) if n_u else None, n_u, tg, flags, _ptr(out),
                                            status.ctypes.data_as(C.POINTER(C.c_int))), "dmf_wls_intercept")
        self.wls_status = status
        if (status == 2).any():
            raise ZeroDivisionError("Weights sum to zero, can't be normalized")
        redo = np.flatnonzero(status != 0)
        if redo.size:
            if host_arrays is None:
                raise RuntimeError(f"wls_intercept: the device did not solve samples {redo.tolist()} (rank-deficient "
                                   "profiles or iteration cap) and no host_arrays were given to solve them on the host")
            from .init_func import wls_intercept as host_wls

            meth_f, counts, R_full = host_arrays() if callable(host_arrays) else host_arrays
            for k in redo:
                x = counts[:, k:k + 1] * meth_f[:, k:k + 1] if target == "dv" else meth_f[:, k:k + 1]
                out[:, k:k + 1] = host_wls(x, counts[:, k:k + 1], R_full)
        return out

    def wls_moments(self, u=None, target="v", f64_arrays=False):
        tg, u, n_u, flags = self._wls_args(u, target, f64_arrays)
        out = np.empty((2 * (self.n_c + n_u) + 2, self.S), dtype=np.float64)
        L.check(self._lib.dmf_wls_moments(self.ctx._h, self._h, _ptr(u) if n_u else None, n_u, tg, flags, _ptr(out)),
                "dmf_wls_moments")
        return out

    def _wls_args(self, u, target, f64_arrays):
        try:
            tg = {"v": L.DMF_WLS_TARGET_V, "dv": L.DMF_WLS_TARGET_DV}[target]
        except KeyError:
            raise ValueError(f'target must be "v" or "dv", got {target!r}') from None
        flags, n_u = 0, 0
        if u is not None:
            if getattr(u, "is_cuda", False):
                from .staging import DeviceArray

                if isinstance(u, DeviceArray):
                    ok = u.ctx is self.ctx
                else:
                    ok = (_is_torch(u) and u.is_contiguous() and u.element_size() == 8 and u.is_floating_point()
                          and u.device.index == self.ctx.device)
                    if ok:
                        import torch

                        torch.cuda.current_stream(u.device).synchronize()
                if not ok:
                    raise ValueError("a device u must be a float64 staging.DeviceArray / contiguous CUDA tensor on the "
                                     "context's GPU")
                u = u.reshape(self.N, -1)
                flags = L.DMF_PTR_DEVICE
            else:
                u = _host_f64(u, "u").reshape(self.N, -1)
            n_u = int(u.shape[1])
        if f64_arrays:
            flags |= L.DMF_WLS_F64_ARRAYS
        return tg, u, n_u, flags

    def svd_gram(self, H1=None):
        if self.n_c:
            H1 = _host_f64(H1, "H1")
            if H1.shape != (self.n_c, self.S):
                raise ValueError(f"H1 shape {H1.shape} != {(self.n_c, self.S)}")
        else:
            H1 = None
        out = np.empty((self.S, self.S), dtype=np.float64)
        counts = (C.c_int64 * 2)()
        L.check(self._lib.dmf_svd_gram(self.ctx._h, self._h, _ptr(H1), 0, _ptr(out), counts), "dmf_svd_gram")
        return out, int(counts[0]), int(counts[1])

    def nndsvd(self, rank, keep_on_device=False, host_arrays=None):
        from .init_func import constrained_nndsvd, nndsvd_from_eig, nndsvd_initialize

        rank = int(rank)
        if rank < 1:
            raise ValueError(f"rank must be at least 1, got {rank}")

        def host_route():
            if host_arrays is None:
                raise RuntimeError("nndsvd: the device route does not take this problem and no host_arrays were given")
            meth_f, counts, R_trunc = host_arrays() if callable(host_arrays) else host_arrays
            if self.n_c:
                W, H = constrained_nndsvd(meth_f, R_trunc, counts, rank)
                u0 = W[:, self.n_c:]
            else:
                W, H = nndsvd_initialize(meth_f, rank)
                u0 = np.clip(W, 0, 1)
            u0 = np.ascontiguousarray(u0)
            if keep_on_device:
                from .staging import to_device

                u0, = to_device((u0,), self.ctx)
            return u0, H

        if rank > self.S:
            raise ValueError(f"rank {rank} exceeds the {self.S} samples")
        H1 = self.wls_intercept(None, "v", host_arrays=host_arrays, f64_arrays=True) if self.n_c else None
        try:
            gram, negatives, _ = self.svd_gram(H1)
        except L.DemethifyHipError as e:
            if e.status != L.DMF_ERR_UNSUPPORTED:
                raise
            return host_route()
        if not self.n_c and negatives:
            raise ValueError("The input matrix contains negative elements.")
        lam, vec = np.linalg.eigh(gram)
        lam, vec = lam[::-1][:rank], np.ascontiguousarray(vec[:, ::-1][:, :rank])
        if not lam[-1] > 1e-10 * lam[0]:
            return host_route()
        sigma = np.sqrt(lam)
        try:
            u_dev, norms = self.svd_factor(H1, vec / sigma)
        except L.DemethifyHipError as e:
            if e.status != L.DMF_ERR_UNSUPPORTED:
                raise
            return host_route()
        sign, scale, H2 = nndsvd_from_eig(sigma, vec, norms)
        u0 = self.svd_finish(u_dev, sign, scale, keep_on_device)
        return u0, (np.vstack([H1, H2]) if self.n_c else H2)

    def svd_factor(self, H1, e_over_sigma):
        from .staging import DeviceArray

        H1 = _host_f64(H1, "H1") if self.n_c else None
        e_over_sigma = _host_f64(e_over_sigma, "e_over_sigma")
        if e_over_sigma.ndim != 2 or e_over_sigma.shape[0] != self.S:
            raise ValueError(f"e_over_sigma shape {e_over_sigma.shape} does not match {self.S} samples")
        rank = int(e_over_sigma.shape[1])
        norms = np.empty((2, rank), dtype=np.float64)
        t = C.c_void_p()
        L.check(self._lib.dmf_svd_factor(self.ctx._h, self._h, _ptr(H1), _ptr(e_over_sigma), rank, 0, _ptr(norms),
                                         C.byref(t)), "dmf_svd_factor")
        return DeviceArray(self.ctx, t.value, (self.N, rank)), norms

    def svd_finish(self, t_dev, sign, scale, keep_on_device=False):
        n, rank = t_dev.shape
        sign = np.ascontiguousarray(sign, dtype=np.float64)
        scale = np.ascontiguousarray(scale, dtype=np.float64)
        if sign.shape != (rank,) or scale.shape != (rank,):
            raise ValueError(f"sign and scale need {rank} values each")
        if keep_on_device:
            L.check(self._lib.dmf_svd_finish(self.ctx._h, _ptr(t_dev), n, rank, _ptr(sign), _ptr(scale), L.DMF_PTR_DEVICE,
                                             None), "dmf_svd_finish")
            return t_dev
        u0 = np.empty((n, rank), dtype=np.float64)
        try:
            L.check(self._lib.dmf_svd_finish(self.ctx._h, _ptr(t_dev), n, rank, _ptr(sign), _ptr(scale), 0, _ptr(u0)),
                    "dmf_svd_finish")
        finally:
            t_dev.close()
        return u0

    def solve_many(self, u0s, alpha0s, mode, n_iter1, n_iter2, tol, idx=None, iters_per_launch=0, purity=None):
        u0s = np.ascontiguousarray(u0s, dtype=np.float64)
        alpha0s = np.ascontiguousarray(alpha0s, dtype=np.float64)
        if u0s.ndim != 3 or u0s.shape[1] != self.N:
            raise ValueError(f"u0s is B x {self.N} x n_u, got shape {u0s.shape}")
        B, _, n_u = u0s.shape
        K = self.n_c + n_u
        if alpha0s.shape != (B, K, self.S):
            raise ValueError(f"alpha0s shape {alpha0s.shape} != {(B, K, self.S)}")
        if idx is not None:
            idx = np.ascontiguousarray(idx, dtype=np.int64)
            if idx.shape != (B, self.N):
                raise ValueError(f"idx shape {idx.shape} != {(B, self.N)}")
        if purity is not None:
            purity = np.ascontiguousarray(purity, dtype=np.float64)
            if purity.shape != (self.S,):
                raise ValueError(f"purity needs one value per sample ({self.S}), got shape {purity.shape}")
            if int(mode) != L.DMF_MODE_PARTIAL:
                raise ValueError("a purity constraint needs the partial-reference mode (DMF_MODE_PARTIAL)")
            if self.n_c < 1:
                raise ValueError("a purity constraint needs a reference: there is no known block to hold at that mass")
        u = np.empty((B, self.N, n_u), dtype=np.float64)
        alpha = np.empty((B, K, self.S), dtype=np.float64)
        cost = np.empty(B, dtype=np.float64)
        iters = np.empty(B, dtype=np.int64)
        if purity is not None:
            L.check(self._lib.dmf_solve_small_purity(self.ctx._h, self._h, B, _ptr(idx), _ptr(u0s), _ptr(alpha0s), _ptr(purity),
                                                     n_u, int(mode), int(n_iter1), int(n_iter2), float(tol),
                                                     int(iters_per_launch), 0, _ptr(u), _ptr(alpha), _ptr(cost), _ptr(iters)),
                    "dmf_solve_small_purity")
            return u, alpha, cost, iters
        L.check(self._lib.dmf_solve_small(self.ctx._h, self._h, B, _ptr(idx), _ptr(u0s), _ptr(alpha0s), n_u, int(mode),
                                          int(n_iter1), int(n_iter2), float(tol), int(iters_per_launch), 0, _ptr(u),
                                          _ptr(alpha), _ptr(cost), _ptr(iters)), "dmf_solve_small")
        return u, alpha, cost, iters

    def update_u(self, u, u_prev, alpha, n_iter2, a1, l_w_prev, l_w, mode=L.DMF_MODE_PARTIAL):
        u = np.ascontiguousarray(u, dtype=np.float64).reshape(self.N, -1)
        u_prev = np.ascontiguousarray(u_prev, dtype=np.float64).reshape(u.shape)
        alpha = np.ascontiguousarray(alpha, dtype=np.float64)
        n_u = u.shape[1]
        if alpha.shape != (self.n_c + n_u, self.S):
            raise ValueError(f"alpha shape {alpha.shape} != {(self.n_c + n_u, self.S)}")
        sc = (C.c_double * 3)(float(a1), float(l_w_prev), float(l_w))
        out_u, out_up = np.empty_like(u), np.empty_like(u)
        L.check(self._lib.dmf_update_u(self.ctx._h, self._h, _ptr(u), _ptr(u_prev), _ptr(alpha), n_u,
                                       int(n_iter2), int(mode), 0, sc, _ptr(out_u), _ptr(out_up)),
                "dmf_update_u")
        return out_u, out_up, sc[0], sc[1]

    def update_alpha(self, u, alpha, alpha_prev, n_iter2, a2, l_h_prev, l_h):
        u = np.ascontiguousarray(u, dtype=np.float64).reshape(self.N, -1)
        alpha = np.ascontiguousarray(alpha, dtype=np.float64)
        alpha_prev = np.ascontiguousarray(alpha_prev, dtype=np.float64)
        n_u = u.shape[1]
        if alpha.shape != (self.n_c + n_u, self.S) or alpha_prev.shape != alpha.shape:
            raise ValueError(f"alpha shape {alpha.shape} != {(self.n_c + n_u, self.S)}")
        sc = (C.c_double * 3)(float(a2), float(l_h_prev), float(l_h))
        out_a, out_ap = np.empty_like(alpha), np.empty_like(alpha)
        L.check(self._lib.dmf_update_alpha(self.ctx._h, self._h, _ptr(u), n_u, _ptr(alpha), _ptr(alpha_prev),
                                           int(n_iter2), 0, sc, _ptr(out_a), _ptr(out_ap)),
                "dmf_update_alpha")
        return out_a, out_ap, sc[0], sc[1]


class Solver:

    def __init__(self, problem: Problem, u0, alpha0, mode=L.DMF_MODE_PARTIAL):
        self.problem = problem
        self._lib = problem._lib
        flags = 0
        if getattr(u0, "is_cuda", False) or getattr(alpha0, "is_cuda", False):
            from .staging import DeviceArray

            for t in (u0, alpha0):
                if isinstance(t, DeviceArray):
                    ok = t.ctx is problem.ctx
                else:
                    ok = (_is_torch(t) and t.is_cuda and t.is_contiguous() and t.element_size() == 8
                          and t.is_floating_point() and t.device.index == problem.ctx.device)
                if not ok:
                    raise ValueError("u0 and alpha0 must both be host arrays, or both be float64 device arrays "
                                     "(staging.DeviceArray / contiguous CUDA tensors) on the context's GPU")
            u0 = u0.reshape(problem.N, -1)
            flags = L.DMF_PTR_DEVICE
            if getattr(alpha0, "in_unit_range", None) is True:
                flags |= L.DMF_INIT_IN_UNIT_RANGE
        else:
            u0 = np.ascontiguousarray(u0, dtype=np.float64).reshape(problem.N, -1)
            alpha0 = np.ascontiguousarray(alpha0, dtype=np.float64)
        self.n_u = int(u0.shape[1])
        self.K = problem.n_c + self.n_u
        if tuple(alpha0.shape) != (self.K, problem.S):
            raise ValueError(f"alpha shape {tuple(alpha0.shape)} != {(self.K, problem.S)}")
        h = C.c_void_p()
        L.check(self._lib.dmf_solver_create(problem.ctx._h, problem._h, _ptr(u0), _ptr(alpha0), self.n_u,
                                            int(mode), flags, C.byref(h)), "dmf_solver_create")
        self._h = h

    def set_purity(self, purity):
        purity = np.ascontiguousarray(purity, dtype=np.float64).ravel()
        if purity.shape != (self.problem.S,):
            raise ValueError(f"purity needs one value per sample ({self.problem.S}), got {purity.shape}")
        L.check(self._lib.dmf_solver_set_purity(self._h, _ptr(purity), 0), "dmf_solver_set_purity")

    def step(self, n_outer: int, n_iter2: int, tol: float):
        it, conv = C.c_int64(), C.c_int()
        L.check(self._lib.dmf_solver_step(self._h, int(n_outer), int(n_iter2), float(tol), C.byref(it),
                                          C.byref(conv)), "dmf_solver_step")
        return it.value, bool(conv.value)

    def get(self):
        u = np.empty((self.problem.N, self.n_u), dtype=np.float64)
        alpha = np.empty((self.K, self.problem.S), dtype=np.float64)
        cost, it = C.c_double(), C.c_int64()
        L.check(self._lib.dmf_solver_get(self._h, 0, _ptr(u), _ptr(alpha), C.byref(cost), C.byref(it)),
                "dmf_solver_get")
        return u, alpha, cost.value, it.value

    def direct_cost(self) -> float:
        out = C.c_double()
        L.check(self._lib.dmf_solver_cost(self._h, C.byref(out)), "dmf_solver_cost")
        return out.value

    def holdout_error(self, full: Problem):
        ss, n = C.c_double(), C.c_int64()
        L.check(self._lib.dmf_solver_holdout_error(self._h, full._h, C.byref(ss), C.byref(n)), "dmf_solver_holdout_error")
        return ss.value, n.value

    def cost_begin(self):
        L.check(self._lib.dmf_solver_cost_begin(self._h), "dmf_solver_cost_begin")

    def cost_end(self) -> float:
        out = C.c_double()
        L.check(self._lib.dmf_solver_cost_end(self._h, C.byref(out)), "dmf_solver_cost_end")
        return out.value

    def describe(self, n_iter2: int = 20) -> str:
        buf = C.create_string_buffer(512)
        L.check(self._lib.dmf_solver_describe(self._h, int(n_iter2), buf, len(buf)), "dmf_solver_describe")
        return buf.value.decode()

    def u_phase_describe(self, n_iter2: int = 20, route="solver") -> str:
        buf = C.create_string_buffer(2048)
        L.check(self._lib.dmf_solver_u_phase_describe(self._h, int(n_iter2), _route(route), buf, len(buf)),
                "dmf_solver_u_phase_describe")
        return buf.value.decode()

    def gram(self, kind="integer"):
        try:
            k = {"integer": L.DMF_GRAM_INTEGER, "fp64": L.DMF_GRAM_FP64, "last": L.DMF_GRAM_LAST}[kind]
        except KeyError:
            raise ValueError(f'kind must be "integer", "fp64" or "last", got {kind!r}') from None
        out = np.empty(((self.K + 1) * (self.K + 2) // 2, self.problem.S), dtype=np.float64)
        buf = C.create_string_buffer(256)
        L.check(self._lib.dmf_solver_gram(self._h, k, _ptr(out), buf, len(buf)), "dmf_solver_gram")
        return out, buf.value.decode()

    def row_moments(self):
        n_u = self.n_u
        out = np.empty((self.problem.N, n_u + n_u * (n_u + 1) // 2), dtype=np.float64)
        buf = C.create_string_buffer(2048)
        L.check(self._lib.dmf_solver_row_moments(self._h, _ptr(out), buf, len(buf)), "dmf_solver_row_moments")
        return out, buf.value.decode()

    def momentum_state(self, arrays=True):
        sc = (C.c_double * len(L.MOMENTUM_SCALARS))()
        alpha_prev = np.empty((self.K, self.problem.S), dtype=np.float64) if arrays else None
        u_prev = np.empty((self.problem.N, self.n_u), dtype=np.float64) if arrays else None
        L.check(self._lib.dmf_solver_momentum_state(self._h, sc, _ptr(alpha_prev), _ptr(u_prev)),
                "dmf_solver_momentum_state")
        out = {name: (int(v) if i >= 11 else float(v)) for i, (name, v) in enumerate(zip(L.MOMENTUM_SCALARS, sc))}
        if arrays:
            out["alpha_prev"], out["u_prev"] = alpha_prev, u_prev
        return out

    def stop_info(self):
        on, nc, nu, cs = C.c_int(), C.c_int64(), C.c_int64(), C.c_double()
        L.check(self._lib.dmf_solver_stop_info(self._h, C.byref(on), C.byref(nc), C.byref(nu), C.byref(cs)),
                "dmf_solver_stop_info")
        return {"confirm_stops": bool(on.value), "n_confirmed": nc.value, "n_unconfirmed": nu.value,
                "last_stream_cost": cs.value}

    def rowpass_launches(self):
        total, paired = C.c_int64(), C.c_int64()
        L.check(self._lib.dmf_solver_rowpass_launches(self._h, C.byref(total), C.byref(paired)),
                "dmf_solver_rowpass_launches")
        return total.value, paired.value

    def get_alpha(self):
        alpha = np.empty((self.K, self.problem.S), dtype=np.float64)
        L.check(self._lib.dmf_solver_get(self._h, 0, None, _ptr(alpha), None, None), "dmf_solver_get")
        return alpha

    def _on_device(self, t, floating):
        from .staging import DeviceArray

        ctx = self.problem.ctx
        if isinstance(t, DeviceArray):
            return t.ctx is ctx
        ok = (_is_torch(t) and t.is_cuda and t.is_contiguous() and t.element_size() == 8
              and t.is_floating_point() == floating and t.device.index == ctx.device)
        if ok:
            import torch

            ok = floating or t.dtype == torch.int64
        if ok:
            torch.cuda.current_stream(t.device).synchronize()
        return ok

    def match_components(self, anchor, idx=None):
        on_device = self._on_device
        if not on_device(anchor, True):
            raise ValueError("anchor must be a float64 staging.DeviceArray / contiguous CUDA tensor on the context's GPU")
        n_el = int(np.prod(tuple(anchor.shape)))
        if n_el == 0 or n_el % self.n_u:
            raise ValueError(f"anchor shape {tuple(anchor.shape)} does not hold rows of {self.n_u} profiles")
        n_rows = n_el // self.n_u
        if idx is not None:
            if not on_device(idx, False):
                raise ValueError("idx must be the int64 row indices in HBM (staging.indices_to_device) on the context's GPU")
            if int(np.prod(tuple(idx.shape))) != self.problem.N:
                raise ValueError(f"idx holds {int(np.prod(tuple(idx.shape)))} indices, the problem has {self.problem.N} rows")
        P = np.empty((self.n_u, self.n_u), dtype=np.float64)
        L.check(self._lib.dmf_solver_match_components(self._h, _ptr(anchor), n_rows, _ptr(idx), _ptr(P)),
                "dmf_solver_match_components")
        return P

    def copy_u_to(self, tensor, columns=None):
        if not (_is_torch(tensor) and tensor.is_cuda and tensor.is_contiguous() and tensor.numel() == self.problem.N * self.n_u
                and tensor.element_size() == 8 and tensor.device.index == self.problem.ctx.device):
            raise ValueError("copy_u_to needs a contiguous float64 CUDA tensor of N * n_u elements on the context's GPU")
        if columns is not None:
            cols = np.ascontiguousarray(columns, dtype=np.int32).ravel()
            if cols.size != self.n_u or not np.array_equal(np.sort(cols), np.arange(self.n_u)):
                raise ValueError(f"columns must be a permutation of 0..{self.n_u - 1}, got {list(np.ravel(columns))}")
            L.check(self._lib.dmf_solver_get_u_permuted(self._h, cols.ctypes.data_as(C.POINTER(C.c_int32)), _ptr(tensor)),
                    "dmf_solver_get_u_permuted")
            return
        L.check(self._lib.dmf_solver_get(self._h, L.DMF_PTR_DEVICE, _ptr(tensor), None, None, None), "dmf_solver_get")

    def copy_u_by_cpg(self, tensor, idx, n_rows, columns=None):
        n_rows = int(n_rows)
        if not (_is_torch(tensor) and tensor.is_cuda and tensor.is_contiguous() and tensor.numel() == n_rows * self.n_u
                and n_rows >= 1 and tensor.element_size() == 8 and tensor.is_floating_point()
                and tensor.device.index == self.problem.ctx.device):
            raise ValueError("copy_u_by_cpg needs a contiguous float64 CUDA tensor of n_rows * n_u elements on the context's GPU")
        if not self._on_device(idx, False):
            raise ValueError("idx must be the int64 row indices in HBM (staging.indices_to_device) on the context's GPU")
        if int(np.prod(tuple(idx.shape))) != self.problem.N:
            raise ValueError(f"idx holds {int(np.prod(tuple(idx.shape)))} indices, the problem has {self.problem.N} rows")
        cols = None
        if columns is not None:
            cols = np.ascontiguousarray(columns, dtype=np.int32).ravel()
            if cols.size != self.n_u or not np.array_equal(np.sort(cols), np.arange(self.n_u)):
                raise ValueError(f"columns must be a permutation of 0..{self.n_u - 1}, got {list(np.ravel(columns))}")
            cols = cols.ctypes.data_as(C.POINTER(C.c_int32))
        L.check(self._lib.dmf_solver_get_u_by_row(self._h, _ptr(idx), n_rows, cols, _ptr(tensor)), "dmf_solver_get_u_by_row")

    def get_cost(self):
        cost, it = C.c_double(), C.c_int64()
        L.check(self._lib.dmf_solver_get(self._h, 0, None, None, C.byref(cost), C.byref(it)), "dmf_solver_get")
        return cost.value, it.value

    def close(self):
        if getattr(self, "_h", None):
            self._lib.dmf_solver_destroy(self._h)
            self._h = None

    def __del__(self):
        try:
            self.close()
        except Exception:
            pass

    def __enter__(self):
        return self

    def __exit__(self, *exc):
        self.close()
```

include/demethify_hip.h:

```cpp
#ifndef DEMETHIFY_HIP_H
#define DEMETHIFY_HIP_H

#include <stddef.h>
#include <stdint.h>

#ifdef __cplusplus
extern "C" {
#endif

typedef enum dmf_status {
    DMF_OK = 0,
    DMF_ERR_BAD_ARG = 1,
    DMF_ERR_BAD_SHAPE = 2,
    DMF_ERR_HIP = 3,
    DMF_ERR_NONFINITE = 4,
    DMF_ERR_UNSUPPORTED = 5,
    DMF_ERR_NO_DEVICE = 6
} dmf_status;

enum {
    DMF_PTR_DEVICE = 1,
    DMF_COUNTS_F64 = 2,
    DMF_INIT_IN_UNIT_RANGE = 4
};

enum {
    DMF_SELECT_COUNTS_F32_EXACT = 1,
    DMF_SELECT_PURITY = 2,
    DMF_SELECT_ALPHA_OUTSIDE_UNIT = 4,
    DMF_SELECT_V_UNALIGNED = 8,
    DMF_SELECT_X16 = 16
};

enum {
    DMF_MODE_PARTIAL = 0,
    DMF_MODE_UNSUPERVISED = 1
};

enum {
    DMF_KERNEL_ROWPASS = 0,
    DMF_KERNEL_GRAM = 1,
    DMF_KERNEL_ALPHA = 2,
    DMF_KERNEL_COST = 3,
    DMF_KERNEL_FAMILIES = 4
};

typedef struct dmf_context dmf_context;
typedef struct dmf_problem dmf_problem;
typedef struct dmf_solver dmf_solver;

const char* dmf_status_string(int status);
const char* dmf_last_error(void);
int dmf_abi_version(void);

int dmf_context_create(int device, void* stream, dmf_context** out);
int dmf_context_destroy(dmf_context* ctx);
int dmf_context_synchronize(dmf_context* ctx);
int dmf_context_set_profiling(dmf_context* ctx, int enabled);
int dmf_context_kernel_time(dmf_context* ctx, int family, double* total_ms, int64_t* launches);
int dmf_context_reset_kernel_time(dmf_context* ctx);
int dmf_context_set_generic(dmf_context* ctx, int level);
int dmf_context_set_x16(dmf_context* ctx, int enabled);
int dmf_context_set_rowpass_pair(dmf_context* ctx, int enabled);
int dmf_context_set_stop_confirmation(dmf_context* ctx, int mode);

int dmf_problem_create(dmf_context* ctx, int64_t N, int64_t S, int64_t n_c,
                       const double* V, const void* counts, const double* Rt,
                       int flags, dmf_problem** out);
int dmf_problem_gather(dmf_context* ctx, const dmf_problem* src, const int64_t* idx,
                       int64_t n_idx, dmf_problem** out);
int dmf_problem_gather_device(dmf_context* ctx, const dmf_problem* src, const int64_t* idx_dev,
                              int64_t n_idx, dmf_problem** out);
int dmf_problem_mask(dmf_context* ctx, const dmf_problem* src, const uint8_t* train_bits, int flags, dmf_problem** out);
int dmf_problem_destroy(dmf_problem* p);
int dmf_problem_shape(const dmf_problem* p, int64_t* N, int64_t* S, int64_t* n_c);
int dmf_problem_gram_known(const dmf_problem* p, double* out, char* out_text, int64_t cap);
enum { DMF_REPORT_INTS = 16, DMF_REPORT_DBLS = 8 };
int dmf_problem_report(const dmf_problem* p, int64_t* out_ints, double* out_dbls);
enum {
    DMF_ARRAY_V = 0, DMF_ARRAY_D = 1, DMF_ARRAY_RT = 2, DMF_ARRAY_RTP = 3, DMF_ARRAY_D16 = 4, DMF_ARRAY_X16 = 5,
    DMF_ARRAY_W16 = 6, DMF_ARRAY_DT8 = 7, DMF_ARRAY_MASK_BITS = 8, DMF_ARRAY_CONSTS = 9
};
int dmf_problem_copy_out(const dmf_problem* p, int which, void* out, int64_t bytes);

int dmf_cost(dmf_context* ctx, const dmf_problem* p, const double* u, int64_t n_u,
             const double* alpha, int flags, double* out_cost);
int dmf_cost_describe(int64_t S, int64_t n_c, int64_t n_u, int has_u16, int64_t SD, int v_align, int rtp_present, int level,
                      char* buf, int64_t cap);
int dmf_problem_cost_describe(dmf_context* ctx, const dmf_problem* p, int64_t n_u, char* buf, int64_t cap);
int dmf_gram_i8_describe(int64_t N, int64_t S, int64_t n_c, int64_t n_u, int nd, char* buf, int64_t cap);
int dmf_project_simplex(dmf_context* ctx, const double* X, int64_t K, int64_t S, double z,
                        int flags, double* out);
int dmf_update_u(dmf_context* ctx, const dmf_problem* p, const double* u, const double* u_prev,
                 const double* alpha, int64_t n_u, int64_t n_iter2, int mode, int flags,
                 double* scalars_io, double* out_u, double* out_u_prev);
int dmf_update_alpha(dmf_context* ctx, const dmf_problem* p, const double* u, int64_t n_u,
                     const double* alpha, const double* alpha_prev, int64_t n_iter2, int flags,
                     double* scalars_io, double* out_alpha, double* out_alpha_prev);

enum { DMF_WLS_TARGET_V = 0, DMF_WLS_TARGET_DV = 1 };
enum { DMF_WLS_F64_ARRAYS = 8 };
int dmf_wls_intercept(dmf_context* ctx, const dmf_problem* p, const double* u, int64_t n_u, int target,
                      int flags, double* out_alpha, int* out_status);
int dmf_wls_moments(dmf_context* ctx, const dmf_problem* p, const double* u, int64_t n_u, int target, int flags,
                    double* out_mom);
int dmf_nnls_normal(dmf_context* ctx, const double* gb, const double* mom, int64_t K, int64_t S, double* out_alpha,
                    int* out_status);

int dmf_svd_gram(dmf_context* ctx, const dmf_problem* p, const double* H1, int flags, double* out_C, int64_t* out_flags);
int dmf_svd_factor(dmf_context* ctx, const dmf_problem* p, const double* H1, const double* E_over_sigma, int64_t rank,
                   int flags, double* out_norms, void** out_T);
int dmf_svd_finish(dmf_context* ctx, void* T, int64_t N, int64_t rank, const double* sign, const double* scale, int flags,
                   double* out_u);

int dmf_percentile_axis0(dmf_context* ctx, const double* x, int64_t n, int64_t m, const double* q,
                         int64_t n_q, int flags, double* out);
int dmf_nanpercentile_axis0(dmf_context* ctx, const double* x, int64_t n, int64_t m, const double* q,
                            int64_t n_q, int flags, double* out);

int dmf_solver_create(dmf_context* ctx, const dmf_problem* p, const double* u0,
                      const double* alpha0, int64_t n_u, int mode, int flags, dmf_solver** out);
int dmf_solver_set_purity(dmf_solver* s, const double* purity, int flags);
int dmf_solver_step(dmf_solver* s, int64_t n_outer, int64_t n_iter2, double tol,
                    int64_t* iters_done_total, int* converged);
int dmf_solver_get(dmf_solver* s, int flags, double* out_u, double* out_alpha,
                   double* out_cost, int64_t* out_iters);
int dmf_solver_match_components(dmf_solver* s, const void* anchor_dev, int64_t n_anchor_rows, const int64_t* idx_dev,
                                double* out_P);
int dmf_solver_get_u_permuted(dmf_solver* s, const int32_t* src_col, void* dst_dev);
int dmf_solver_get_u_by_row(dmf_solver* s, const int64_t* idx_dev, int64_t n_dst_rows, const int32_t* src_col ,
                            void* dst_dev);
int dmf_solver_cost(dmf_solver* s, double* out_cost);
int dmf_solver_cost_begin(dmf_solver* s);
int dmf_solver_cost_end(dmf_solver* s, double* out_cost);
int dmf_solver_holdout_error(dmf_solver* s, const dmf_problem* full, double* sum_sq, int64_t* n_test);
enum { DMF_GRAM_INTEGER = 0, DMF_GRAM_FP64 = 1, DMF_GRAM_LAST = 2 };
int dmf_solver_gram(dmf_solver* s, int kind, double* out_gb, char* out_text, int64_t cap);
int dmf_solver_row_moments(dmf_solver* s, double* out_cm, char* out_text, int64_t cap);
enum { DMF_MOMENTUM_SCALARS = 16 };
int dmf_solver_momentum_state(const dmf_solver* s, double* scalars, double* alpha_prev, double* u_prev);
int dmf_solver_destroy(dmf_solver* s);
int dmf_solver_describe(const dmf_solver* s, int64_t n_iter2, char* buf, int64_t cap);
int dmf_select_describe(int64_t N, int64_t S, int64_t n_c, int64_t n_u, int nd, int level, int64_t n_iter2, int flags,
                        char* buf, int64_t cap);
enum { DMF_ROUTE_SOLVER = 0, DMF_ROUTE_UPDATE_U = 1 };
int dmf_u_phase_describe(int64_t N, int64_t S, int64_t n_c, int64_t n_u, int nd, int level, int64_t n_iter2, int flags, int route,
                         char* buf, int64_t cap);
int dmf_solver_u_phase_describe(const dmf_solver* s, int64_t n_iter2, int route, char* buf, int64_t cap);
int dmf_solver_stop_info(const dmf_solver* s, int* confirm_stops, int64_t* n_confirmed, int64_t* n_unconfirmed,
                         double* last_stream_cost);
int dmf_solver_rowpass_launches(const dmf_solver* s, int64_t* total, int64_t* paired);
int dmf_solve(dmf_context* ctx, const dmf_problem* p, const double* u0, const double* alpha0,
              int64_t n_u, int mode, int64_t n_iter1, int64_t n_iter2, double tol, int flags,
              double* out_u, double* out_alpha, double* out_cost, int64_t* out_iters);

int dmf_solve_small_supported(int64_t N, int64_t S, int64_t n_c, int64_t n_u, int mode);
int dmf_solve_small(dmf_context* ctx, const dmf_problem* p, int64_t B, const int64_t* idx, const double* u0,
                    const double* alpha0, int64_t n_u, int mode, int64_t n_iter1, int64_t n_iter2, double tol,
                    int64_t iters_per_launch, int flags, double* out_u, double* out_alpha, double* out_cost,
                    int64_t* out_iters);
int dmf_solve_small_purity(dmf_context* ctx, const dmf_problem* p, int64_t B, const int64_t* idx, const double* u0,
                           const double* alpha0, const double* purity, int64_t n_u, int mode, int64_t n_iter1,
                           int64_t n_iter2, double tol, int64_t iters_per_launch, int flags, double* out_u,
                           double* out_alpha, double* out_cost, int64_t* out_iters);

int dmf_table_scan(const char* path, char sep, int64_t* n_rows, int* col_percent_modified, int* col_valid_coverage,
                   int* n_cols);
int dmf_table_read(const char* path, char sep, int col_percent_modified, int col_valid_coverage, int64_t n_rows,
                   double* out_freq, int64_t stride_freq, double divide_by, int64_t* out_cov, int64_t stride_cov,
                   int n_threads);
void* dmf_host_alloc(size_t bytes, int* pinned);
void dmf_host_free(void* p, int pinned);

int dmf_write_interval_csv(const char* path, const char* header_line, const double* lower, const double* upper,
                           int64_t n_rows, int n_cols, int numpy_scalar_repr, int n_threads);

int dmf_stage_upload(dmf_context* ctx, const void* host, size_t bytes, void** out_dev);
int dmf_stage_free(dmf_context* ctx, void* dev);
int dmf_stage_download(dmf_context* ctx, const void* dev, size_t bytes, void* host);

int dmf_mask_draw(dmf_context* ctx, uint32_t key[624], int* pos, int64_t N, int64_t S,
                  uint64_t threshold, void** out_bits, int64_t* n_kept);

#ifdef __cplusplus
}
#endif
#endif
```

Measured before the change: 1799 outer iters/s.

## Defer rowpass phase C into a byte-packed LDS ring processed by idle waves

Adds a deferred-C variant of the paired rowpass kernel. X counts are packed to bytes in a 6-slot per-wave LDS ring, and the phase-C MFMA accumulation runs up to two cycles later on the waves not doing phase B, instead of after a block-wide barrier. A tail loop drains the remaining ring entries. The goal is to overlap phase C with phase B, remove the serialized phase-C step and shrink the X tile footprint. In exchange it adds LDS for the ring and extra ubuf sets, and it only applies when counts fit in a byte, S is 256 and the NKC/NU instance is allowed.

```diff
diff --git a/demethify_amd/_lib.py b/demethify_amd/_lib.py
--- a/demethify_amd/_lib.py
+++ b/demethify_amd/_lib.py
@@ -54,6 +54,7 @@
     "dmf_context_set_generic": (C.c_int, [_p, C.c_int]),
     "dmf_context_set_x16": (C.c_int, [_p, C.c_int]),
     "dmf_context_set_rowpass_pair": (C.c_int, [_p, C.c_int]),
+    "dmf_context_set_rowpass_defer_c": (C.c_int, [_p, C.c_int]),
     "dmf_context_set_stop_confirmation": (C.c_int, [_p, C.c_int]),
     "dmf_problem_create": (C.c_int, [_p, _i64, _i64, _i64, _p, _p, _p, C.c_int, C.POINTER(_p)]),
     "dmf_problem_gather": (C.c_int, [_p, _p, _p, _i64, C.POINTER(_p)]),
@@ -100,6 +101,7 @@
     "dmf_solver_u_phase_describe": (C.c_int, [_p, _i64, C.c_int, C.c_char_p, _i64]),
     "dmf_solver_stop_info": (C.c_int, [_p, C.POINTER(C.c_int), C.POINTER(_i64), C.POINTER(_i64), _dbl_p]),
     "dmf_solver_rowpass_launches": (C.c_int, [_p, C.POINTER(_i64), C.POINTER(_i64)]),
+    "dmf_solver_rowpass_schedule_counts": (C.c_int, [_p, C.POINTER(_i64), C.POINTER(_i64), C.POINTER(_i64)]),
     "dmf_table_scan": (C.c_int, [C.c_char_p, C.c_char, C.POINTER(_i64), C.POINTER(C.c_int), C.POINTER(C.c_int),
                                  C.POINTER(C.c_int)]),
     "dmf_table_read": (C.c_int, [C.c_char_p, C.c_char, C.c_int, C.c_int, _i64, _p, _i64, C.c_double, _p, _i64, C.c_int]),
diff --git a/demethify_amd/csrc/dmf_api.h b/demethify_amd/csrc/dmf_api.h
--- a/demethify_amd/csrc/dmf_api.h
+++ b/demethify_amd/csrc/dmf_api.h
@@ -54,6 +54,7 @@
     int generic_level = 0;
     bool x16 = true;
     bool rowpass_pair = true;
+    bool rowpass_defer_c = true;
     double* scratch = nullptr;
     hipMemPool_t pool = nullptr;
     std::unordered_map<void*, size_t> live;
@@ -226,6 +227,7 @@
     double cf_stream = 0.0;
     long long cf_stream_iter = -1;
     long long n_rowpass = 0, n_rowpass_pair = 0;
+    long long n_rowpass_defer = 0;
     long long n_confirmed = 0, n_unconfirmed = 0;
     dmf::IterateView iterate() const {
         dmf::IterateView it;
diff --git a/demethify_amd/csrc/dmf_api_context.hip b/demethify_amd/csrc/dmf_api_context.hip
--- a/demethify_amd/csrc/dmf_api_context.hip
+++ b/demethify_amd/csrc/dmf_api_context.hip
@@ -318,6 +318,12 @@
     return DMF_OK;
 }
 
+int dmf_context_set_rowpass_defer_c(dmf_context* ctx, int enabled) {
+    if (ctx == nullptr || enabled < 0 || enabled > 1) return DMF_ERR_BAD_ARG;
+    ctx->rowpass_defer_c = enabled != 0;
+    return DMF_OK;
+}
+
 int dmf_context_set_stop_confirmation(dmf_context* ctx, int mode) {
     if (ctx == nullptr || mode < 0 || mode > 2) return DMF_ERR_BAD_ARG;
     ctx->stop_confirmation = mode;
diff --git a/demethify_amd/csrc/dmf_api_solver.hip b/demethify_amd/csrc/dmf_api_solver.hip
--- a/demethify_amd/csrc/dmf_api_solver.hip
+++ b/demethify_amd/csrc/dmf_api_solver.hip
@@ -147,15 +147,16 @@
     const dmf::IterationPlan plan = dmf::plan_iteration(s->key, s->spec, n_iter2, s->purity != nullptr);
     if (plan.row == dmf::RowKind::RowpassV2) {
         int grid = 0;
-        bool paired = false;
+        bool paired = false, deferred = false;
         {
             FamilyScope scope(ctx, DMF_KERNEL_ROWPASS);
             dmf::ProblemView pv = p->view();
             if (!s->key.x16) pv.X16 = nullptr;
             HIP_TRY(dmf::launch_rowpass_v2(pv, s->iterate(), n_iter2, s->scratch(), &grid, s->key.rowpass_pair, &paired,
-                                           ctx->stream));
+                                           s->key.rowpass_defer_c && s->key.x_byte, &deferred, ctx->stream));
             ++s->n_rowpass;
             s->n_rowpass_pair += paired ? 1 : 0;
+            s->n_rowpass_defer += deferred ? 1 : 0;
         }
         return enqueue_gram_i8_tail(s, plan.alpha, n_iter2, grid);
     }
@@ -289,6 +290,8 @@
     key.SD = p->SD;
     key.x16 = key.nd > 0 && p->X16 != nullptr;
     key.rowpass_pair = ctx->rowpass_pair;
+    key.rowpass_defer_c = ctx->rowpass_defer_c;
+    key.x_byte = key.x16 && p->h_consts[kIntCountMax] <= 255.0;
     key.level = ctx->generic_level;
     key.d_f32_exact = p->d_f32_exact;
     key.rtp_present = n_c == 0 || p->Rtp != nullptr;
@@ -723,6 +726,14 @@
     return DMF_OK;
 }
 
+int dmf_solver_rowpass_schedule_counts(const dmf_solver* s, int64_t* total, int64_t* paired, int64_t* deferred) {
+    if (s == nullptr) return DMF_ERR_BAD_ARG;
+    if (total) *total = s->n_rowpass;
+    if (paired) *paired = s->n_rowpass_pair;
+    if (deferred) *deferred = s->n_rowpass_defer;
+    return DMF_OK;
+}
+
 int dmf_solve(dmf_context* ctx, const dmf_problem* p, const double* u0, const double* alpha0, int64_t n_u,
               int mode, int64_t n_iter1, int64_t n_iter2, double tol, int flags, double* out_u,
               double* out_alpha, double* out_cost, int64_t* out_iters) {
diff --git a/demethify_amd/csrc/dmf_internal.h b/demethify_amd/csrc/dmf_internal.h
--- a/demethify_amd/csrc/dmf_internal.h
+++ b/demethify_amd/csrc/dmf_internal.h
@@ -286,7 +286,7 @@
 bool rowpass_v2_supported(int S, int n_c, int n_u, int n_iter2);
 int rowpass_v2_grid(int64_t N, int S);
 hipError_t launch_rowpass_v2(const ProblemView& p, const IterateView& it, int n_iter2, const UScratch& scratch, int* grid_out,
-                             bool pair, bool* paired_out, hipStream_t st);
+                             bool pair, bool* paired_out, bool defer_c, bool* deferred_out, hipStream_t st);
 bool rowpass_v2_pair_fits(int S, int n_u, int n_iter2);
 bool gram_i8_supported(int n_c, int n_u, int ND, int64_t N, int SD);
 struct GramI8Plan {
diff --git a/demethify_amd/csrc/dmf_kernels_rowpass2.hip b/demethify_amd/csrc/dmf_kernels_rowpass2.hip
--- a/demethify_amd/csrc/dmf_kernels_rowpass2.hip
+++ b/demethify_amd/csrc/dmf_kernels_rowpass2.hip
@@ -15,11 +15,12 @@
 typedef int v4i __attribute__((ext_vector_type(4)));
 
 #ifdef DMF_STAMPS
-#define DMF2_STAMP_DECL unsigned long long st_last = dmf2_stamp(), st_seg[16] = {0, 0, 0, 0, 0, 0, 0, 0, 0, 0, 0, 0, 0, 0, 0, 0};
+#define DMF2_NSTAMP 20
+#define DMF2_STAMP_DECL unsigned long long st_last = dmf2_stamp(), st_seg[DMF2_NSTAMP] = {0, 0, 0, 0, 0, 0, 0, 0, 0, 0, 0, 0, 0, 0, 0, 0, 0, 0, 0, 0};
 #define DMF2_STAMP(i) { const unsigned long long st_now = dmf2_stamp(); st_seg[i] += st_now - st_last; st_last = st_now; }
 #define DMF2_STAMP_FLUSH                                                                                        \
     st_seg[15] = __builtin_amdgcn_s_getreg(4 | (31 << 11));                                                     \
-    if (lane == 0) for (int i_ = 0; i_ < 16; ++i_) stamps_out[((size_t)blockIdx.x * 4 + wave) * 16 + i_] = st_seg[i_];
+    if (lane == 0) for (int i_ = 0; i_ < DMF2_NSTAMP; ++i_) stamps_out[((size_t)blockIdx.x * 4 + wave) * DMF2_NSTAMP + i_] = st_seg[i_];
 __device__ __forceinline__ unsigned long long dmf2_stamp() {
     unsigned long long t;
     __builtin_amdgcn_sched_barrier(0);
@@ -40,6 +41,12 @@
 #ifndef DMF_V2_STAGGER
 #define DMF_V2_STAGGER 12
 #endif
+#ifndef DMF_V2_DEFER_PRIO
+#define DMF_V2_DEFER_PRIO 1
+#endif
+#ifndef DMF_V2_STAGGER_DEFER
+#define DMF_V2_STAGGER_DEFER 0
+#endif
 
 namespace {
 constexpr int kRowV = 66;
@@ -48,6 +55,9 @@
 constexpr int kTileDBytes2 = 16 * kRowD * 2;
 constexpr int kTileBytes2 = kTileVBytes2 + kTileDBytes2;
 constexpr int kTileBytesX = 2 * kTileDBytes2;
+constexpr int kRingBlockBytes = 16 * 64;
+constexpr int kRingBytes = 6 * kRingBlockBytes;
+constexpr int kDeferUbufSets = 6;
 }
 
 template <int NU, bool AT_PREV>
@@ -79,7 +89,7 @@
     }
 }
 
-template <int NKC, int NU, int MAXW = 4, bool XS = false, bool PAIR = false>
+template <int NKC, int NU, int MAXW = 4, bool XS = false, bool PAIR = false, bool DEFER_C = false>
 __global__ __launch_bounds__(64 * MAXW, MAXW == 4 ? 2 : 1) void k_rowpass_v2(
     const double* __restrict__ V, const unsigned short* __restrict__ D16, const unsigned short* __restrict__ X16, int SD,
     const double* __restrict__ Rtp,
@@ -92,7 +102,9 @@
     ) {
     static_assert(NU >= 1 && NU <= 4, "one phase-B pass per block, 4x4x4 MFMA for the c product");
     static_assert(!PAIR || (XS && MAXW == 4), "the pair schedule: X16 form, two workgroups per CU");
+    static_assert(!DEFER_C || PAIR, "the deferred-C schedule is a pair schedule");
     constexpr int NSET = PAIR ? 2 : 1;
+    constexpr int NUB = DEFER_C ? kDeferUbufSets : NSET;
     constexpr int NCT = 4 * NKC;
     constexpr int NP = NU * (NU + 1) / 2;
     constexpr int SLOT = (NU + 2) & ~1;
@@ -107,9 +119,9 @@
 
     double* __restrict__ beta_tab = lds_dyn;
     double* __restrict__ ubuf = beta_tab + ((n_iter2 + 1) & ~1);
-    double* __restrict__ red = ubuf + NSET * 16 * NU;
+    double* __restrict__ red = ubuf + NUB * 16 * NU;
     double* __restrict__ u2red = red + NSET * MAXW * NV * 16;
-    constexpr int TB = XS ? kTileBytesX : kTileBytes2;
+    constexpr int TB = XS ? (DEFER_C ? kTileDBytes2 : kTileBytesX) : kTileBytes2;
     char* __restrict__ tile = reinterpret_cast<char*>(u2red + MAXW) + (size_t)wave * TB;
     struct BlockTile {
         double* V;
@@ -119,6 +131,10 @@
         char* const t = tile + (size_t)set * NW * TB;
         unsigned short* const d = reinterpret_cast<unsigned short*>(t + (XS ? 0 : kTileVBytes2));
         return BlockTile{reinterpret_cast<double*>(t), d, d + 16 * kRowD};
+    };
+    unsigned int* const ring = reinterpret_cast<unsigned int*>(tile + (size_t)(NSET * NW - wave) * TB + (size_t)wave * kRingBytes);
+    auto ring_at = [&](int slot, int row, int dword) {
+        return ring + slot * (kRingBlockBytes / 4) + (4 * (row & 3) + (row >> 2)) * 16 + ((dword + 4 * (row & 3)) & 15);
     };
 
     if (const double* __restrict__ mrow = momentum_row(state, n_iter2)) {
@@ -262,9 +278,15 @@
     double* __restrict__ const mine_m1 = red + (size_t)wave * NV * 16 + (4 * q * NU + pl) * SLOT + 1 + (pj - pl + NU) % NU;
     double* __restrict__ const mine_m2 = red + (size_t)wave * NV * 16 + (4 * q * NU + pj) * SLOT + 1 + (pl - pj) % NU;
 
-    auto tile_store = [&](int set) {
+    auto tile_store = [&](int set, int rslot) {
         const BlockTile T = block_tile(set);
-        if constexpr (XS) {
+        if constexpr (DEFER_C) {
+#pragma unroll
+            for (int i = 0; i < 2; ++i)
+                *reinterpret_cast<v2u*>(ring_at(rslot, 8 * i + d_row, 2 * (lane & 7))) =
+                    v2u{__builtin_amdgcn_perm(px[set][i].y, px[set][i].x, 0x06040200u),
+                        __builtin_amdgcn_perm(px[set][i].w, px[set][i].z, 0x06040200u)};
+        } else if constexpr (XS) {
 #pragma unroll
             for (int i = 0; i < 2; ++i) *reinterpret_cast<v4u*>(T.X + (8 * i + d_row) * kRowD + d_col) = px[set][i];
         } else {
@@ -278,7 +300,7 @@
 #endif
     };
 
-    auto phase_a = [&](int set, int st_a, int st_p) {
+    auto phase_a = [&](int set, int rslot, int st_a, int st_p) {
         const BlockTile T = block_tile(set);
         const double* __restrict__ const tileV = T.V;
         unsigned short* __restrict__ const tileD = T.D;
@@ -293,7 +315,9 @@
         };
         using Strip = std::conditional_t<XS, StripX, StripV>;
         auto load_strip = [&](int t, Strip& R) {
-            if constexpr (XS) {
+            if constexpr (DEFER_C) {
+                R.xw.x = *ring_at(rslot, m16, 4 * t + q);
+            } else if constexpr (XS) {
                 R.xw = *reinterpret_cast<const v2u*>(tileX + m16 * kRowD + t * 16 + 4 * q);
             } else {
                 const double* __restrict__ tv = tileV + m16 * kRowV + t * 16 + 4 * qs;
@@ -312,7 +336,8 @@
             const v4d d = {(double)(R.dw.x & 0xFFFFu), (double)(R.dw.x >> 16), (double)(R.dw.y & 0xFFFFu), (double)(R.dw.y >> 16)};
             v4d w;
             if constexpr (XS) {
-                const v4d x = {(double)(R.xw.x & 0xFFFFu), (double)(R.xw.x >> 16), (double)(R.xw.y & 0xFFFFu), (double)(R.xw.y >> 16)};
+                const v4d x = DEFER_C ? v4d{(double)(R.xw.x & 0xFFu), (double)((R.xw.x >> 8) & 0xFFu), (double)((R.xw.x >> 16) & 0xFFu), (double)(R.xw.x >> 24)}
+                                      : v4d{(double)(R.xw.x & 0xFFFFu), (double)(R.xw.x >> 16), (double)(R.xw.y & 0xFFFFu), (double)(R.xw.y >> 16)};
 #pragma unroll
                 for (int r = 0; r < 4; ++r) w[r] = fma(d[r], e[r], x[r]);
             } else {
@@ -403,7 +428,7 @@
         DMF2_STAMP(st_p)
     };
 
-    auto phase_b = [&](int set, int64_t row0, double uu0, double up0) {
+    auto phase_b = [&](int uset, int set, int64_t row0, double uu0, double up0) {
         __builtin_amdgcn_s_setprio(3);
         DMF2_SUB_BEGIN
         const bool ok = b_lane && row0 + rl < N;
@@ -457,7 +482,7 @@
             }
         }
         DMF2_SUB(9)
-        if (b_lane) ubuf[set * 16 * NU + rl * NU + jb] = ok ? uu : 0.0;
+        if (b_lane) ubuf[uset * 16 * NU + rl * NU + jb] = ok ? uu : 0.0;
         if (ok) {
             const __amdgpu_buffer_rsrc_t ru = __builtin_amdgcn_make_buffer_rsrc((void*)(u + row0 * NU), 0, span((N - row0) * NU * 8), 0x00020000);
             const __amdgpu_buffer_rsrc_t rp = __builtin_amdgcn_make_buffer_rsrc((void*)(u_prev + row0 * NU), 0, span((N - row0) * NU * 8), 0x00020000);
@@ -500,12 +525,32 @@
 #endif
     };
 
+    auto phase_c_ring = [&](int pp, int b01) {
+        const int rslot = 2 * (pp % 3) + b01;
+        const double* __restrict__ const ub = ubuf + (2 * (pp % 3) + b01) * 16 * NU;
+        unsigned int xw[4];
+        double ua[4];
+#pragma unroll
+        for (int R = 0; R < 4; ++R) {
+            xw[R] = *ring_at(rslot, R + c_row, m16);
+            ua[R] = (m16 & 3) < NU ? ub[(R + c_row) * NU + (m16 & 3)] : 0.0;
+        }
+#pragma unroll
+        for (int R = 0; R < 4; ++R)
+#pragma unroll
+            for (int t = 0; t < 4; ++t)
+                bu[t] = __builtin_amdgcn_mfma_f64_4x4x4f64(ua[R], (double)((xw[R] >> (8 * t)) & 0xFFu), bu[t], 0, 0, 0);
+    };
+
     for (int s = 0; s < nk; s += NSET) {
         const bool has2 = PAIR && s + 1 < nk;
         const int64_t blk = blockIdx.x + (int64_t)s * gridDim.x;
+        const int cyc = s >> 1;
+        const bool b_role = !DEFER_C || (wave >> 1) == (cyc & 1);
         __builtin_amdgcn_s_setprio(1);
-        tile_store(0);
-        if (has2) tile_store(1);
+        const int rs0 = 2 * (cyc % 3);
+        tile_store(0, rs0);
+        if (has2) tile_store(1, rs0 + 1);
         const int bset = pair_set(s);
         const bool my_turn = bset == 1 || wave == s % NW;
         const double uu0 = pu;
@@ -513,13 +558,17 @@
         __builtin_amdgcn_wave_barrier();
         __builtin_amdgcn_s_setprio(0);
         DMF2_STAMP(0)
-        phase_a(0, 1, 2);
-        if (has2) phase_a(1, 11, 12);
+        phase_a(0, rs0, 1, 2);
+        if (has2) phase_a(1, rs0 + 1, 11, 12);
         asm volatile("s_waitcnt lgkmcnt(0)" ::: "memory");
         __builtin_amdgcn_s_barrier();
         DMF2_STAMP(3)
 #ifndef DMF_V2_NO_STAGGER
-        if (!my_turn) __builtin_amdgcn_s_sleep(DMF_V2_STAGGER);
+        if constexpr (!DEFER_C) {
+            if (!my_turn) __builtin_amdgcn_s_sleep(DMF_V2_STAGGER);
+        } else if (DMF_V2_STAGGER_DEFER > 0) {
+            if (!b_role) __builtin_amdgcn_s_sleep(DMF_V2_STAGGER_DEFER);
+        }
 #endif
         if (s + NSET < nk) {
             const int64_t nb = blk + NSET * (int64_t)gridDim.x;
@@ -527,16 +576,43 @@
             prefetch_tile(nb, 0);
             if (PAIR && s + 3 < nk) prefetch_tile(nb + gridDim.x, 1);
         }
-        DMF2_STAMP(7)
-        if (my_turn) phase_b(bset, (blk + (int64_t)bset * gridDim.x) * 16, uu0, up0);
+        if (b_role) { DMF2_STAMP(7) } else { DMF2_STAMP(16) }
+        if (my_turn) phase_b((DEFER_C ? rs0 : 0) + bset, bset, (blk + (int64_t)bset * gridDim.x) * 16, uu0, up0);
         DMF2_STAMP(4)
+        if constexpr (DEFER_C) {
+            if (!b_role) {
+                if (DMF_V2_DEFER_PRIO > 0) __builtin_amdgcn_s_setprio(DMF_V2_DEFER_PRIO);
+#pragma unroll 1
+                for (int pp = cyc < 2 ? 0 : cyc - 2; pp < cyc; ++pp) {
+                    phase_c_ring(pp, 0);
+                    phase_c_ring(pp, 1);
+                }
+                if (DMF_V2_DEFER_PRIO > 0) __builtin_amdgcn_s_setprio(0);
+            }
+            DMF2_STAMP(6)
+        }
         asm volatile("s_waitcnt lgkmcnt(0)" ::: "memory");
         __builtin_amdgcn_s_barrier();
-        DMF2_STAMP(5)
-        phase_c(0);
-        DMF2_STAMP(6)
-        if (has2) phase_c(1);
-        __builtin_amdgcn_s_setprio(0);
+        if (b_role) { DMF2_STAMP(5) } else { DMF2_STAMP(17) }
+        if constexpr (!DEFER_C) {
+            phase_c(0);
+            DMF2_STAMP(6)
+            if (has2) phase_c(1);
+            __builtin_amdgcn_s_setprio(0);
+            DMF2_STAMP(13)
+        }
+    }
+    if constexpr (DEFER_C) {
+        if (nk > 0) {
+            const int last = (nk - 1) >> 1;
+            const bool lone = (nk & 1) != 0;
+            const int first = ((wave >> 1) != (last & 1) || last == 0) ? last : last - 1;
+#pragma unroll 1
+            for (int pp = first; pp <= last; ++pp) {
+                phase_c_ring(pp, 0);
+                if (pp < last || !lone) phase_c_ring(pp, 1);
+            }
+        }
         DMF2_STAMP(13)
     }
 
@@ -547,7 +623,7 @@
     if (q < NU) {
 #pragma unroll
         for (int t = 0; t < 4; ++t) {
-            const int sC = wcol0 + 16 * t + m16;
+            const int sC = wcol0 + (DEFER_C ? 4 * m16 + t : 16 * t + m16);
             if (sC < S) slab[((int64_t)blockIdx.x * NU + q) * S + sC] = bu[t];
         }
     }
@@ -558,13 +634,15 @@
     }
 }
 
-size_t rowpass_v2_lds_bytes(int S, int n_u, int n_iter2, bool x16, bool pair = false) {
+size_t rowpass_v2_lds_bytes(int S, int n_u, int n_iter2, bool x16, bool pair = false, bool defer_c = false) {
     const int NW = (S + 63) / 64;
     const int maxw = NW <= 4 ? 4 : 8;
     const int nset = pair ? 2 : 1;
+    const int nub = defer_c ? kDeferUbufSets : nset;
     const int nv = n_u * ((n_u + 2) & ~1);
-    const size_t doubles = (size_t)((n_iter2 + 1) & ~1) + (size_t)nset * (16 * n_u + maxw * nv * 16) + maxw;
-    return doubles * sizeof(double) + (size_t)nset * NW * (x16 ? kTileBytesX : kTileBytes2);
+    const size_t doubles = (size_t)((n_iter2 + 1) & ~1) + (size_t)nub * 16 * n_u + (size_t)nset * maxw * nv * 16 + maxw;
+    const int tile = defer_c ? kTileDBytes2 : (x16 ? kTileBytesX : kTileBytes2);
+    return doubles * sizeof(double) + (size_t)nset * NW * tile + (defer_c ? (size_t)NW * kRingBytes : 0);
 }
 
 bool rowpass_v2_supported(int S, int n_c, int n_u, int n_iter2) {
@@ -580,6 +658,14 @@
     const int NW = (S + 63) / 64;
     if (NW < 2 || NW > 4) return false;
     return rowpass_v2_lds_bytes(S, n_u, n_iter2, true, true) * (size_t)rowpass_v2_per_cu(NW) <= (size_t)160 * 1024;
+}
+
+constexpr bool rowpass_v2_defer_instance(int nkc, int nu) { return !(nkc == 4 && nu >= 3); }
+bool rowpass_v2_defer_fits(int S, int n_c, int n_u, int n_iter2) {
+    const int NW = (S + 63) / 64;
+    if (NW != 4 || !rowpass_v2_pair_fits(S, n_u, n_iter2) || !rowpass_v2_defer_instance((n_c + 3) / 4, n_u)) return false;
+    const size_t lds = (rowpass_v2_lds_bytes(S, n_u, n_iter2, true, true, true) + 2047) & ~(size_t)2047;
+    return lds * (size_t)rowpass_v2_per_cu(NW) <= (size_t)160 * 1024;
 }
 
 int rowpass_v2_grid(int64_t N, int S) {
@@ -590,20 +676,22 @@
 }
 
 hipError_t launch_rowpass_v2(const ProblemView& p, const IterateView& it, int n_iter2, const UScratch& scratch, int* grid_out,
-                             bool pair, bool* paired_out, hipStream_t st) {
+                             bool pair, bool* paired_out, bool defer_c, bool* deferred_out, hipStream_t st) {
     const int S = p.S, NW = (S + 63) / 64;
     pair = pair && p.X16 != nullptr && rowpass_v2_pair_fits(S, it.n_u, n_iter2);
     if (paired_out != nullptr) *paired_out = pair;
+    defer_c = defer_c && pair && rowpass_v2_defer_fits(S, p.n_c, it.n_u, n_iter2);
+    if (deferred_out != nullptr) *deferred_out = defer_c;
     return dispatch_int<0, 4>((p.n_c + 3) / 4, [&](auto nkc) {
         return dispatch_bool(p.X16 != nullptr, [&](auto xs) {
             return dispatch_int<1, 4>(it.n_u, [&](auto nu) {
-                const auto launch = [&](auto maxw, auto pair_t) {
+                const auto launch = [&](auto maxw, auto pair_t, auto defer_t) {
                     constexpr int NU = decltype(nu)::value, MAXW = decltype(maxw)::value;
-                    constexpr bool XS = decltype(xs)::value, PAIR = decltype(pair_t)::value;
-                    constexpr auto kernel = k_rowpass_v2<decltype(nkc)::value, NU, MAXW, XS, PAIR>;
-                    const size_t lds = rowpass_v2_lds_bytes(S, NU, n_iter2, XS, PAIR);
+                    constexpr bool XS = decltype(xs)::value, PAIR = decltype(pair_t)::value, DEFER_C = decltype(defer_t)::value;
+                    constexpr auto kernel = k_rowpass_v2<decltype(nkc)::value, NU, MAXW, XS, PAIR, DEFER_C>;
+                    const size_t lds = rowpass_v2_lds_bytes(S, NU, n_iter2, XS, PAIR, DEFER_C);
                     constexpr size_t kLdsCap = (size_t)(MAXW == 4 ? 80 : 160) * 1024;
-                    if (NW > MAXW || (MAXW == 8 && NW <= 4) || (PAIR && NW < 2) || lds > kLdsCap || p.N < 1 ||
+                    if (NW > MAXW || (MAXW == 8 && NW <= 4) || (PAIR && NW < 2) || (DEFER_C && NW != 4) || lds > kLdsCap || p.N < 1 ||
                         p.SD < NW * 64 || (p.SD & 7) != 0 || p.ND < 1 || p.ND > 2)
                         return hipErrorInvalidValue;
                     if (lds > 48 * 1024) {
@@ -621,11 +709,14 @@
                                        );
                     return hipGetLastError();
                 };
-                if (S > 256) return launch(std::integral_constant<int, 8>{}, std::false_type{});
+                if (S > 256) return launch(std::integral_constant<int, 8>{}, std::false_type{}, std::false_type{});
                 if constexpr (decltype(xs)::value) {
-                    if (pair) return launch(std::integral_constant<int, 4>{}, std::true_type{});
+                    if constexpr (rowpass_v2_defer_instance(decltype(nkc)::value, decltype(nu)::value)) {
+                        if (pair && defer_c) return launch(std::integral_constant<int, 4>{}, std::true_type{}, std::true_type{});
+                    }
+                    if (pair) return launch(std::integral_constant<int, 4>{}, std::true_type{}, std::false_type{});
                 }
-                return launch(std::integral_constant<int, 4>{}, std::false_type{});
+                return launch(std::integral_constant<int, 4>{}, std::false_type{}, std::false_type{});
             });
         });
     });
diff --git a/demethify_amd/csrc/dmf_select.h b/demethify_amd/csrc/dmf_select.h
--- a/demethify_amd/csrc/dmf_select.h
+++ b/demethify_amd/csrc/dmf_select.h
@@ -17,6 +17,8 @@
     int SD = 0;
     bool x16 = false;
     bool rowpass_pair = true;
+    bool rowpass_defer_c = true;
+    bool x_byte = false;
     int level = 0;
     bool d_f32_exact = false;
     bool rtp_present = true;
diff --git a/demethify_amd/device.py b/demethify_amd/device.py
--- a/demethify_amd/device.py
+++ b/demethify_amd/device.py
@@ -87,6 +87,9 @@
 
     def set_rowpass_pair(self, enabled: bool):
         L.check(self._lib.dmf_context_set_rowpass_pair(self._h, int(bool(enabled))), "dmf_context_set_rowpass_pair")
+
+    def set_rowpass_defer_c(self, enabled: bool):
+        L.check(self._lib.dmf_context_set_rowpass_defer_c(self._h, int(bool(enabled))), "dmf_context_set_rowpass_defer_c")
 
     def set_stop_confirmation(self, mode: int):
         L.check(self._lib.dmf_context_set_stop_confirmation(self._h, int(mode)), "dmf_context_set_stop_confirmation")
@@ -704,6 +707,12 @@
                 "dmf_solver_rowpass_launches")
         return total.value, paired.value
 
+    def rowpass_schedule_counts(self):
+        total, paired, deferred = C.c_int64(), C.c_int64(), C.c_int64()
+        L.check(self._lib.dmf_solver_rowpass_schedule_counts(self._h, C.byref(total), C.byref(paired), C.byref(deferred)),
+                "dmf_solver_rowpass_schedule_counts")
+        return total.value, paired.value, deferred.value
+
     def get_alpha(self):
         alpha = np.empty((self.K, self.problem.S), dtype=np.float64)
         L.check(self._lib.dmf_solver_get(self._h, 0, None, _ptr(alpha), None, None), "dmf_solver_get")
diff --git a/include/demethify_hip.h b/include/demethify_hip.h
--- a/include/demethify_hip.h
+++ b/include/demethify_hip.h
@@ -62,6 +62,7 @@
 int dmf_context_set_generic(dmf_context* ctx, int level);
 int dmf_context_set_x16(dmf_context* ctx, int enabled);
 int dmf_context_set_rowpass_pair(dmf_context* ctx, int enabled);
+int dmf_context_set_rowpass_defer_c(dmf_context* ctx, int enabled);
 int dmf_context_set_stop_confirmation(dmf_context* ctx, int mode);
 
 int dmf_problem_create(dmf_context* ctx, int64_t N, int64_t S, int64_t n_c,
@@ -150,6 +151,7 @@
 int dmf_solver_stop_info(const dmf_solver* s, int* confirm_stops, int64_t* n_confirmed, int64_t* n_unconfirmed,
                          double* last_stream_cost);
 int dmf_solver_rowpass_launches(const dmf_solver* s, int64_t* total, int64_t* paired);
+int dmf_solver_rowpass_schedule_counts(const dmf_solver* s, int64_t* total, int64_t* paired, int64_t* deferred);
 int dmf_solve(dmf_context* ctx, const dmf_problem* p, const double* u0, const double* alpha0,
               int64_t n_u, int mode, int64_t n_iter1, int64_t n_iter2, double tol, int flags,
               double* out_u, double* out_alpha, double* out_cost, int64_t* out_iters);
```

Measured after the change: 1851 outer iters/s, median of 6. +2.9%, better.
